# hongsukchoi/Pose2Mesh_RELEASE

Hardware: AMD Instinct MI355X
Metric: SMPL meshes/sec fwd+bwd at batch 256 (higher is better)
Workload: dtype f32 (emulated on the BF16 matrix pipe: every operand as 3 exact bf16 slices = 24-bit significands, 6 slice products per fp32 product, fp32 accumulate)

## Files before the change

include/p2m.h:

```cpp
#ifndef P2M_H_
#define P2M_H_

#include <stddef.h>
#include <stdint.h>

#ifdef __cplusplus
extern "C" {
#endif

typedef enum {
  P2M_OK = 0,
  P2M_ERR_INVALID = -1,
  P2M_ERR_HIP = -2,
  P2M_ERR_NOMEM = -3
} p2m_status;

enum { P2M_ARITH_F32 = 0, P2M_ARITH_BF16X3 = 1, P2M_ARITH_F16X2 = 2 };

typedef struct p2m_graph* p2m_graph_t;

const char* p2m_last_error_string(void);
const char* p2m_version(void);
int p2m_stream_capture_id(void* stream, unsigned long long* id_out);

int p2m_graph_create(const int32_t* row_ptr, const int32_t* col, const float* val,
                     int32_t V, int32_t nnz, p2m_graph_t* out);
int p2m_graph_destroy(p2m_graph_t g);
int p2m_graph_info(p2m_graph_t g, int32_t info[4]);

int p2m_cheb_basis_fwd(p2m_graph_t g, const float* X, float* T1, float* T2,
                       int32_t B, int32_t F, int32_t in_shift, void* stream);

int p2m_cheb_basis_bwd(p2m_graph_t g, const float* d0, const float* d1, const float* d2,
                       const float* resid, float* dX,
                       int32_t B, int32_t F, int32_t out_shift, void* stream);

int p2m_cheb_combine_small(p2m_graph_t g, const float* P, int32_t ldp, int32_t nc, const float* bias,
                           float* Y, int32_t B, void* stream);
int p2m_cheb_expand_small(p2m_graph_t g, const float* G, int32_t nc, float* E, int32_t lde, int32_t B,
                          void* stream);
int p2m_cheb_combine_small_real(p2m_graph_t g, const float* P, int32_t ldp, int32_t nc, const float* bias, float* Y,
                                int32_t B, const int32_t* out_index, int32_t out_rows, float scale, void* stream);

int p2m_weight_pack(const float* W, float* Wt, float* W2, float* W3, int32_t Fout, int32_t Fin, int32_t K,
                    void* stream);
int p2m_weight_grad_unpack(const float* P, const float* Pdb, int32_t nchunks, float* dW, float* db,
                           int32_t Fout, int32_t Fin, int32_t K, int32_t accumulate, int32_t layout,
                           int32_t pdb_stride, void* stream);

int p2m_gemm_planes(const float* A0, const float* A1, const float* A2, int32_t nplanesA, int32_t Ka,
                    int32_t a0_shift, const float* Bm, const void* Bsplit, int32_t arith, const void* a_amax,
                    int32_t a_bits, const float* bias, const float* addend,
                    float* C0, float* C1, float* C2, int32_t nplanesC, int32_t Nc, int32_t pair_out,
                    int64_t M, float* stats, const float* act_scale, const float* act_shift, int32_t act_relu,
                    void* amax_out, void* stream);
int64_t p2m_weight_split_elems(int32_t K, int32_t N, int32_t arith);
int p2m_weight_split(const float* Bm, int32_t K, int32_t N, int32_t arith, const void* amax_in, int32_t amax_bits,
                     void* Bx, void* stream);
typedef struct p2m_conv_weights {
  const float* W;
  int32_t Fout, Fin;
  float fake_a, fake_b;
  int32_t eff_bits, reserved;
  void *Bx_f, *Bx_ef, *Bx_b, *Bx_eb;
  void* amax;
} p2m_conv_weights;
int p2m_conv_weights_prepare(const p2m_conv_weights* dev_desc, int32_t n, int32_t arith, void* stream);
int p2m_amax(const float* x, int64_t n, void* word, void* stream);
int p2m_amax_rows(p2m_graph_t g, int32_t row_set, const float* x, int32_t B, int32_t F, void* word, void* stream);
int32_t p2m_stats_tile_rows(void);

int p2m_gemm_tn(const float* A0, const float* A1, const float* A2, int32_t nplanesA, int32_t Ka,
                int32_t a0_shift, const float* G0, const float* G1, const float* G2, int32_t nplanesG,
                int32_t Gc, int64_t M, int64_t chunk_rows, float* P, float* Pdb, int32_t arith,
                const void* a_amax, int32_t a_bits, const void* g_amax, int32_t g_bits, void* stream);

int p2m_bn_finalize(const float* stats, int32_t ntiles, int64_t M, const float* gamma, const float* beta,
                    float* running_mean, float* running_var, float momentum, float eps,
                    float* mean, float* invstd, float* scale, float* shift, int32_t N, int32_t tile_rows,
                    void* stream);
int p2m_bn_eval_coeffs(const float* gamma, const float* beta, const float* running_mean,
                       const float* running_var, float eps, float* mean, float* invstd, float* scale,
                       float* shift, int32_t N, void* stream);
int p2m_bn_act_fwd(const float* y, const float* scale, const float* shift, int32_t relu,
                   const float* resid, int32_t Fres, int32_t res_shift,
                   float* x, int64_t M, int32_t F, p2m_graph_t classes , int32_t real_rows_only,
                   void* amax_out, void* stream);
int32_t p2m_bn_bwd_blocks(int64_t M, int32_t F);
int32_t p2m_bn_bwd_blocks_classes(p2m_graph_t classes, int64_t M, int32_t F);
int p2m_bn_bwd_reduce(const float* gx, const float* y, const float* scale, const float* shift,
                      const float* mean, const float* invstd, int32_t relu, float* part,
                      int64_t M, int32_t F, p2m_graph_t classes, void* stream);
int p2m_bn_bwd_finalize(const float* part, int32_t nblk, int64_t M, float* dgamma, float* dbeta,
                        float* coef, int32_t accumulate, int32_t F, void* stream);
int32_t p2m_bn_bwd_blocks_fake(p2m_graph_t g, int32_t B, int32_t F);
int p2m_bn_bwd_reduce_fake(p2m_graph_t g, const float* gx, const float* y, const float* scale, const float* shift,
                           const float* mean, const float* invstd, int32_t relu, float* part, int32_t B, int32_t F,
                           void* stream);
int p2m_bn_bwd_apply(const float* gx, const float* y, const float* scale, const float* shift,
                     const float* mean, const float* invstd, const float* gamma, const float* coef,
                     int32_t relu, float* gy, float* pair_gx, float* pair_gy, int64_t M, int32_t F,
                     p2m_graph_t classes, int32_t zero_holes, void* amax_out, void* stream);

int p2m_pair_sum(const float* in, float* out, int64_t Mout, int32_t F, p2m_graph_t classes ,
                 void* stream);
int p2m_lerp_bwd_add(const float* g, float* dst, int64_t M, int32_t F, int32_t Fres, void* stream);

int p2m_graph_split_info(p2m_graph_t g, int32_t counts[2] , float coef[2] );
int p2m_cheb_basis_fwd_real(p2m_graph_t g, const float* X, float* T1c, float* T2c, int32_t B, int32_t F,
                            int32_t in_shift, const float* act_scale , const float* act_shift, void* stream);
int p2m_graph_pair_info(p2m_graph_t g, int32_t counts[2] );
int p2m_graph_plan_info(p2m_graph_t g, int32_t ntiles[3]);
int p2m_cheb_basis_pair(p2m_graph_t g, const float* G, float* P1c, float* P2c, int32_t B, int32_t F, void* stream);
int p2m_gemm_planes_rows(p2m_graph_t g, int32_t row_set, int32_t B, const float* A0, const float* A1,
                         const float* A2, int32_t nplanesA, int32_t Ka, int32_t a0_shift, int32_t planes_compact,
                         const float* Bm, const void* Bsplit, int32_t arith, const void* a_amax, int32_t a_bits,
                         const float* bias, const float* addend, float* C,
                         int32_t N, float* stats, const float* act_scale, const float* act_shift, int32_t act_relu,
                         void* amax_out, const float* in_scale , const float* in_shift, void* stream);
int32_t p2m_rows_tiles_per_sample(p2m_graph_t g, int32_t row_set);
int p2m_gemm_tn_rows(p2m_graph_t g, int32_t row_set, int32_t B, const float* A, int32_t Ka, int32_t a0_shift,
                     const float* G0, const float* G1, const float* G2, int32_t nplanesG, int32_t Gc,
                     int32_t planes_compact, int32_t splits, float* P, float* Pdb, int32_t arith,
                     const void* a_amax, const void* g_amax, int32_t g_bits, const float* a_scale,
                     const float* a_shift, void* stream);
int p2m_weight_eff(const float* Wt, float* We, int32_t Ka, int32_t N, float a, float b, void* stream);
int p2m_weight_grad_unpack2(const float* P, const float* Pdb, int32_t nchunks, const float* P2, const float* Pdb2,
                            int32_t nchunks2, float s1, float s2, float* dW, float* db, int32_t Fout, int32_t Fin,
                            int32_t K, int32_t accumulate, void* stream);
int p2m_bn_finalize_rows(const float* stats_a, int32_t tps_a, int32_t rows_a, const float* stats_b, int32_t tps_b,
                         int32_t rows_b, int32_t B, const float* gamma, const float* beta, float* running_mean,
                         float* running_var, float momentum, float eps, float* mean, float* invstd, float* scale,
                         float* shift, int32_t N, void* stream);

int p2m_bn_finalize_split(p2m_graph_t g, const float* stats_real, const float* stats_fake, int32_t B,
                          const float* gamma, const float* beta, float* running_mean, float* running_var,
                          float momentum, float eps, float* mean, float* invstd, float* scale, float* shift,
                          int32_t N, void* stream);

int32_t p2m_cheb_tile_gemm_supported(p2m_graph_t g, int32_t plan, int32_t Ka, int32_t N);
int32_t p2m_cheb_tile_gemm_bnr_slots(p2m_graph_t g, int32_t plan, int32_t arith, int32_t N, int32_t B);
int32_t p2m_cheb_tile_gemm_mg(int32_t arith, int32_t N);
int p2m_cheb_tile_gemm(p2m_graph_t g, int32_t plan, const float* X, const float* A0, int32_t Ka, const void* Bx,
                       int32_t arith, const void* x_amax, const float* bias, const float* addend, float* C, int32_t N,
                       float* stats, float* E1, float* E2, const float* act_scale, const float* act_shift,
                       int32_t act_relu, void* amax_out, const float* in_scale, const float* in_shift,
                       const float* bnr_y, const float* bnr_co, float* bnr_part, int32_t B, void* stream);
int p2m_act_bound(const float* scale, const float* shift, int32_t N, const void* y_amax, void* word, void* stream);
int32_t p2m_graph_plane_bits(p2m_graph_t g, int32_t plan);
int p2m_bn_finalize_tiles(p2m_graph_t g, int32_t plan, const float* stats_real, const float* stats_fake, int32_t B,
                          const float* gamma, const float* beta, float* running_mean, float* running_var,
                          float momentum, float eps, float* mean, float* invstd, float* scale, float* shift,
                          int32_t N, void* stream);

int p2m_graph_fake_ids(p2m_graph_t g, int32_t* out );
int p2m_graph_real_ids(p2m_graph_t g, int32_t* out);
int p2m_graph_set_classes(p2m_graph_t g, const int32_t* rep_of );
int p2m_graph_class_info(p2m_graph_t g, int32_t counts[3] );
int p2m_stats_rows_w(p2m_graph_t g, const float* y, int32_t B, int32_t N, float* stats, void* stream);
int p2m_class_reduce(p2m_graph_t g, const float* in, float* out, int32_t B, int32_t F, void* stream);

int p2m_chebconv_fwd(p2m_graph_t g, const float* X, const float* Wt, const float* bias,
                     float* T1, float* T2, float* Y, float* stats,
                     int32_t B, int32_t Fin, int32_t Fout, int32_t in_shift, void* stream);

int64_t p2m_mesh_loss_workspace(int32_t B, int32_t nv, int32_t F, int32_t J);
int p2m_mesh_loss(const float* cam_mesh, int32_t V0, const int32_t* perm, int32_t nv, const float* gt_mesh,
                  const float* valid_mesh, const int32_t* faces, int32_t F, const int32_t* vf_ptr,
                  const int32_t* vf_idx, const int32_t* jr_ptr, const int32_t* jr_idx, const float* jr_val,
                  const int32_t* vj_ptr, const int32_t* vj_idx, const float* vj_val, int32_t J,
                  const float* gt_pose, const float* valid_pose, float w_vertex, float w_normal, float w_edge,
                  float w_joint, float* workspace, float* losses, float* grad_cam, int32_t B, void* stream);

int p2m_coord_loss(const float* pred, const float* target, const float* valid, int32_t per_mask, int64_t n, float w,
                   float* loss, float* grad, void* stream);

int p2m_mesh_epilogue(const float* cam_mesh, int32_t V0, const int32_t* perm, int32_t nv, float scale,
                      const int32_t* jr_ptr, const int32_t* jr_idx, const float* jr_val, int32_t J,
                      float* mesh, float* joints, int32_t B, void* stream);

int p2m_rigid_align(const float* A, const float* B, int32_t nb, int32_t N, float* c, float* R, float* t, float* A2,
                    void* stream);
int p2m_mesh_eval(const float* pred_mesh, const float* gt_mesh, int32_t B, int32_t B_real, int32_t nv, float gt_mesh_scale,
                  const int32_t* ra_ptr, const int32_t* ra_idx, const float* ra_val, int32_t JA, int32_t root_A,
                  const int32_t* sub_A, int32_t nsub_A, const float* pred_joints_A, const float* gt_joints_A,
                  const int32_t* re_ptr, const int32_t* re_idx, const float* re_val, int32_t JE, int32_t root_E, const int32_t* sub_E,
                  int32_t nsub_E, const float* gt_joints_E, int32_t pa_mesh, float* mpjpe_A, float* mpvpe, float* mpjpe_E,
                  float* pa_mpjpe_E, float* pa_mpvpe, double* sample_means, const int32_t* group, int32_t n_groups,
                  double* totals, void* stream);

int32_t p2m_nn_target_tile(void);
int32_t p2m_nn_query_tile(int32_t n);
int64_t p2m_nn_workspace(int32_t B, int32_t nA, int32_t nB);
int p2m_mesh_fscore(const float* pred_mesh, const float* gt_mesh, int32_t B, int32_t B_real, int32_t nv, float gt_mesh_scale,
                    const int32_t* r_ptr, const int32_t* r_idx, const float* r_val, int32_t J, int32_t root,
                    const float* pred_centre, const float* gt_centre, int32_t variants, const float* thresholds,
                    int32_t n_thresholds, void* workspace, int64_t workspace_bytes, float* d_pred, float* d_gt,
                    float* pa_d_pred, float* pa_d_gt, int32_t* counts, double* scores, const int32_t* group, int32_t n_groups,
                    double* totals, void* stream);
int p2m_point_nn(const float* A, const float* B, int32_t nb, int32_t nA, int32_t nB, float* dAB, float* dBA, void* workspace,
                 int64_t workspace_bytes, void* stream);

// ... 142 lines not shown
```

pose2mesh_release_amd/_lib.py:

```python
import ctypes
import os

HERE = os.path.dirname(os.path.abspath(__file__))
LIBDIR = os.path.join(HERE, "lib")


class P2MError(RuntimeError):
    pass


_c = ctypes
_i32, _i64, _f32, _f64, _vp = _c.c_int32, _c.c_int64, _c.c_float, _c.c_double, _c.c_void_p


class FitSchedule(_c.Structure):
    _fields_ = [("n", _i32), ("first_step", _i32 * 8), ("lr", _f64 * 8)]


HIP_SYMBOLS = {
    "p2m_last_error_string": (_c.c_char_p, []),
    "p2m_version": (_c.c_char_p, []),
    "p2m_stream_capture_id": (_c.c_int, [_vp, _c.POINTER(_c.c_uint64)]),
    "p2m_graph_create": (_c.c_int, [_vp, _vp, _vp, _i32, _i32, _c.POINTER(_vp)]),
    "p2m_graph_destroy": (_c.c_int, [_vp]),
    "p2m_graph_info": (_c.c_int, [_vp, _c.POINTER(_i32 * 4)]),
    "p2m_cheb_basis_fwd": (_c.c_int, [_vp, _vp, _vp, _vp, _i32, _i32, _i32, _vp]),
    "p2m_cheb_basis_bwd": (_c.c_int, [_vp, _vp, _vp, _vp, _vp, _vp, _i32, _i32, _i32, _vp]),
    "p2m_cheb_combine_small": (_c.c_int, [_vp, _vp, _i32, _i32, _vp, _vp, _i32, _vp]),
    "p2m_cheb_combine_small_real": (_c.c_int, [_vp, _vp, _i32, _i32, _vp, _vp, _i32, _vp, _i32, _f32, _vp]),
    "p2m_cheb_expand_small": (_c.c_int, [_vp, _vp, _i32, _vp, _i32, _i32, _vp]),
    "p2m_weight_pack": (_c.c_int, [_vp, _vp, _vp, _vp, _i32, _i32, _i32, _vp]),
    "p2m_weight_grad_unpack": (_c.c_int, [_vp, _vp, _i32, _vp, _vp, _i32, _i32, _i32, _i32, _i32, _i32, _vp]),
    "p2m_graph_split_info": (_c.c_int, [_vp, _c.POINTER(_i32 * 2), _c.POINTER(_f32 * 2)]),
    "p2m_cheb_basis_fwd_real": (_c.c_int, [_vp, _vp, _vp, _vp, _i32, _i32, _i32, _vp, _vp, _vp]),
    "p2m_graph_pair_info": (_c.c_int, [_vp, _c.POINTER(_i32 * 2)]),
    "p2m_graph_plan_info": (_c.c_int, [_vp, _c.POINTER(_i32 * 3)]),
    "p2m_cheb_basis_pair": (_c.c_int, [_vp, _vp, _vp, _vp, _i32, _i32, _vp]),
    "p2m_gemm_planes_rows": (_c.c_int, [_vp, _i32, _i32, _vp, _vp, _vp, _i32, _i32, _i32, _i32, _vp, _vp, _i32, _vp, _i32,
                                        _vp, _vp, _vp, _i32, _vp, _vp, _vp, _i32, _vp, _vp, _vp, _vp]),
    "p2m_rows_tiles_per_sample": (_i32, [_vp, _i32]),
    "p2m_gemm_tn_rows": (_c.c_int, [_vp, _i32, _i32, _vp, _i32, _i32, _vp, _vp, _vp, _i32, _i32, _i32, _i32, _vp, _vp,
                                    _i32, _vp, _vp, _i32, _vp, _vp, _vp]),
    "p2m_weight_eff": (_c.c_int, [_vp, _vp, _i32, _i32, _f32, _f32, _vp]),
    "p2m_weight_grad_unpack2": (_c.c_int, [_vp, _vp, _i32, _vp, _vp, _i32, _f32, _f32, _vp, _vp, _i32, _i32, _i32,
                                           _i32, _vp]),
    "p2m_bn_finalize_rows": (_c.c_int, [_vp, _i32, _i32, _vp, _i32, _i32, _i32, _vp, _vp, _vp, _vp, _f32, _f32, _vp,
                                        _vp, _vp, _vp, _i32, _vp]),
    "p2m_bn_finalize_split": (_c.c_int, [_vp, _vp, _vp, _i32, _vp, _vp, _vp, _vp, _f32, _f32, _vp, _vp, _vp, _vp, _i32,
                                         _vp]),
    "p2m_cheb_tile_gemm_supported": (_i32, [_vp, _i32, _i32, _i32]),
    "p2m_cheb_tile_gemm_mg": (_i32, [_i32, _i32]),
    "p2m_cheb_tile_gemm": (_c.c_int, [_vp, _i32, _vp, _vp, _i32, _vp, _i32, _vp, _vp, _vp, _vp, _i32, _vp, _vp, _vp, _vp,
                                      _vp, _i32, _vp, _vp, _vp, _vp, _vp, _vp, _i32, _vp]),
    "p2m_cheb_tile_gemm_bnr_slots": (_i32, [_vp, _i32, _i32, _i32, _i32]),
    "p2m_bn_bwd_blocks_fake": (_i32, [_vp, _i32, _i32]),
    "p2m_bn_bwd_reduce_fake": (_c.c_int, [_vp, _vp, _vp, _vp, _vp, _vp, _vp, _i32, _vp, _i32, _i32, _vp]),
    "p2m_act_bound": (_c.c_int, [_vp, _vp, _i32, _vp, _vp, _vp]),
    "p2m_graph_plane_bits": (_i32, [_vp, _i32]),
    "p2m_amax": (_c.c_int, [_vp, _i64, _vp, _vp]),
    "p2m_conv_weights_prepare": (_c.c_int, [_vp, _i32, _i32, _vp]),
    "p2m_amax_rows": (_c.c_int, [_vp, _i32, _vp, _i32, _i32, _vp, _vp]),
    "p2m_bn_finalize_tiles": (_c.c_int, [_vp, _i32, _vp, _vp, _i32, _vp, _vp, _vp, _vp, _f32, _f32, _vp, _vp, _vp, _vp,
                                         _i32, _vp]),
    "p2m_graph_fake_ids": (_c.c_int, [_vp, _vp]),
    "p2m_graph_real_ids": (_c.c_int, [_vp, _vp]),
    "p2m_graph_set_classes": (_c.c_int, [_vp, _vp]),
    "p2m_graph_class_info": (_c.c_int, [_vp, _c.POINTER(_i32 * 3)]),
    "p2m_stats_rows_w": (_c.c_int, [_vp, _vp, _i32, _i32, _vp, _vp]),
    "p2m_class_reduce": (_c.c_int, [_vp, _vp, _vp, _i32, _i32, _vp]),
    "p2m_gemm_planes": (_c.c_int, [_vp, _vp, _vp, _i32, _i32, _i32, _vp, _vp, _i32, _vp, _i32, _vp, _vp, _vp, _vp, _vp,
                                   _i32, _i32, _i32, _i64, _vp, _vp, _vp, _i32, _vp, _vp]),
    "p2m_weight_split_elems": (_i64, [_i32, _i32, _i32]),
    "p2m_weight_split": (_c.c_int, [_vp, _i32, _i32, _i32, _vp, _i32, _vp, _vp]),
    "p2m_stats_tile_rows": (_i32, []),
    "p2m_gemm_tn": (_c.c_int, [_vp, _vp, _vp, _i32, _i32, _i32, _vp, _vp, _vp, _i32, _i32, _i64, _i64, _vp, _vp,
                               _i32, _vp, _i32, _vp, _i32, _vp]),
    "p2m_bn_finalize": (_c.c_int, [_vp, _i32, _i64, _vp, _vp, _vp, _vp, _f32, _f32, _vp, _vp, _vp, _vp,
                                   _i32, _i32, _vp]),
    "p2m_bn_eval_coeffs": (_c.c_int, [_vp, _vp, _vp, _vp, _f32, _vp, _vp, _vp, _vp, _i32, _vp]),
    "p2m_bn_act_fwd": (_c.c_int, [_vp, _vp, _vp, _i32, _vp, _i32, _i32, _vp, _i64, _i32, _vp, _i32, _vp, _vp]),
    "p2m_bn_bwd_blocks": (_i32, [_i64, _i32]),
    "p2m_bn_bwd_blocks_classes": (_i32, [_vp, _i64, _i32]),
    "p2m_bn_bwd_reduce": (_c.c_int, [_vp, _vp, _vp, _vp, _vp, _vp, _i32, _vp, _i64, _i32, _vp, _vp]),
    "p2m_bn_bwd_finalize": (_c.c_int, [_vp, _i32, _i64, _vp, _vp, _vp, _i32, _i32, _vp]),
    "p2m_bn_bwd_apply": (_c.c_int, [_vp, _vp, _vp, _vp, _vp, _vp, _vp, _vp, _i32, _vp, _vp, _vp, _i64, _i32, _vp,
                                    _i32, _vp, _vp]),
    "p2m_pair_sum": (_c.c_int, [_vp, _vp, _i64, _i32, _vp, _vp]),
    "p2m_lerp_bwd_add": (_c.c_int, [_vp, _vp, _i64, _i32, _i32, _vp]),
    "p2m_coord_loss": (_c.c_int, [_vp, _vp, _vp, _i32, _i64, _f32, _vp, _vp, _vp]),
    "p2m_mesh_loss_workspace": (_i64, [_i32, _i32, _i32, _i32]),
    "p2m_mesh_loss": (_c.c_int, [_vp, _i32, _vp, _i32, _vp, _vp, _vp, _i32, _vp, _vp, _vp, _vp, _vp, _vp, _vp, _vp,
                                 _i32, _vp, _vp, _f32, _f32, _f32, _f32, _vp, _vp, _vp, _i32, _vp]),
    "p2m_mesh_epilogue": (_c.c_int, [_vp, _i32, _vp, _i32, _f32, _vp, _vp, _vp, _i32, _vp, _vp, _i32, _vp]),
    "p2m_adam_step": (_c.c_int, [_vp, _vp, _vp, _vp, _i64, _i64, _f32, _f32, _f32, _f32, _f32, _vp]),
    "p2m_rmsprop_step": (_c.c_int, [_vp, _vp, _vp, _i64, _f32, _f32, _f32, _f32, _vp]),
    "p2m_adam_step_dev": (_c.c_int, [_vp, _vp, _vp, _vp, _i64, _vp, _f32, _f32, _f32, _vp]),
    "p2m_rmsprop_step_dev": (_c.c_int, [_vp, _vp, _vp, _i64, _vp, _f32, _f32, _vp]),
    "p2m_gemm_tn_acc": (_c.c_int, [_vp, _i32, _vp, _i32, _i64, _vp, _i32, _vp, _vp, _vp]),
    "p2m_pn_stage_fwd": (_c.c_int, [_vp, _i32, _vp, _vp, _vp, _i32, _i32, _vp, _vp, _vp, _vp, _f32, _f32, _vp, _f32, _vp,
                                    _vp, _vp, _vp, _vp, _i32, _i32, _i32, _vp]),
    "p2m_pn_stage_bwd": (_c.c_int, [_vp, _i32, _vp, _i32, _i32, _vp, _vp, _vp, _vp, _vp, _vp, _f32, _vp, _vp, _vp, _vp,
                                    _vp, _i32, _vp, _i32, _i32, _i32, _vp]),
    "p2m_chebconv_fwd": (_c.c_int, [_vp, _vp, _vp, _vp, _vp, _vp, _vp, _vp, _i32, _i32, _i32, _i32, _vp]),
    "p2m_rigid_align": (_c.c_int, [_vp, _vp, _i32, _i32, _vp, _vp, _vp, _vp, _vp]),
    "p2m_mesh_eval": (_c.c_int, [_vp, _vp, _i32, _i32, _i32, _f32, _vp, _vp, _vp, _i32, _i32, _vp, _i32, _vp, _vp, _vp, _vp,
                                 _vp, _i32, _i32, _vp, _i32, _vp, _i32, _vp, _vp, _vp, _vp, _vp, _vp, _vp, _i32, _vp, _vp]),
    "p2m_nn_target_tile": (_i32, []),
    "p2m_nn_query_tile": (_i32, [_i32]),
    "p2m_nn_workspace": (_i64, [_i32, _i32, _i32]),
    "p2m_mesh_fscore": (_c.c_int, [_vp, _vp, _i32, _i32, _i32, _f32, _vp, _vp, _vp, _i32, _i32, _vp, _vp, _i32, _vp, _i32,
                                   _vp, _i64, _vp, _vp, _vp, _vp, _vp, _vp, _vp, _i32, _vp, _vp]),
    "p2m_point_nn": (_c.c_int, [_vp, _vp, _i32, _i32, _i32, _vp, _vp, _vp, _i64, _vp]),
    "p2m_error_profile_workspace": (_i64, [_i32, _i32]),
    "p2m_error_profile": (_c.c_int, [_vp, _vp, _vp, _i32, _i32, _i32, _f32, _i32, _i32, _vp, _i32, _vp, _i64, _vp, _vp, _vp,
                                     _vp, _i32, _vp, _vp, _vp, _vp, _vp, _vp, _vp]),
    "p2m_body_sample_tile": (_i32, []),
    "p2m_body_vertex_tile": (_i32, []),
    "p2m_body_workspace": (_i64, [_i32, _i32, _i32]),
    "p2m_body_forward": (_c.c_int, [_vp, _vp, _vp, _i32, _vp, _i32, _f32, _i32, _i32, _i32, _i32, _vp, _vp, _vp, _vp, _vp,
                                    _vp, _vp, _i32, _vp, _vp, _i32, _vp, _vp, _vp, _i32, _vp, _i64, _vp, _vp, _vp, _vp]),
    "p2m_body_backward_workspace": (_i64, [_i32, _i32, _i32, _i32]),
    "p2m_body_backward": (_c.c_int, [_vp, _vp, _vp, _i32, _i32, _i32, _f32, _i32, _i32, _i32, _i32, _vp, _vp, _vp, _vp, _vp,
                                     _vp, _vp, _vp, _i32, _vp, _vp, _i32, _vp, _vp, _vp, _i32, _vp, _i64, _vp, _vp, _vp, _vp,
                                     _i64, _vp, _vp, _vp, _vp]),
    "p2m_pose_noise_coco": (_c.c_int, [_vp, _vp, _vp, _vp, _vp, _vp, _i32, _vp]),
    "p2m_pose_noise_table": (_c.c_int, [_vp, _vp, _vp, _vp, _i32, _f32, _f32, _vp, _vp, _i32, _vp]),
    "p2m_train_sample_workspace": (_i64, [_i32]),
    "p2m_train_sample": (_c.c_int, [_vp, _vp, _f32, _vp, _vp, _i32, _i32, _vp, _vp, _vp, _i32, _i32, _vp, _vp, _vp, _i32, _vp,
                                    _i32, _i32, _vp, _vp, _f32, _vp, _vp, _f32, _i32, _i32, _vp, _vp, _vp, _vp, _vp, _i32,
                                    _f32, _f32, _vp, _vp, _i64] + [_vp] * 12),
    "p2m_annot_gather": (_c.c_int, [_vp] * 10 + [_i64, _i32, _i32, _i32, _vp, _i32, _i32, _vp, _vp, _i32, _i32, _i32, _i32,
                                    _f64, _f64] + [_vp] * 10),
    "p2m_body_select": (_c.c_int, [_vp, _vp, _vp, _i32, _vp, _i32, _i32, _i32, _i32, _vp, _vp, _vp, _vp]),
    "p2m_mesh_project": (_c.c_int, [_vp, _vp, _i32, _i32, _i32, _i32, _vp, _vp, _vp]),
    "p2m_mesh_render_workspace": (_c.c_int, [_i32, _i32, _i32, _i32, _i32, _c.POINTER(_i64)]),
    "p2m_mesh_render": (_c.c_int, [_vp, _vp, _i32, _vp, _vp, _vp, _i32, _f32, _f32, _f32, _i32, _vp, _i32, _i32, _i32, _i32,
                                   _i32, _i32, _vp, _vp, _vp, _vp, _vp, _vp, _vp]),
    "p2m_vertex_normals": (_c.c_int, [_vp, _vp, _vp, _vp, _i32, _i32, _i32, _i32, _vp, _vp, _vp]),
    "p2m_mesh_shade": (_c.c_int, [_vp, _vp, _vp, _vp, _i32, _vp, _vp, _vp, _i32, _vp, _vp, _i32, _f32, _vp, _i32, _i32, _vp, _i32,
                                  _vp, _i32, _f32, _i32, _i32, _i32, _i32, _i32, _vp, _vp, _vp, _vp, _vp]),
    "p2m_pose_prepare": (_c.c_int, [_vp, _i32, _i32, _f32, _f32, _f32, _vp, _vp, _vp, _vp, _vp]),
    "p2m_camera_fit": (_c.c_int, [_vp, _vp, _vp, _vp, _vp, _i32, _i32, FitSchedule, _i32, _f32, _f64, _f64, _f64, _vp, _vp, _vp,
                                  _vp]),
    "p2m_one_euro_lookahead": (_i32, []),
    "p2m_one_euro": (_c.c_int, [_vp, _vp, _vp, _i32, _i32, _i32, _f64, _f64, _f64, _f64, _vp, _vp, _vp, _vp, _vp]),
    "p2m_video_eval": (_c.c_int, [_vp, _vp, _vp, _vp, _i32, _i32, _i32, _i32, _vp, _vp, _vp, _vp, _vp, _vp, _vp, _vp]),
    "p2m_pose_overlay_workspace": (_c.c_int, [_i32, _i32, _i32, _i32, _c.POINTER(_i64)]),
    "p2m_pose_overlay": (_c.c_int, [_vp, _i32, _i32, _i32, _i32, _vp, _i32, _vp, _i32, _vp, _c.c_uint32, _vp, _vp, _i32, _i32,
                                    _f32, _i32, _i32, _i32, _i32, _i32, _vp, _vp, _i64, _vp]),
    "p2m_crowd_select": (_c.c_int, [_vp, _vp, _i32, _i32, _i32, _vp, _i32, _f64, _f64, _f64, _vp, _vp, _vp, _vp, _vp, _vp, _vp,
                                    _vp]),
    "p2m_person_colours": (_c.c_int, [_vp, _i32, _f64, _f64, _vp, _vp, _vp]),
    "p2m_pose_track": (_c.c_int, [_vp, _i32, _i32, _i32, _i32, _i32, _f64, _f64, _i32, _i32, _vp, _vp, _vp, _vp, _vp, _vp, _vp,
                                  _vp, _vp, _vp, _vp, _vp]),
}

HOST_SYMBOLS = {
    "p2m_hem_match": (_i64, [_vp, _vp, _vp, _i64, _vp, _i64, _vp, _vp]),
    "p2m_tree_order_level": (_i64, [_vp, _i64, _vp, _i64, _vp]),
# ... 40 lines not shown
```

pose2mesh_release_amd/csrc/basis.hip:

```cpp
#include <cstdlib>

#include "p2m_common.h"

namespace p2m {

constexpr int ROWS_PER_BLOCK = 4;

static int basis_spb() { return 8; }

static bool basis_tiled() {
  static int v = [] { const char* e = getenv("P2M_BASIS_TILED"); return e ? atoi(e) : 1; }();
  return v != 0;
}

__device__ __forceinline__ int xcd_swizzle(int bid, int nb) {
  return (nb & 7) == 0 ? (bid & 7) * (nb >> 3) + (bid >> 3) : bid;
}

__device__ __forceinline__ void fma4(float4& acc, float s, const float4& x) {
  acc.x = fmaf(s, x.x, acc.x); acc.y = fmaf(s, x.y, acc.y);
  acc.z = fmaf(s, x.z, acc.z); acc.w = fmaf(s, x.w, acc.w);
}

template <int LPR>
// ... 137 lines not shown
  const long ibase = (long)b * g.V * F + f;
  float acc = 0.f;
  for (int ch = 0; ch < (1 << out_shift); ch++) {
    int row = (p << out_shift) + ch;
    acc += d0[ibase + (long)row * F];
    if (resid) acc += resid[ibase + (long)row * F];
    for (int j = g.rowptr[row]; j < g.rowptr[row + 1]; j++) {
      long o = ibase + (long)g.col[j] * F;
      acc = fmaf(g.a[j], d1[o], acc);
      acc = fmaf(g.b[j], d2[o], acc);
    }
  }
  dX[idx] = acc;
}

template <int NC>
__global__ __launch_bounds__(256) void k_combine_small(Graph g, const float* __restrict__ P, int ldp,
                                                        const float* __restrict__ bias, float* __restrict__ Y, int B,
                                                        const int* __restrict__ ids, int nset,
                                                        const int* __restrict__ out_index, int out_rows, float scale,
                                                        int skip_real) {
  const int n = ids ? nset : g.V;
  long idx = (long)blockIdx.x * blockDim.x + threadIdx.x;
  if (idx >= (long)B * n) return;
  const int b = (int)(idx / n);
  const int i = (int)(idx - (long)b * n);
  const int row = ids ? ids[i] : i;
  if (skip_real && g.rowptr[row + 1] - g.rowptr[row] > 1) return;
  const long base = (long)b * g.V * ldp;
  const int src = g.rep_of ? g.rep_of[row] : row;
  const float* p0 = P + base + (long)src * ldp;
  float acc[NC];
#pragma unroll
  for (int c = 0; c < NC; c++) acc[c] = p0[c] + (bias ? bias[c] : 0.f);
  for (int j = g.rowptr[src]; j < g.rowptr[src + 1]; j++) {
    const float* q = P + base + (long)g.col[j] * ldp;
    const float a = g.a[j], bb = g.b[j];
#pragma unroll
    for (int c = 0; c < NC; c++) acc[c] = fmaf(bb, q[2 * NC + c], fmaf(a, q[NC + c], acc[c]));
  }
  long orow = row;
  int rows_out = g.V;
  if (out_index) {
    orow = out_index[row];
    rows_out = out_rows;
    if (orow < 0) return;
  }
  float* y = Y + ((long)b * rows_out + orow) * NC;
#pragma unroll
  for (int c = 0; c < NC; c++) y[c] = out_index ? acc[c] * scale : acc[c];
}

template <int NC>
__global__ __launch_bounds__(256) void k_expand_small(Graph g, const float* __restrict__ G, float* __restrict__ E,
                                                       int lde, int B, int skip_real) {
  long idx = (long)blockIdx.x * blockDim.x + threadIdx.x;
  if (idx >= (long)B * g.V) return;
  const int row = (int)(idx % g.V);
  if (skip_real && g.rowptr[row + 1] - g.rowptr[row] > 1) return;
  const long base = (idx - row) * NC;
  float t1[NC], t2[NC];
#pragma unroll
  for (int c = 0; c < NC; c++) t1[c] = t2[c] = 0.f;
  for (int j = g.rowptr[row]; j < g.rowptr[row + 1]; j++) {
    const float* q = G + base + (long)g.col[j] * NC;
    const float a = g.a[j], b = g.b[j];
#pragma unroll
    for (int c = 0; c < NC; c++) {
      t1[c] = fmaf(a, q[c], t1[c]);
      t2[c] = fmaf(b, q[c], t2[c]);
    }
  }
  float* e = E + idx * lde;
#pragma unroll
  for (int c = 0; c < NC; c++) {
    e[c] = G[idx * NC + c];
    e[NC + c] = t1[c];
    e[2 * NC + c] = t2[c];
  }
  for (int c = 3 * NC; c < lde; c++) e[c] = 0.f;
}

constexpr int SMALL_SPB = 8;
template <int NC>
__global__ __launch_bounds__(256) void k_combine_small_tile(TilePlan pl, const int* __restrict__ real_ids, int V,
                                                             const float* __restrict__ P, int ldp,
                                                             const float* __restrict__ bias, float* __restrict__ Y, int B,
                                                             const int* __restrict__ out_index, int out_rows,
                                                             float scale) {
  __shared__ float4 ents[TILE_ECAP];
  __shared__ int rowoff[TILE_RMAX + 1];
  __shared__ float xs[SMALL_SPB][TILE_UCAP][2 * NC];
  const int tile = blockIdx.x % pl.ntiles, sg = blockIdx.x / pl.ntiles;
  const int t = threadIdx.x;
  const int r0 = pl.tile_row[tile], R = pl.tile_row[tile + 1] - r0;
  const int u0 = pl.tile_u[tile], U = pl.tile_u[tile + 1] - u0;
  const int e0 = pl.erow[r0], nE = pl.erow[r0 + R] - e0;
  for (int i = t; i < nE; i += 256) ents[i] = pl.ent[e0 + i];
  if (t <= R) rowoff[t] = pl.erow[r0 + t] - e0;
  const int b0 = sg * SMALL_SPB;
  for (int q = t; q < U * SMALL_SPB; q += 256) {
    const int u = q % U, sl = q / U, b = b0 + sl;
    if (b < B) {
      const float* src = P + ((long)b * V + pl.ucol[u0 + u]) * ldp + NC;
#pragma unroll
      for (int c = 0; c < 2 * NC; c++) xs[sl][u][c] = src[c];
    }
  }
  __syncthreads();
  const int i = t % TILE_RMAX, sl = t / TILE_RMAX, b = b0 + sl;
  if (i >= R || b >= B) return;
  const int row = real_ids[r0 + i];
  const float* p0 = P + ((long)b * V + row) * ldp;
  float acc[NC];
#pragma unroll
  for (int c = 0; c < NC; c++) acc[c] = p0[c] + (bias ? bias[c] : 0.f);
  for (int j = rowoff[i]; j < rowoff[i + 1]; j++) {
    const float4 en = ents[j];
    const float* q = xs[sl][__float_as_int(en.z)];
#pragma unroll
    for (int c = 0; c < NC; c++) acc[c] = fmaf(en.y, q[NC + c], fmaf(en.x, q[c], acc[c]));
  }
  long orow = row;
  int rows_out = V;
  if (out_index) {
    orow = out_index[row];
    rows_out = out_rows;
    if (orow < 0) return;
  }
  float* y = Y + ((long)b * rows_out + orow) * NC;
#pragma unroll
  for (int c = 0; c < NC; c++) y[c] = out_index ? acc[c] * scale : acc[c];
}

template <int NC>
__global__ __launch_bounds__(256) void k_expand_small_tile(TilePlan pl, const int* __restrict__ real_ids, int V,
                                                            const float* __restrict__ G, float* __restrict__ E, int lde,
                                                            int B) {
  __shared__ float4 ents[TILE_ECAP];
  __shared__ int rowoff[TILE_RMAX + 1];
  __shared__ float xs[SMALL_SPB][TILE_UCAP][NC];
  const int tile = blockIdx.x % pl.ntiles, sg = blockIdx.x / pl.ntiles;
  const int t = threadIdx.x;
  const int r0 = pl.tile_row[tile], R = pl.tile_row[tile + 1] - r0;
  const int u0 = pl.tile_u[tile], U = pl.tile_u[tile + 1] - u0;
  const int e0 = pl.erow[r0], nE = pl.erow[r0 + R] - e0;
  for (int i = t; i < nE; i += 256) ents[i] = pl.ent[e0 + i];
  if (t <= R) rowoff[t] = pl.erow[r0 + t] - e0;
  const int b0 = sg * SMALL_SPB;
  for (int q = t; q < U * SMALL_SPB; q += 256) {
    const int u = q % U, sl = q / U, b = b0 + sl;
    if (b < B) {
      const float* src = G + ((long)b * V + pl.ucol[u0 + u]) * NC;
#pragma unroll
      for (int c = 0; c < NC; c++) xs[sl][u][c] = src[c];
    }
  }
  __syncthreads();
  const int i = t % TILE_RMAX, sl = t / TILE_RMAX, b = b0 + sl;
  if (i >= R || b >= B) return;
  const long ridx = (long)b * V + real_ids[r0 + i];
  float t1[NC], t2[NC];
#pragma unroll
  for (int c = 0; c < NC; c++) t1[c] = t2[c] = 0.f;
  for (int j = rowoff[i]; j < rowoff[i + 1]; j++) {
    const float4 en = ents[j];
    const float* q = xs[sl][__float_as_int(en.z)];
#pragma unroll
    for (int c = 0; c < NC; c++) {
      t1[c] = fmaf(en.x, q[c], t1[c]);
      t2[c] = fmaf(en.y, q[c], t2[c]);
    }
  }
  float* e = E + ridx * lde;
#pragma unroll
  for (int c = 0; c < NC; c++) {
    e[c] = G[ridx * NC + c];
    e[NC + c] = t1[c];
    e[2 * NC + c] = t2[c];
  }
  for (int c = 3 * NC; c < lde; c++) e[c] = 0.f;
}

constexpr int EXP_NC = 3, EXP_Q = 3;

__device__ __forceinline__ void expand_stage_row(float4* r, const float* g, const float* t1, const float* t2) {
  r[0] = make_float4(g[0], g[1], g[2], t1[0]);
  r[1] = make_float4(t1[1], t1[2], t2[0], t2[1]);
  r[2] = make_float4(t2[2], 0.f, 0.f, 0.f);
}

__device__ __forceinline__ void expand_copy_out(const float4* res, const long* erow, int nrows, float* __restrict__ E, int lde) {
  const int L4 = lde >> 2;
  for (int u = threadIdx.x; u < nrows * L4; u += 256) {
    const int i = u / L4, q = u - i * L4;
    const long er = erow[i];
    if (er < 0) continue;
    const float4 v = q < EXP_Q ? res[i * EXP_Q + q] : make_float4(0.f, 0.f, 0.f, 0.f);
    reinterpret_cast<float4*>(E + er * lde)[q] = v;
// ... 23 lines not shown
          t1[c] = fmaf(a, q[c], t1[c]);
          t2[c] = fmaf(b, q[c], t2[c]);
        }
      }
#pragma unroll
      for (int c = 0; c < EXP_NC; c++) gv[c] = G[idx * EXP_NC + c];
      expand_stage_row(res + threadIdx.x * EXP_Q, gv, t1, t2);
      er = idx;
    }
  }
  erow[threadIdx.x] = er;
  __syncthreads();
  expand_copy_out(res, erow, 256, E, lde);
}

__global__ __launch_bounds__(256) void k_expand_small_tile_rows(TilePlan pl, const int* __restrict__ real_ids, int V,
                                                                 const float* __restrict__ G, float* __restrict__ E, int lde,
                                                                 int B) {
  __shared__ float4 ents[TILE_ECAP];
  __shared__ int rowoff[TILE_RMAX + 1];
  __shared__ float xs[SMALL_SPB][TILE_UCAP][EXP_NC];
  __shared__ float4 res[256 * EXP_Q];
  __shared__ long erow[256];
  const int bid = xcd_block_id(blockIdx.x, gridDim.x);
  const int tile = bid % pl.ntiles, sg = bid / pl.ntiles;
  const int t = threadIdx.x;
  const int r0 = pl.tile_row[tile], R = pl.tile_row[tile + 1] - r0;
  const int u0 = pl.tile_u[tile], U = pl.tile_u[tile + 1] - u0;
  const int e0 = pl.erow[r0], nE = pl.erow[r0 + R] - e0;
  for (int i = t; i < nE; i += 256) ents[i] = pl.ent[e0 + i];
  if (t <= R) rowoff[t] = pl.erow[r0 + t] - e0;
  const int b0 = sg * SMALL_SPB;
  for (int q = t; q < U * SMALL_SPB; q += 256) {
    const int u = q % U, sl = q / U, b = b0 + sl;
    if (b < B) {
      const float* src = G + ((long)b * V + pl.ucol[u0 + u]) * EXP_NC;
#pragma unroll
      for (int c = 0; c < EXP_NC; c++) xs[sl][u][c] = src[c];
    }
  }
  __syncthreads();
  const int i = t % TILE_RMAX, sl = t / TILE_RMAX, b = b0 + sl;
  long er = -1;
  if (i < R && b < B) {
    const long ridx = (long)b * V + real_ids[r0 + i];
    float t1[EXP_NC], t2[EXP_NC], gv[EXP_NC];
#pragma unroll
    for (int c = 0; c < EXP_NC; c++) t1[c] = t2[c] = 0.f;
    for (int j = rowoff[i]; j < rowoff[i + 1]; j++) {
      const float4 en = ents[j];
      const float* q = xs[sl][__float_as_int(en.z)];
#pragma unroll
      for (int c = 0; c < EXP_NC; c++) {
        t1[c] = fmaf(en.x, q[c], t1[c]);
        t2[c] = fmaf(en.y, q[c], t2[c]);
      }
    }
#pragma unroll
    for (int c = 0; c < EXP_NC; c++) gv[c] = G[ridx * EXP_NC + c];
    expand_stage_row(res + t * EXP_Q, gv, t1, t2);
    er = ridx;
  }
  erow[t] = er;
  __syncthreads();
  expand_copy_out(res, erow, 256, E, lde);
}

}

using namespace p2m;

static int combine_small_launch(p2m_graph_t gh, const float* P, int32_t ldp, int32_t nc, const float* bias, float* Y,
                                int32_t B, int real_only, const int32_t* out_index, int32_t out_rows, float scale,
                                void* stream) {
  const Graph& g = *reinterpret_cast<const Graph*>(gh);
  const int* ids = real_only ? g.real_ids : nullptr;
  const int nset = real_only ? g.n_real : g.V;
  const long tot = (long)B * nset;
  if (tot == 0) return P2M_OK;
  hipStream_t s = (hipStream_t)stream;
  int skip_real = 0;
  const TilePlan& pl = g.plan[0];
  if (pl.ntiles > 0 && basis_tiled() && nc == 3) {
    hipLaunchKernelGGL(k_combine_small_tile<3>, dim3(pl.ntiles * cdiv(B, SMALL_SPB)), dim3(256), 0, s, pl, g.real_ids, g.V,
                       P, ldp, bias, Y, B, out_index, out_rows, scale);
    if (real_only) return check_launch("cheb_combine_small(tiled)");
    skip_real = 1;
  }
#define P2M_COMBINE(NCv) hipLaunchKernelGGL(k_combine_small<NCv>, dim3(cdiv(tot, 256)), dim3(256), 0, s, g, P, ldp, bias, \
                                            Y, B, ids, nset, out_index, out_rows, scale, skip_real)
  switch (nc) {
    case 1: P2M_COMBINE(1); break;
    case 2: P2M_COMBINE(2); break;
    case 3: P2M_COMBINE(3); break;
    case 4: P2M_COMBINE(4); break;
    default: set_error("p2m_cheb_combine_small: nc must be 1..4 (got %d)", nc); return P2M_ERR_INVALID;
  }
#undef P2M_COMBINE
  return check_launch("cheb_combine_small");
}

extern "C" int p2m_cheb_combine_small(p2m_graph_t gh, const float* P, int32_t ldp, int32_t nc, const float* bias,
                                      float* Y, int32_t B, void* stream) {
  P2M_CHECK_ARG(gh && P && Y && ldp >= 3 * nc, "null pointer or ldp < 3*nc");
  if (B <= 0) return P2M_OK;
  return combine_small_launch(gh, P, ldp, nc, bias, Y, B, 0, nullptr, 0, 1.f, stream);
}

extern "C" int p2m_cheb_combine_small_real(p2m_graph_t gh, const float* P, int32_t ldp, int32_t nc, const float* bias,
                                           float* Y, int32_t B, const int32_t* out_index, int32_t out_rows,
                                           float scale, void* stream) {
  P2M_CHECK_ARG(gh && P && Y && ldp >= 3 * nc, "null pointer or ldp < 3*nc");
  P2M_CHECK_ARG(out_index == nullptr || out_rows > 0, "out_rows must be positive with out_index");
  if (B <= 0) return P2M_OK;
  return combine_small_launch(gh, P, ldp, nc, bias, Y, B, 1, out_index, out_rows, scale, stream);
}

extern "C" int p2m_cheb_expand_small(p2m_graph_t gh, const float* G, int32_t nc, float* E, int32_t lde, int32_t B,
                                     void* stream) {
  P2M_CHECK_ARG(gh && G && E && lde >= 3 * nc, "null pointer or lde < 3*nc");
  if (B <= 0) return P2M_OK;
  const Graph& g = *reinterpret_cast<const Graph*>(gh);
  const long tot = (long)B * g.V;
  hipStream_t s = (hipStream_t)stream;
  int skip_real = 0;
  const TilePlan& pl = g.plan[0];
  const bool rows16 = nc == 3 && lde % 4 == 0 && (reinterpret_cast<uintptr_t>(E) & 15) == 0 && narrow_rows();
  if (pl.ntiles > 0 && basis_tiled() && nc == 3) {
    if (rows16)
      hipLaunchKernelGGL(k_expand_small_tile_rows, dim3(pl.ntiles * cdiv(B, SMALL_SPB)), dim3(256), 0, s, pl, g.real_ids,
                         g.V, G, E, lde, B);
    else
      hipLaunchKernelGGL(k_expand_small_tile<3>, dim3(pl.ntiles * cdiv(B, SMALL_SPB)), dim3(256), 0, s, pl, g.real_ids, g.V,
                         G, E, lde, B);
    skip_real = 1;
  }
  if (rows16) {
    hipLaunchKernelGGL(k_expand_small_rows, dim3(cdiv(tot, 256)), dim3(256), 0, s, g, G, E, lde, B, skip_real);
    return check_launch("cheb_expand_small");
  }
  switch (nc) {
    case 1: hipLaunchKernelGGL(k_expand_small<1>, dim3(cdiv(tot, 256)), dim3(256), 0, s, g, G, E, lde, B, skip_real); break;
    case 2: hipLaunchKernelGGL(k_expand_small<2>, dim3(cdiv(tot, 256)), dim3(256), 0, s, g, G, E, lde, B, skip_real); break;
    case 3: hipLaunchKernelGGL(k_expand_small<3>, dim3(cdiv(tot, 256)), dim3(256), 0, s, g, G, E, lde, B, skip_real); break;
    case 4: hipLaunchKernelGGL(k_expand_small<4>, dim3(cdiv(tot, 256)), dim3(256), 0, s, g, G, E, lde, B, skip_real); break;
    default: set_error("p2m_cheb_expand_small: nc must be 1..4 (got %d)", nc); return P2M_ERR_INVALID;
  }
  return check_launch("cheb_expand_small");
}


namespace p2m {
typedef float f32x4v __attribute__((ext_vector_type(4)));

template <int LPR>
__global__ __launch_bounds__(512, 2) void k_basis_tile(TilePlan pl, const float* __restrict__ X,
                                                        float* __restrict__ T1, float* __restrict__ T2, int B, int F,
                                                        long x_rows, int nset, int spb,
                                                        const float* __restrict__ in_scale = nullptr,
                                                        const float* __restrict__ in_shift = nullptr) {
  constexpr int NT = 512;
  constexpr int FB = LPR * 4;
  constexpr int RPI = NT / LPR;
  constexpr int NPF = (TILE_UCAP + RPI - 1) / RPI;
  __shared__ __attribute__((aligned(16))) float xs[TILE_UCAP * FB];
  __shared__ __attribute__((aligned(16))) f32x4v ents[TILE_ECAP];
  __shared__ int rowoff[TILE_RMAX + 1];

// ... 199 lines not shown
```

pose2mesh_release_amd/csrc/gemm.hip:

```cpp
#include <cstdlib>
#include <type_traits>

#include "p2m_split.h"

namespace p2m {

constexpr int BM = 128;
constexpr int BK = 32;
constexpr int AS_LD = BK + 1;

struct GemmArgs {
  const float* A[3];
  const float* Bm;
  const float* bias;
  const float* addend;
  const float* act_scale;
  const float* act_shift;
  int act_relu;
  int pair_out;
  float* C[3];
  float* stats;
  long M;
  int nplanesA, Ka, a0_shift;
  int N, Nc;
  int ntm, ntn;
  const int* ids;
  int nset, V, tps, compact;
  const float* row_w;
  const unsigned short* Bx;
  int Npad, Ktot;
  const unsigned* a_amax;
  const unsigned* b_amax;
  int a_bits;
  unsigned* amax_out;
  const float* in_scale;
  const float* in_shift;
};

__device__ __forceinline__ bool tile_of_block(int bid, int ntm, int ntn, int& mt, int& nt) {
  int xcd = bid & 7;
  int slot = bid >> 3;
  nt = slot % ntn;
  mt = (slot / ntn) * 8 + xcd;
  return mt < ntm;
}

constexpr int ROWTAB_WORDS = 2 * BM + 2;
__device__ __forceinline__ void rows_weights_fill(const GemmArgs& g, int* rowtab, int i, int t) {
  float* wtab = reinterpret_cast<float*>(rowtab + BM);
  const float w = (i < g.nset) ? g.row_w[i] : 0.f;
  wtab[t] = w;
  float s = w;
#pragma unroll
  for (int o = 32; o > 0; o >>= 1) s += __shfl_xor(s, o);
  if ((t & 63) == 0) wtab[BM + (t >> 6)] = s;
}

template <bool ROWS>
__device__ __forceinline__ void epi_group_rows(const int* rowtab, long m0, long M, int ml0, int (&rl)[4]) {
  if (ROWS) {
    const u32x4 rt = *reinterpret_cast<const u32x4*>(rowtab + ml0);
#pragma unroll
    for (int e = 0; e < 4; e++) rl[e] = (int)rt[e];
  } else {
#pragma unroll
    for (int e = 0; e < 4; e++) rl[e] = (m0 + ml0 + e < M) ? ml0 + e : -1;
  }
}

constexpr int EPI_BARRIERS = 2;
#ifndef P2M_EPI_COPYOUT_DEFAULT
#define P2M_EPI_COPYOUT_DEFAULT true
#endif
constexpr int EPI_STRIP_ROWS = 8;
constexpr int EPI_RED_WORDS(int BN) { return 4 * BN; }
constexpr int EPI_LDS_WORDS(int BN, bool CO) { return EPI_RED_WORDS(BN) + (CO ? 4 * 2 * EPI_STRIP_ROWS * (BN / 2) : 0); }
template <int BN, bool EXTRA, bool ROWS, bool CO = false, bool CO_STATS = CO>
__device__ __forceinline__ void gemm_epilogue(const GemmArgs& g, floatx16 (&acc)[2][BN / 64], float* smem,
                                              const int* rowtab, int mt, long m0, int n0, int rs_i0, int wm, int wn,
                                              int l31, int lhi, int descale = 0) {
  constexpr int WTN = BN / 2;
  constexpr int TN = WTN / 32;
  constexpr int TM = 2;
  constexpr int NG = TM * 4;
  const int wnu = __builtin_amdgcn_readfirstlane(wn);
  const bool live = n0 + wnu * WTN < g.N;
  const bool has_stats = (!CO || CO_STATS) && g.stats != nullptr;
  const bool wst = ROWS && g.row_w != nullptr && has_stats;
  const float* wtab = reinterpret_cast<const float*>(rowtab + BM);
  const int mlw = wm * 64 + 4 * lhi;
  float csum[TN];
  float vmax = 0.f;
#pragma unroll
  for (int j = 0; j < TN; j++) csum[j] = 0.f;
  float val[TM][TN][16];
#pragma unroll
  for (int i = 0; i < TM; i++)
#pragma unroll
    for (int j = 0; j < TN; j++)
#pragma unroll
      for (int r = 0; r < 16; r++) val[i][j][r] = acc[i][j][r];

  if (live) {
    float bias_v[TN], sc_v[TN], sh_v[TN];
    bool cok[TN];
    unsigned c4[TN];
    char* Cb[TN];
    const bool pair = !CO && EXTRA && !ROWS && g.pair_out;
    const long rowbase = ROWS ? (long)(mt / g.tps) * g.V : m0;
    const int rowbase32 = (int)rowbase;
    const unsigned pitch = (unsigned)g.Nc * 4u;
#pragma unroll
    for (int j = 0; j < TN; j++) {
      const int nu = n0 + wnu * WTN + j * 32;
      const int n = nu + l31;
      cok[j] = n < g.N;
      bias_v[j] = (g.bias != nullptr && cok[j]) ? g.bias[n] : 0.f;
      sc_v[j] = (g.act_scale != nullptr && cok[j]) ? g.act_scale[n] : 1.f;
      sh_v[j] = (g.act_scale != nullptr && cok[j]) ? g.act_shift[n] : 0.f;
      const int q = (nu >= g.Nc ? 1 : 0) + (nu >= 2 * g.Nc ? 1 : 0);
      float* const Cq = q == 0 ? g.C[0] : (q == 1 ? g.C[1] : g.C[2]);
      Cb[j] = reinterpret_cast<char*>(Cq + (pair ? rowbase >> 1 : rowbase) * g.Nc);
      c4[j] = (unsigned)(n - q * g.Nc) * 4u;
    }
    const char* const Ab = reinterpret_cast<const char*>(g.addend + (EXTRA && g.addend != nullptr ? rowbase * g.Nc : 0));
    constexpr unsigned NOROW = 0xFFFFFFFFu;

    auto row_offsets = [&](int gi, unsigned (&ro)[4]) {
      int rl[4];
      epi_group_rows<ROWS>(rowtab, m0, g.M, mlw + (gi >> 2) * 32 + (gi & 3) * 8, rl);
#pragma unroll
      for (int e = 0; e < 4; e++) {
        ro[e] = rl[e] >= 0 ? (unsigned)(ROWS ? rl[e] - rowbase32 : rl[e]) * pitch : NOROW;
        asm volatile("" : "+v"(ro[e]));
      }
    };
    auto walk = [&](auto add_tag, auto keep_tag) {
      constexpr bool ADD = decltype(add_tag)::value;
      constexpr bool KEEP = decltype(keep_tag)::value;
      float ad[2][ADD ? TN : 1][4];
      auto fetch = [&](int gi) {
        unsigned ro[4];
        row_offsets(gi, ro);
#pragma unroll
        for (int e = 0; e < 4; e++) {
          const unsigned lo = ro[e] != NOROW ? ro[e] : 0u;
#pragma unroll
          for (int j = 0; j < TN; j++)
            ad[gi & 1][j][e] = *reinterpret_cast<const float*>(Ab + (lo + (cok[j] ? c4[j] : 0u)));
        }
      };
      if constexpr (ADD) fetch(0);
#pragma unroll
      for (int j = 0; j < TN; j++) asm volatile("" : "+v"(bias_v[j]), "+v"(sc_v[j]), "+v"(sh_v[j]));
#pragma unroll
      for (int gi = 0; gi < NG; gi++) {
        const int i = gi >> 2, r0 = (gi & 3) * 4;
        const int ml0 = mlw + i * 32 + (gi & 3) * 8;
        if constexpr (ADD) {
          if (gi + 1 < NG) fetch(gi + 1);
        }
        __builtin_amdgcn_sched_barrier(0);
        unsigned ro[4];
        row_offsets(gi, ro);
        float vg[TN][4];
#pragma unroll
        for (int e = 0; e < 4; e++) {
          const int r = r0 + e;
          const bool rok = ro[e] != NOROW;
#pragma unroll
          for (int j = 0; j < TN; j++) {
            float v = __builtin_ldexpf(val[i][j][r], descale) + bias_v[j];
            if (g.act_scale != nullptr) v = fmaf(v, sc_v[j], sh_v[j]);
            if (g.act_relu) v = fmaxf(v, 0.f);
            if constexpr (ADD) v += ad[gi & 1][j][e];
            asm volatile("" : "+v"(v));
            vg[j][e] = v;
            if constexpr (KEEP) val[i][j][r] = v;
            if (!pair && rok && cok[j]) {
#ifdef P2M_PL_ABL_NOSTORE
              if (v == 12345.678f)
#endif
              *reinterpret_cast<float*>(Cb[j] + (ro[e] + c4[j])) = v;
            }
          }
        }
        if (pair) {
#pragma unroll
          for (int e = 0; e < 4; e += 2) {
            if (m0 + ml0 + e < g.M) {
#pragma unroll
              for (int j = 0; j < TN; j++)
                if (cok[j]) {
                  const float pv = vg[j][e] + (m0 + ml0 + e + 1 < g.M ? vg[j][e + 1] : 0.f);
                  *reinterpret_cast<float*>(Cb[j] + ((unsigned)((ml0 + e) >> 1) * pitch + c4[j])) = pv;
                  vmax = fmaxf(vmax, amax_abs(pv));
                }
            }
          }
        } else {
          f32x4 w4 = {0.f, 0.f, 0.f, 0.f};
          if (KEEP && wst) w4 = *reinterpret_cast<const f32x4*>(wtab + ml0);
#pragma unroll
          for (int e = 0; e < 4; e++)
#pragma unroll
            for (int j = 0; j < TN; j++) {
              const float v = vg[j][e];
              const bool ok = ro[e] != NOROW && cok[j];
              if constexpr (KEEP) {
                const float term = wst ? w4[e] * v : v;
                csum[j] += ok ? term : 0.f;
              }
              vmax = fmaxf(vmax, ok ? amax_abs(v) : 0.f);
            }
        }
#pragma unroll
        for (int j = 0; j < TN; j++) asm volatile("" : "+v"(csum[j]));
        asm volatile("" : "+v"(vmax));
        __builtin_amdgcn_sched_barrier(0);
      }
    };
    auto walk_co = [&](auto add_tag, auto keep_tag) {
      constexpr bool ADD = decltype(add_tag)::value;
      constexpr bool KEEP = decltype(keep_tag)::value;
      static_assert(!(ADD && KEEP), "statistics with an addend keep the 4-byte walk");
      constexpr int SB = EPI_STRIP_ROWS * WTN;
      float* const strip = smem + EPI_RED_WORDS(BN) + (wm * 2 + wnu) * 2 * SB;
      int lane = lhi * 32 + l31;
      asm volatile("" : "+v"(lane));
      const int srow = lane >> 3;
      const unsigned col16 = (unsigned)(lane & 7) * 16u;
      float* const wr = strip + (lane >> 5) * 4 * WTN + (lane & 31);
      const int rd0 = srow * WTN + (TN == 2 ? (srow & 1) * 32 : 0) + (lane & 7) * 4;
      const float* rd[TN];
      char* Cc[TN];
      const char* Ac[TN];
      bool ju[TN];
#pragma unroll
      for (int j = 0; j < TN; j++) {
        const int nu = n0 + wnu * WTN + j * 32;
        const int q = (nu >= g.Nc ? 1 : 0) + (nu >= 2 * g.Nc ? 1 : 0);
        ju[j] = nu < g.N;
        Cc[j] = Cb[j] + (unsigned)(nu - q * g.Nc) * 4u;
        Ac[j] = Ab + (ADD && ju[j] ? (unsigned)nu * 4u : 0u);
        rd[j] = strip + (rd0 ^ (j * 32));
      }
      auto co_row = [&](int gi) {
        const int tr = wm * 64 + (gi >> 2) * 32 + (gi & 3) * 8 + srow;
        unsigned ro;
        if (ROWS) {
          const int rl = rowtab[tr];
          ro = rl >= 0 ? (unsigned)(rl - rowbase32) * pitch + col16 : NOROW;
        } else {
          ro = m0 + tr < g.M ? (unsigned)tr * pitch + col16 : NOROW;
        }
        asm volatile("" : "+v"(ro));
        return ro;
      };
      f32x4 cp[TN];
      f32x4 ad[2][ADD ? TN : 1];
      unsigned ro_cur = NOROW, ro_nxt = co_row(0);
#pragma unroll
      for (int j = 0; j < TN; j++) asm volatile("" : "+v"(bias_v[j]), "+v"(sc_v[j]), "+v"(sh_v[j]));
      auto stage = [&](int gi) {
        if constexpr (ADD) {
          const unsigned lo = ro_nxt != NOROW ? ro_nxt : col16;
#pragma unroll
          for (int j = 0; j < TN; j++) ad[gi & 1][j] = *reinterpret_cast<const f32x4*>(Ac[j] + lo);
        }
        __builtin_amdgcn_sched_barrier(0);
        const int i = gi >> 2, r0 = (gi & 3) * 4;
        unsigned ro4[4] = {0u, 0u, 0u, 0u};
        f32x4 w4 = {0.f, 0.f, 0.f, 0.f};
        if constexpr (KEEP) {
          row_offsets(gi, ro4);
          if (wst) w4 = *reinterpret_cast<const f32x4*>(wtab + mlw + i * 32 + (gi & 3) * 8);
        }
#pragma unroll
        for (int e = 0; e < 4; e++)
#pragma unroll
          for (int j = 0; j < TN; j++) {
            const int r = r0 + e;
            float v = __builtin_ldexpf(val[i][j][r], descale) + bias_v[j];
            if (g.act_scale != nullptr) v = fmaf(v, sc_v[j], sh_v[j]);
            if (g.act_relu) v = fmaxf(v, 0.f);
            asm volatile("" : "+v"(v));
            if constexpr (KEEP) {
              val[i][j][r] = v;
              const float term = wst ? w4[e] * v : v;
              csum[j] += (ro4[e] != NOROW && cok[j]) ? term : 0.f;
            }
            wr[(gi & 1) * SB + e * WTN + (TN == 2 ? (j ^ (e & 1)) * 32 : 0)] = v;
          }
        if constexpr (KEEP) {
#pragma unroll
          for (int j = 0; j < TN; j++) asm volatile("" : "+v"(csum[j]));
        }
      };
      auto fetch = [&](int gi) {
        asm volatile("s_waitcnt lgkmcnt(0)" ::: "memory");
        ro_cur = ro_nxt;
        if (gi + 1 < NG) ro_nxt = co_row(gi + 1);
#pragma unroll
        for (int j = 0; j < TN; j++) cp[j] = *reinterpret_cast<const f32x4*>(rd[j] + (gi & 1) * SB);
      };
      auto copy_out = [&](int gi) {
#pragma unroll
        for (int j = 0; j < TN; j++) {
          f32x4 v = cp[j];
          if constexpr (ADD) v += ad[gi & 1][j];
          const bool ok = ro_cur != NOROW && ju[j];
          if (ok) *reinterpret_cast<f32x4*>(Cc[j] + ro_cur) = v;
          const float m4 = fmaxf(fmaxf(amax_abs(v[0]), amax_abs(v[1])), fmaxf(amax_abs(v[2]), amax_abs(v[3])));
          vmax = fmaxf(vmax, ok ? m4 : 0.f);
        }
        asm volatile("" : "+v"(vmax));
      };
      constexpr bool PIPE = !KEEP;
#pragma unroll
      for (int gi = 0; gi <= NG; gi++) {
        if (gi < NG) stage(gi);
        if constexpr (PIPE) {
          if (gi >= 1) copy_out(gi - 1);
          if (gi < NG) fetch(gi);
        } else if (gi < NG) {
          fetch(gi);
          copy_out(gi);
        }
        __builtin_amdgcn_sched_barrier(0);
      }
    };
    const bool add = EXTRA && g.addend != nullptr;
    if constexpr (CO) {
      if (has_stats) {
        if (add) walk(std::true_type{}, std::true_type{});
        else walk_co(std::false_type{}, std::true_type{});
      } else {
        if (add) walk_co(std::true_type{}, std::false_type{});
        else walk_co(std::false_type{}, std::false_type{});
      }
    } else if (has_stats) {
      if (add) walk(std::true_type{}, std::true_type{});
      else walk(std::false_type{}, std::true_type{});
    } else {
      if (add) walk(std::true_type{}, std::false_type{});
      else walk(std::false_type{}, std::false_type{});
    }
  }

  if (has_stats) {
    float* red = smem;
    float* red2 = smem + 2 * BN;
    long rows_valid = ROWS ? (long)(g.nset - rs_i0) : g.M - m0;
    if (rows_valid > BM) rows_valid = BM;
    if (live) {
#pragma unroll
      for (int j = 0; j < TN; j++) {
        csum[j] += __shfl_xor(csum[j], 32);
        if (lhi == 0) red[wm * BN + wn * WTN + j * 32 + l31] = csum[j];
      }
    }
    __syncthreads();
    if (live) {
      float mean[TN], m2[TN];
#pragma unroll
      for (int j = 0; j < TN; j++) {
        const int cl = wn * WTN + j * 32 + l31;
        const float tot = red[cl] + red[BN + cl];
        mean[j] = tot / (wst ? wtab[BM] + wtab[BM + 1] : (float)rows_valid);
        m2[j] = 0.f;
        csum[j] = tot;
      }
#pragma unroll
      for (int gi = 0; gi < NG; gi++) {
        const int i = gi >> 2, r0 = (gi & 3) * 4;
        const int ml0 = mlw + i * 32 + (gi & 3) * 8;
        int rl[4];
        epi_group_rows<ROWS>(rowtab, m0, g.M, ml0, rl);
        f32x4 w4 = {0.f, 0.f, 0.f, 0.f};
        if (wst) w4 = *reinterpret_cast<const f32x4*>(wtab + ml0);
#pragma unroll
        for (int e = 0; e < 4; e++)
#pragma unroll
          for (int j = 0; j < TN; j++) {
            const float d = val[i][j][r0 + e] - mean[j];
            const float wd = wst ? w4[e] * d : d;
            m2[j] = rl[e] >= 0 ? fmaf(wd, d, m2[j]) : m2[j];
          }
      }
#pragma unroll
      for (int j = 0; j < TN; j++) {
        m2[j] += __shfl_xor(m2[j], 32);
        if (lhi == 0) red2[wm * BN + wn * WTN + j * 32 + l31] = m2[j];
// ... 842 lines not shown
  auto store_stage = [&](int buf) {
    float* as = As + buf * RK * BM;
#pragma unroll
    for (int ps = 0; ps < 4; ps++)
      *reinterpret_cast<float4*>(as + (ps * 8 + a_r) * BM + a_c4) = ra[ps];
    float* gs = Gs + buf * RK * BN;
#pragma unroll
    for (int ps = 0; ps < GPASS; ps++)
      *reinterpret_cast<float4*>(gs + (ps * GROWS + g_r) * BN + g_c4) = rg[ps];
  };

  load_ids(r_begin);
  load_stage(r_begin);
  store_stage(0);
  __syncthreads();
  int it = 0;
  for (long r0 = r_begin; r0 < r_end; r0 += RK, it++) {
    const int cur = it & 1;
    const bool more = (r0 + RK) < r_end;
    if (more) load_stage(r0 + RK);
    const float* as = As + cur * RK * BM + lhi * BM + wm * 64 + l31;
    const float* gs = Gs + cur * RK * BN + lhi * BN + wn * WTN + l31;
#pragma unroll
    for (int ks = 0; ks < RK / 2; ks++) {
      float a[TM], b[TN];
#pragma unroll
      for (int i = 0; i < TM; i++) a[i] = as[2 * ks * BM + i * 32];
#pragma unroll
      for (int j = 0; j < TN; j++) b[j] = gs[2 * ks * BN + j * 32];
#pragma unroll
      for (int i = 0; i < TM; i++)
#pragma unroll
        for (int j = 0; j < TN; j++)
          acc[i][j] = __builtin_amdgcn_mfma_f32_32x32x2f32(a[i], b[j], acc[i][j], 0, 0, 0);
    }
    if (more) store_stage(cur ^ 1);
    __syncthreads();
  }

  float* Pc = g.P + (long)chunk * g.Ktot * g.N;
#pragma unroll
  for (int i = 0; i < TM; i++)
#pragma unroll
    for (int j = 0; j < TN; j++) {
      const int n = n0 + wn * WTN + j * 32 + l31;
#pragma unroll
      for (int r = 0; r < 16; r++) {
        const int krow = kk0 + wm * 64 + i * 32 + (r & 3) + 8 * (r >> 2) + 4 * lhi;
        if (krow < g.Ktot && n < g.N) {
          float* d = Pc + (long)krow * g.N + n;
          *d = g.accum ? *d + acc[i][j][r] : acc[i][j][r];
        }
      }
    }
  if (kt == 0 && g.Pdb != nullptr) {
    float* red = smem;
    *reinterpret_cast<float4*>(red + g_r * BN + g_c4) = dbs;
    __syncthreads();
    if (t < BN) {
      float s = 0.f;
#pragma unroll
      for (int q = 0; q < GROWS; q++) s += red[q * BN + t];
      if (n0 + t < g.N) g.Pdb[(long)chunk * g.N + n0 + t] = s;
    }
  }
}

typedef int i32x4 __attribute__((ext_vector_type(4)));

#ifdef P2M_TN_TRACE
__device__ unsigned long long g_tn_tr[8][32][4];
#ifndef P2M_TN_TRACE_S0
#define P2M_TN_TRACE_S0 40
#endif
#define P2M_TNT(s, ev)                                                                                          \
  do {                                                                                                          \
    if (tnt_on && (s) >= P2M_TN_TRACE_S0 && (s) < P2M_TN_TRACE_S0 + 32)                                         \
      g_tn_tr[threadIdx.x >> 6][(s) - P2M_TN_TRACE_S0][ev] = __builtin_amdgcn_s_memtime();                      \
  } while (0)
#else
#define P2M_TNT(s, ev) do { } while (0)
#endif

template <int BN, bool ROWS, int NS>
__global__ __launch_bounds__(512, 2) void k_gemm_tn_ws(TnArgs g) {
  typedef typename SliceFrag<NS>::type frag_t;
  constexpr int RK = 16;
  constexpr int LDX = RK + 8;
  constexpr int WTN = BN / 2;
  constexpr int TN = WTN / 32;
  constexpr int TM = 2;
  constexpr int A_BUF = NS * BM * LDX;
  constexpr int G_BUF = NS * BN * LDX;
  __shared__ __attribute__((aligned(16))) float smem[(2 * A_BUF + 2 * G_BUF) / 2];
  unsigned short* As = reinterpret_cast<unsigned short*>(smem);
  unsigned short* Gs = As + 2 * A_BUF;

  const int ntiles = g.nkt * g.ntn;
  int tile, chunk;
  if (g.nchunks >= 8) {
    const int slot = blockIdx.x >> 3;
    tile = slot % ntiles;
    chunk = (slot / ntiles) * 8 + (blockIdx.x & 7);
  } else {
    tile = blockIdx.x % ntiles;
    chunk = blockIdx.x / ntiles;
  }
  if (chunk >= g.nchunks) return;
  const int kt = tile / g.ntn, nt = tile % g.ntn;
  const int kk0 = kt * BM, n0 = nt * BN;
  const int spc = ROWS ? g.spc : 1;
  const int rs_b = ROWS ? (spc > 1 ? chunk * spc : chunk / g.splits) : 0;
  const int nsamp = (ROWS && spc > 1) ? (g.B - rs_b < spc ? g.B - rs_b : spc) : 1;
  const long r_begin = ROWS ? (spc > 1 ? 0L : (long)(chunk - rs_b * g.splits) * g.chunk_rows) : (long)chunk * g.chunk_rows;
  long r_end = r_begin + g.chunk_rows;
  if (r_end > (ROWS ? (long)g.nset : g.M)) r_end = ROWS ? (long)g.nset : g.M;
  const int nst = r_end > r_begin ? (int)((r_end - r_begin + RK - 1) / RK) : 0;

  const int t = threadIdx.x;
  const bool producer = t >= 256;
#ifdef P2M_TN_TRACE
  const bool tnt_on = blockIdx.x == P2M_TN_TRACE && (t & 63) == 0 && BN == 128 && ROWS;
#endif
  const int pt = t & 255;
  const int lane = t & 63, wave = (t >> 6) & 3;
  const int wm = wave >> 1, wn = wave & 1;
  const int l31 = lane & 31, lhi = lane >> 5;

  floatx16 acc[TM][TN];
#pragma unroll
  for (int i = 0; i < TM; i++)
#pragma unroll
    for (int j = 0; j < TN; j++)
#pragma unroll
      for (int r = 0; r < 16; r++) acc[i][j][r] = 0.f;

  const bool is_a = __builtin_amdgcn_readfirstlane((int)(pt < 128)) != 0;
  const int st = pt & 127;
  const int rq = st & 3;
  const int c4 = is_a ? (st >> 2) : (st >> 2) % (BN / 4);
  const float* src;
  int pitch, shift;
  bool compact_rows;
  unsigned short* dst;
  int slice_stride;
  {
    if (is_a) {
      int kk = kk0 + c4 * 4;
      if (kk >= g.Ktot) kk = 0;
      const int ap = kk / g.Ka;
      src = g.A[ap] + (kk - ap * g.Ka);
      pitch = g.Ka;
      shift = (ap == 0) ? g.a0_shift : 0;
      compact_rows = false;
      dst = As + (c4 >> 2) * 16 * LDX + (c4 & 3) * 2 * LDX + rq * 4;
      slice_stride = BM * LDX;
    } else {
      int n = n0 + c4 * 4;
      if (n >= g.N) n = 0;
      const int gq = n / g.Gc;
      src = g.G[gq] + (n - gq * g.Gc);
      pitch = g.Gc;
      shift = 0;
      compact_rows = ROWS && gq != 0 && g.compact;
      dst = Gs + (c4 >> 2) * 16 * LDX + (c4 & 3) * 2 * LDX + rq * 4;
      slice_stride = BN * LDX;
    }
  }
  const int buf_stride = is_a ? A_BUF : G_BUF;
  const bool a_act = __builtin_amdgcn_readfirstlane((int)(is_a && g.a_scale != nullptr)) != 0;
  f32x4 act_sc = {1.f, 1.f, 1.f, 1.f}, act_sh = {0.f, 0.f, 0.f, 0.f};
  if (a_act) {
    int kk = kk0 + c4 * 4;
    if (kk >= g.Ktot) kk = 0;
    act_sc = *reinterpret_cast<const f32x4*>(g.a_scale + kk);
    act_sh = *reinterpret_cast<const f32x4*>(g.a_shift + kk);
  }
  float my_sc = 1.f;
  int descale = 0;
  if (NS == 2) {
    const int sa = slice_scale_exp(*g.a_amax, g.a_bits), sg = slice_scale_exp(*g.g_amax, g.g_bits);
    my_sc = exp2_int(is_a ? sa : sg);
    descale = -(sa + sg);
  }
  const int* idp = ROWS ? g.ids + r_begin + rq * 4 : nullptr;
  const long base_row = ROWS ? (compact_rows ? (long)rs_b * g.nset + r_begin : (long)rs_b * g.V) : r_begin;
  const char* srcb = reinterpret_cast<const char*>(src + (base_row >> shift) * pitch);
  const long samp_bytes = ROWS ? (((long)(compact_rows ? g.nset : g.V) >> shift) * pitch) * 4 : 0;
  const unsigned pitch4 = (unsigned)pitch * 4u;
  const int nrows_m1 = (int)(r_end - r_begin) - 1;

  f32x4 x0[4], x1[4];
  i32x4 id0 = {0, 0, 0, 0}, id1 = {0, 0, 0, 0};
  f32x4 dbs = {0.f, 0.f, 0.f, 0.f};

  static_assert(ID_SLACK >= 5 * RK && RK == ID_STAGE_ROWS, "the id prefetch of the prologue reads stages 0 .. 4");
  auto load_ids = [&](int kc, i32x4& id) {
    if (ROWS) id = *reinterpret_cast<const i32x4*>(idp + (long)kc * RK);
  };
  auto load_stage = [&](int kc, f32x4 (&x)[4], const i32x4& id, auto clamp_tag) {
    constexpr bool CLAMP = decltype(clamp_tag)::value;
#pragma unroll
    for (int ps = 0; ps < 4; ps++) {
      int rel = kc * RK + rq * 4 + ps;
      if (CLAMP && rel > nrows_m1) rel = nrows_m1;
      if (ROWS && !compact_rows) rel = id[ps];
      const unsigned off = __umul24((unsigned)(rel >> shift), pitch4);
#ifdef P2M_TN_ABL_NOLOAD
      x[ps] = f32x4{__uint_as_float(off), 1.f, 2.f, 3.f};
#else
      x[ps] = *reinterpret_cast<const f32x4*>(srcb + off);
#endif
    }
  };
  auto store_stage = [&](int buf, int kc, f32x4 (&x)[4], auto tail_tag) {
    constexpr bool TAIL = decltype(tail_tag)::value;
#pragma unroll
    for (int ps = 0; ps < 4; ps++) asm volatile("" : "+v"(x[ps]));
    P2M_TNT(kc, 1);
    if (a_act) {
#pragma unroll
      for (int ps = 0; ps < 4; ps++)
#pragma unroll
        for (int e = 0; e < 4; e++) x[ps][e] = fmaxf(fmaf(x[ps][e], act_sc[e], act_sh[e]), 0.f);
    }
    if (TAIL) {
      const int rlast = nrows_m1 + 1 - (kc * RK + rq * 4);
#pragma unroll
      for (int ps = 0; ps < 4; ps++)
        if (ps >= rlast) x[ps] = f32x4{0.f, 0.f, 0.f, 0.f};
    }
    if (!is_a) {
#pragma unroll
      for (int ps = 0; ps < 4; ps++) dbs += x[ps];
    }
    unsigned short* d = dst + buf * buf_stride;
#pragma unroll
    for (int e = 0; e < 4; e++) {
      u32x2 sl[NS];
#ifdef P2M_TN_ABL_NOSLICE
      for (int q = 0; q < NS; q++) sl[q] = u32x2{__float_as_uint(x[q & 1][e]), __float_as_uint(x[2 + (q & 1)][e])};
#else
      split_pack4<NS>(x[0][e], x[1][e], x[2][e], x[3][e], my_sc, sl);
#endif
#pragma unroll
      for (int q = 0; q < NS; q++)
        *reinterpret_cast<u32x2*>(d + ((e & 1) + 8 * (e >> 1)) * LDX + q * slice_stride) = sl[q];
    }
    P2M_TNT(kc, 2);
  };
  using std::false_type;
  using std::true_type;
  auto compute = [&](int cur, int kc) {
    const int lrow = (l31 & 16) + 2 * ((l31 & 15) >> 2) + (l31 & 1) + 8 * ((l31 & 3) >> 1);
    const unsigned short* as = As + cur * A_BUF + (wm * 64 + lrow) * LDX + lhi * 8;
    const unsigned short* gs = Gs + cur * G_BUF + (wn * WTN + lrow) * LDX + lhi * 8;
    frag_t fa[NS][TM], fb[NS][TN];
#pragma unroll
    for (int sl = 0; sl < NS; sl++) {
#pragma unroll
      for (int i = 0; i < TM; i++)
        fa[sl][i] = __builtin_bit_cast(frag_t, *reinterpret_cast<const u32x4*>(as + (sl * BM + i * 32) * LDX));
#pragma unroll
      for (int j = 0; j < TN; j++)
        fb[sl][j] = __builtin_bit_cast(frag_t, *reinterpret_cast<const u32x4*>(gs + (sl * BN + j * 32) * LDX));
    }
#ifdef P2M_TN_TRACE
    asm volatile("s_waitcnt lgkmcnt(0)" ::: "memory");
    P2M_TNT(kc, 1);
#endif
#define P2M_PAIR(SA, SB)                                                                       \
  _Pragma("unroll") for (int i = 0; i < TM; i++) _Pragma("unroll") for (int j = 0; j < TN; j++) \
      acc[i][j] = slice_mfma<NS>(fa[SA][i], fb[SB][j], acc[i][j]);
#ifdef P2M_TN_ABL_NOMFMA
    if constexpr (NS == 3) {
      P2M_PAIR(0, 0)
      for (int sl = 1; sl < NS; sl++)
        for (int i = 0; i < TM; i++) for (int j = 0; j < TN; j++) { asm volatile("" :: "v"(fa[sl][i])); asm volatile("" :: "v"(fb[sl][j])); }
    } else
#endif
    if constexpr (NS == 3) {
      P2M_PAIR(2, 0)
      P2M_PAIR(0, 2)
      P2M_PAIR(1, 1)
      P2M_PAIR(1, 0)
      P2M_PAIR(0, 1)
      P2M_PAIR(0, 0)
    } else {
      P2M_PAIR(1, 0)
      P2M_PAIR(0, 1)
      P2M_PAIR(0, 0)
    }
#undef P2M_PAIR
    P2M_TNT(kc, 2);
    (void)kc;
  };
  auto lds_barrier = [] { asm volatile("s_waitcnt lgkmcnt(0)\n\ts_barrier" ::: "memory"); };

  for (int sb = 0; sb < nsamp; sb++) {
  if (nst > 0) {
    if (producer) {
      load_ids(0, id0);
      load_ids(1, id1);
      load_stage(0, x0, id0, true_type{});
      load_ids(2, id0);
      load_stage(nst > 1 ? 1 : 0, x1, id1, true_type{});
      load_ids(3, id1);
      store_stage(0, 0, x0, true_type{});
      load_stage(nst > 2 ? 2 : nst - 1, x0, id0, true_type{});
      load_ids(4, id0);
      lds_barrier();
      int kc = 0;
      for (; kc + 5 < nst; kc += 2) {
        P2M_TNT(kc + 1, 0);
        store_stage(1, kc + 1, x1, false_type{});
        load_stage(kc + 3, x1, id1, false_type{});
        load_ids(kc + 5, id1);
        P2M_TNT(kc + 1, 3);
        lds_barrier();
        P2M_TNT(kc + 2, 0);
        store_stage(0, kc + 2, x0, false_type{});
        load_stage(kc + 4, x0, id0, false_type{});
        load_ids(kc + 6, id0);
        P2M_TNT(kc + 2, 3);
        lds_barrier();
      }
      for (; kc < nst; kc += 2) {
        if (kc + 1 < nst) store_stage(1, kc + 1, x1, true_type{});
        if (kc + 3 < nst) {
          load_stage(kc + 3, x1, id1, true_type{});
          load_ids(kc + 5, id1);
        }
        lds_barrier();
        if (kc + 1 < nst) {
          if (kc + 2 < nst) store_stage(0, kc + 2, x0, true_type{});
          if (kc + 4 < nst) {
            load_stage(kc + 4, x0, id0, true_type{});
            load_ids(kc + 6, id0);
          }
          lds_barrier();
        }
      }
    } else {
      lds_barrier();
      for (int kc = 0; kc < nst; kc++) {
        P2M_TNT(kc, 0);
        compute(kc & 1, kc);
        P2M_TNT(kc, 3);
        lds_barrier();
      }
    }
  }
  srcb += samp_bytes;
  }
  __syncthreads();

  float* Pc = g.P + (long)chunk * g.Ktot * g.N;
  if (!producer) {
#pragma unroll
    for (int i = 0; i < TM; i++)
#pragma unroll
      for (int j = 0; j < TN; j++) {
        const int n = n0 + wn * WTN + j * 32 + l31;
        if (g.accum) {
          float old[16];
#pragma unroll
          for (int r = 0; r < 16; r++) {
            const int krow = kk0 + wm * 64 + i * 32 + (r & 3) + 8 * (r >> 2) + 4 * lhi;
            old[r] = (krow < g.Ktot && n < g.N) ? Pc[(long)krow * g.N + n] : 0.f;
          }
#pragma unroll
          for (int r = 0; r < 16; r++) {
            const int krow = kk0 + wm * 64 + i * 32 + (r & 3) + 8 * (r >> 2) + 4 * lhi;
            if (krow < g.Ktot && n < g.N) Pc[(long)krow * g.N + n] = __builtin_ldexpf(acc[i][j][r], descale) + old[r];
          }
        } else {
#pragma unroll
          for (int r = 0; r < 16; r++) {
            const int krow = kk0 + wm * 64 + i * 32 + (r & 3) + 8 * (r >> 2) + 4 * lhi;
            if (krow < g.Ktot && n < g.N) Pc[(long)krow * g.N + n] = __builtin_ldexpf(acc[i][j][r], descale) + 0.f;
          }
        }
      }
  }
  if (kt == 0 && g.Pdb != nullptr) {
    float* red = smem;
    if (producer && !is_a && (st >> 2) < BN / 4) *reinterpret_cast<f32x4*>(red + rq * BN + c4 * 4) = dbs;
    __syncthreads();
    if (t < BN) {
      const float sum = red[t] + red[BN + t] + red[2 * BN + t] + red[3 * BN + t];
      if (n0 + t < g.N) g.Pdb[(long)chunk * g.N + n0 + t] = sum;
    }
  }
}

__global__ void k_naive_gemm_tn(TnArgs g) {
  int o = blockIdx.x * blockDim.x + threadIdx.x;
  const int chunk = blockIdx.y;
  const long r_begin = (long)chunk * g.chunk_rows;
  long r_end = r_begin + g.chunk_rows;
  if (r_end > g.M) r_end = g.M;
  const int nout = g.Ktot * g.N;
  if (o < nout) {
    int kk = o / g.N, n = o - kk * g.N;
    int p = kk / g.Ka, k = kk - p * g.Ka;
    const float* Ap = g.A[p];
    int sh = p == 0 ? g.a0_shift : 0;
    float acc = 0.f;
    const int q = n / g.Gc;
    const float* Gq = g.G[q] + (n - q * g.Gc);
    for (long r = r_begin; r < r_end; r++) acc = fmaf(Ap[(r >> sh) * g.Ka + k], Gq[r * g.Gc], acc);
    g.P[(long)chunk * nout + o] = g.accum ? g.P[(long)chunk * nout + o] + acc : acc;
  }
  if (g.Pdb != nullptr && o < g.N) {
    float s = 0.f;
    const int q = o / g.Gc;
    const float* Gq = g.G[q] + (o - q * g.Gc);
    for (long r = r_begin; r < r_end; r++) s += Gq[r * g.Gc];
    g.Pdb[(long)chunk * g.N + o] = s;
  }
}

__global__ void k_weight_pack(const float* __restrict__ W, float* __restrict__ Wt, float* __restrict__ W2,
                              float* __restrict__ W3, int Fout, int Fin, int K) {
  long idx = (long)blockIdx.x * blockDim.x + threadIdx.x;
  long tot = (long)Fout * Fin * K;
  if (idx >= tot) return;
  int fout = (int)(idx % Fout);
  long kk = idx / Fout;
  int k = (int)(kk / Fin), fin = (int)(kk % Fin);
  float v = W[(long)fout * Fin * K + (long)fin * K + k];
  Wt[idx] = v;
  if (W2) W2[(long)fout * Fin * K + kk] = v;
  if (W3) W3[((long)k * Fout + fout) * Fin + fin] = v;
}

__global__ __launch_bounds__(256) void k_transpose_tiled(const float* __restrict__ W, float* __restrict__ Wt, int R, int C) {
  __shared__ float tile[64][65];
  const int r0 = blockIdx.y * 64, c0 = blockIdx.x * 64;
  const int tq = threadIdx.x & 15, ty = threadIdx.x >> 4;
  const bool vec = (C & 3) == 0 && (R & 3) == 0;
#pragma unroll
  for (int p = 0; p < 4; p++) {
    const int r = r0 + ty + 16 * p, c = c0 + 4 * tq;
    if (r < R) {
      if (vec && c + 3 < C) {
        const float4 v = *reinterpret_cast<const float4*>(W + (long)r * C + c);
        tile[ty + 16 * p][4 * tq] = v.x; tile[ty + 16 * p][4 * tq + 1] = v.y;
        tile[ty + 16 * p][4 * tq + 2] = v.z; tile[ty + 16 * p][4 * tq + 3] = v.w;
      } else {
        for (int e = 0; e < 4; e++)
          if (c + e < C) tile[ty + 16 * p][4 * tq + e] = W[(long)r * C + c + e];
      }
    }
  }
  __syncthreads();
#pragma unroll
  for (int p = 0; p < 4; p++) {
    const int c = c0 + ty + 16 * p, r = r0 + 4 * tq;
    if (c < C) {
      if (vec && r + 3 < R) {
        float4 v;
        v.x = tile[4 * tq][ty + 16 * p]; v.y = tile[4 * tq + 1][ty + 16 * p];
        v.z = tile[4 * tq + 2][ty + 16 * p]; v.w = tile[4 * tq + 3][ty + 16 * p];
        *reinterpret_cast<float4*>(Wt + (long)c * R + r) = v;
      } else {
        for (int e = 0; e < 4; e++)
          if (r + e < R) Wt[(long)c * R + r + e] = tile[4 * tq + e][ty + 16 * p];
// ... 449 lines not shown
  if (g.Bx != nullptr) {
    const bool co_ws = co && !(ROWS && wide && g.stats != nullptr);
#define P2M_LAUNCH_WS(BNv, EX)                                                                              \
  do {                                                                                                      \
    if (g.a_amax != nullptr) {                                                                              \
      if (co_ws) hipLaunchKernelGGL((k_gemm_planes_ws<BNv, EX, ROWS, 2, true>), grid, dim3(512), 0, s, g);  \
      else hipLaunchKernelGGL((k_gemm_planes_ws<BNv, EX, ROWS, 2, false>), grid, dim3(512), 0, s, g);       \
    } else {                                                                                                \
      if (co_ws) hipLaunchKernelGGL((k_gemm_planes_ws<BNv, EX, ROWS, 3, true>), grid, dim3(512), 0, s, g);  \
      else hipLaunchKernelGGL((k_gemm_planes_ws<BNv, EX, ROWS, 3, false>), grid, dim3(512), 0, s, g);       \
    }                                                                                                       \
  } while (0)
    if (wide) { if (extra) P2M_LAUNCH_WS(128, true); else P2M_LAUNCH_WS(128, false); }
    else { if (extra) P2M_LAUNCH_WS(64, true); else P2M_LAUNCH_WS(64, false); }
#undef P2M_LAUNCH_WS
  } else {
#define P2M_LAUNCH(BNv, EX) hipLaunchKernelGGL((k_gemm_planes<BNv, 32, EX, ROWS>), grid, dim3(256), 0, s, g)
    if (wide) { if (extra) P2M_LAUNCH(128, true); else P2M_LAUNCH(128, false); }
    else { if (extra) P2M_LAUNCH(64, true); else P2M_LAUNCH(64, false); }
#undef P2M_LAUNCH
  }
}

extern "C" int p2m_gemm_planes(const float* A0, const float* A1, const float* A2, int32_t nplanesA, int32_t Ka,
                               int32_t a0_shift, const float* Bm, const void* Bsplit, int32_t arith,
                               const void* a_amax, int32_t a_bits, const float* bias,
                               const float* addend, float* C0, float* C1, float* C2, int32_t nplanesC, int32_t Nc,
                               int32_t pair_out, int64_t M, float* stats, const float* act_scale,
                               const float* act_shift, int32_t act_relu, void* amax_out, void* stream) {
  P2M_CHECK_ARG(nplanesA >= 1 && nplanesA <= 3 && nplanesC >= 1 && nplanesC <= 3, "plane count must be 1..3");
  P2M_CHECK_ARG(arith == P2M_ARITH_F32 || arith == P2M_ARITH_BF16X3 || arith == P2M_ARITH_F16X2, "unknown arithmetic");
  P2M_CHECK_ARG((act_scale == nullptr) == (act_shift == nullptr), "act_scale / act_shift must both be given or both NULL");
  P2M_CHECK_ARG(!((act_scale || act_relu) && (stats || pair_out)), "fused activation excludes stats and pair_out");
  P2M_CHECK_ARG(A0 && Bm && C0 && Ka > 0 && Nc > 0, "null pointer or empty shape");
  P2M_CHECK_ARG(a0_shift == 0 || a0_shift == 1, "a0_shift must be 0 or 1");
  if (M <= 0) return P2M_OK;
  GemmArgs g;
  g.A[0] = A0; g.A[1] = A1; g.A[2] = A2;
  g.C[0] = C0; g.C[1] = C1; g.C[2] = C2;
  for (int p = 0; p < nplanesA; p++) P2M_CHECK_ARG(g.A[p] != nullptr, "missing A plane");
  for (int p = 0; p < nplanesC; p++) P2M_CHECK_ARG(g.C[p] != nullptr, "missing C plane");
  P2M_CHECK_ARG((addend == nullptr && !pair_out) || nplanesC == 1, "addend / pair_out need a single output plane");
  P2M_CHECK_ARG(!(pair_out && stats), "pair_out and stats are mutually exclusive");
  g.Bm = Bm; g.bias = bias; g.addend = addend; g.pair_out = pair_out; g.stats = stats; g.M = M;
  g.act_scale = act_scale; g.act_shift = act_shift; g.act_relu = act_relu;
  g.nplanesA = nplanesA; g.Ka = Ka; g.a0_shift = a0_shift;
  g.N = nplanesC * Nc; g.Nc = Nc;
  g.ids = nullptr; g.nset = 0; g.V = 0; g.tps = 0; g.compact = 0; g.row_w = nullptr;
  g.Bx = nullptr; g.Npad = 0; g.Ktot = 0;
  g.a_amax = g.b_amax = nullptr; g.a_bits = 0;
  g.amax_out = static_cast<unsigned*>(amax_out);
  g.in_scale = g.in_shift = nullptr;
  hipStream_t s = (hipStream_t)stream;
  const bool mfma_ok = (Ka % BK == 0) && (g.N % 32 == 0) && (Nc % 32 == 0);
  if (!mfma_ok) {
    P2M_CHECK_ARG(!pair_out, "pair_out needs the MFMA path (Ka % 32 == 0, N % 32 == 0)");
    P2M_CHECK_ARG(!amax_out, "amax_out needs the MFMA path (Ka % 32 == 0, N % 32 == 0)");
    long tot = M * g.N;
    g.ntm = g.ntn = 0;
    hipLaunchKernelGGL(k_naive_gemm_planes, dim3(cdiv(tot, 256)), dim3(256), 0, s, g);
    if (stats) {
      P2M_CHECK_ARG(nplanesC == 1, "stats need a single output plane");
      hipLaunchKernelGGL(k_naive_tile_stats, dim3(cdiv(M, BM)), dim3(64), 0, s, C0, stats, (long)M, g.N);
    }
    return check_launch("gemm_planes(naive)");
  }
  if (arith != P2M_ARITH_F32) {
    P2M_CHECK_ARG(Bsplit != nullptr, "the slice arithmetics need the pre-split weight (p2m_weight_split)");
    P2M_CHECK_ARG(arith != P2M_ARITH_F16X2 || a_amax != nullptr, "P2M_ARITH_F16X2 needs the amax word of the A planes");
    g.Bx = static_cast<const unsigned short*>(Bsplit);
    g.Npad = cdiv(g.N, 128) * 128;
    g.Ktot = nplanesA * Ka;
    if (arith == P2M_ARITH_F16X2) {
      g.a_amax = static_cast<const unsigned*>(a_amax);
      g.a_bits = a_bits;
      g.b_amax = weight_amax_word(Bsplit, arith, g.Npad, g.Ktot);
    }
  }
  g.ntm = cdiv(M, BM);
  launch_gemm_planes<false>(g, addend != nullptr || pair_out, s);
  return check_launch("gemm_planes");
}

extern "C" int p2m_gemm_planes_rows(p2m_graph_t gh, int32_t row_set, int32_t B, const float* A0, const float* A1,
                                    const float* A2, int32_t nplanesA, int32_t Ka, int32_t a0_shift,
                                    int32_t planes_compact, const float* Bm, const void* Bsplit, int32_t arith,
                                    const void* a_amax, int32_t a_bits, const float* bias,
                                    const float* addend, float* C, int32_t N, float* stats, const float* act_scale,
                                    const float* act_shift, int32_t act_relu, void* amax_out, const float* in_scale,
                                    const float* in_shift, void* stream) {
  P2M_CHECK_ARG(gh && A0 && Bm && C, "null pointer");
  P2M_CHECK_ARG((in_scale == nullptr) == (in_shift == nullptr), "in_scale / in_shift must both be given or both NULL");
  P2M_CHECK_ARG(in_scale == nullptr || (arith != P2M_ARITH_F32 && Ka <= 256),
                "activation on load exists in the slice arithmetics only, for Ka <= 256");
  P2M_CHECK_ARG(arith == P2M_ARITH_F32 || arith == P2M_ARITH_BF16X3 || arith == P2M_ARITH_F16X2, "unknown arithmetic");
  P2M_CHECK_ARG(arith == P2M_ARITH_F32 || Bsplit != nullptr, "the slice arithmetics need the pre-split weight (p2m_weight_split)");
  P2M_CHECK_ARG(arith != P2M_ARITH_F16X2 || a_amax != nullptr, "P2M_ARITH_F16X2 needs the amax word of the A planes");
  P2M_CHECK_ARG((act_scale == nullptr) == (act_shift == nullptr), "act_scale / act_shift must both be given or both NULL");
  P2M_CHECK_ARG(!((act_scale || act_relu) && stats), "fused activation excludes stats");
  P2M_CHECK_ARG(row_set_valid(row_set), "row_set must be 1 (real), 2 (fake), 3 (paired real) or 4 (paired fake)");
  P2M_CHECK_ARG(nplanesA >= 1 && nplanesA <= 3, "plane count must be 1..3");
  P2M_CHECK_ARG(Ka > 0 && Ka % BK == 0 && N > 0 && N % 32 == 0, "Ka and N must be positive multiples of 32");
  P2M_CHECK_ARG(a0_shift == 0 || a0_shift == 1, "a0_shift must be 0 or 1");
  const Graph& gr = *reinterpret_cast<const Graph*>(gh);
  const RowSet rs = row_set_of(gr, row_set);
  if (B <= 0 || rs.n == 0) return P2M_OK;
  P2M_CHECK_ARG((long)rs.V * N < (1l << 30), "one sample of C must stay below 4 GiB (V * N < 2^30)");
  GemmArgs g;
  g.A[0] = A0; g.A[1] = A1; g.A[2] = A2;
  for (int p = 0; p < nplanesA; p++) P2M_CHECK_ARG(g.A[p] != nullptr, "missing A plane");
  g.C[0] = C; g.C[1] = nullptr; g.C[2] = nullptr;
  g.Bm = Bm; g.bias = bias; g.addend = addend; g.pair_out = 0; g.stats = stats;
  g.act_scale = act_scale; g.act_shift = act_shift; g.act_relu = act_relu;
  g.nplanesA = nplanesA; g.Ka = Ka; g.a0_shift = a0_shift; g.N = N; g.Nc = N;
  g.ids = rs.ids; g.nset = rs.n; g.V = rs.V; g.tps = cdiv(rs.n, BM); g.compact = planes_compact;
  g.row_w = (stats != nullptr && row_set == 2) ? gr.fake_wts : nullptr;
  g.Bx = arith == P2M_ARITH_F32 ? nullptr : static_cast<const unsigned short*>(Bsplit);
  g.Npad = cdiv(N, 128) * 128;
  g.Ktot = nplanesA * Ka;
  g.a_amax = g.b_amax = nullptr; g.a_bits = 0;
  if (arith == P2M_ARITH_F16X2) {
    g.a_amax = static_cast<const unsigned*>(a_amax);
    g.a_bits = a_bits;
    g.b_amax = weight_amax_word(Bsplit, arith, g.Npad, g.Ktot);
  }
  g.amax_out = static_cast<unsigned*>(amax_out);
  g.in_scale = in_scale; g.in_shift = in_shift;
  g.M = (long)B * g.tps * BM;
  g.ntm = B * g.tps;
  launch_gemm_planes<true>(g, addend != nullptr, (hipStream_t)stream);
  return check_launch("gemm_planes_rows");
}

extern "C" int32_t p2m_rows_tiles_per_sample(p2m_graph_t gh, int32_t row_set) {
  if (!gh || !row_set_valid(row_set)) return 0;
  const Graph& gr = *reinterpret_cast<const Graph*>(gh);
  return cdiv(row_set_of(gr, row_set).n, BM);
}

static int gemm_tn_impl(const float* A0, const float* A1, const float* A2, int32_t nplanesA, int32_t Ka,
                        int32_t a0_shift, const float* G0, const float* G1, const float* G2, int32_t nplanesG,
                        int32_t Gc, int64_t M, int64_t chunk_rows, float* P, float* Pdb, int32_t arith,
                        const void* a_amax, int32_t a_bits, const void* g_amax, int32_t g_bits, int32_t accumulate,
                        void* stream);
extern "C" int p2m_gemm_tn(const float* A0, const float* A1, const float* A2, int32_t nplanesA, int32_t Ka,
                           int32_t a0_shift, const float* G0, const float* G1, const float* G2, int32_t nplanesG,
                           int32_t Gc, int64_t M, int64_t chunk_rows, float* P, float* Pdb, int32_t arith,
                           const void* a_amax, int32_t a_bits, const void* g_amax, int32_t g_bits, void* stream) {
  return gemm_tn_impl(A0, A1, A2, nplanesA, Ka, a0_shift, G0, G1, G2, nplanesG, Gc, M, chunk_rows, P, Pdb, arith, a_amax,
                      a_bits, g_amax, g_bits, 0, stream);
}
extern "C" int p2m_gemm_tn_acc(const float* A, int32_t Ka, const float* G, int32_t N, int64_t M, float* P, int32_t arith,
                               const void* a_amax, const void* g_amax, void* stream) {
  const int64_t chunk_rows = ((M + 31) / 32) * 32;
  return gemm_tn_impl(A, nullptr, nullptr, 1, Ka, 0, G, nullptr, nullptr, 1, N, M, chunk_rows > 0 ? chunk_rows : 32, P,
                      nullptr, arith, a_amax, 0, g_amax, 0, 1, stream);
}
static int gemm_tn_impl(const float* A0, const float* A1, const float* A2, int32_t nplanesA, int32_t Ka,
                        int32_t a0_shift, const float* G0, const float* G1, const float* G2, int32_t nplanesG,
                        int32_t Gc, int64_t M, int64_t chunk_rows, float* P, float* Pdb, int32_t arith,
                        const void* a_amax, int32_t a_bits, const void* g_amax, int32_t g_bits, int32_t accumulate,
                        void* stream) {
  P2M_CHECK_ARG(nplanesA >= 1 && nplanesA <= 3 && nplanesG >= 1 && nplanesG <= 3, "plane count must be 1..3");
  P2M_CHECK_ARG(arith == P2M_ARITH_F32 || arith == P2M_ARITH_BF16X3 || arith == P2M_ARITH_F16X2, "unknown arithmetic");
  P2M_CHECK_ARG(arith != P2M_ARITH_F16X2 || (a_amax && g_amax), "P2M_ARITH_F16X2 needs the amax words of both operands");
  const int N = nplanesG * Gc;
  P2M_CHECK_ARG(A0 && G0 && P && Ka > 0 && Gc > 0 && chunk_rows > 0, "null pointer or empty shape");
  P2M_CHECK_ARG(a0_shift == 0 || a0_shift == 1, "a0_shift must be 0 or 1");
  if (M <= 0) return P2M_OK;
  TnArgs g;
  g.A[0] = A0; g.A[1] = A1; g.A[2] = A2;
  for (int p = 0; p < nplanesA; p++) P2M_CHECK_ARG(g.A[p] != nullptr, "missing A plane");
  g.G[0] = G0; g.G[1] = G1; g.G[2] = G2; g.Gc = Gc;
  for (int p = 0; p < nplanesG; p++) P2M_CHECK_ARG(g.G[p] != nullptr, "missing G plane");
  g.P = P; g.Pdb = Pdb; g.M = M; g.chunk_rows = chunk_rows;
  g.nplanesA = nplanesA; g.Ka = Ka; g.a0_shift = a0_shift; g.Ktot = nplanesA * Ka; g.N = N;
  g.ids = nullptr; g.nset = 0; g.V = 0; g.splits = 1; g.compact = 0;
  g.a_amax = static_cast<const unsigned*>(a_amax); g.g_amax = static_cast<const unsigned*>(g_amax);
  g.a_bits = a_bits; g.g_bits = g_bits;
  g.a_scale = g.a_shift = nullptr;
  const int nchunks = cdiv(M, chunk_rows);
  g.nchunks = nchunks;
  g.accum = accumulate;
  P2M_CHECK_ARG(!accumulate || nchunks == 1, "accumulation needs the whole reduction in one chunk");
  hipStream_t s = (hipStream_t)stream;
  const bool mfma_ok = (Ka % 4 == 0) && (N % 32 == 0) && (Gc % 4 == 0) && (g.Ktot >= 32);
  if (!mfma_ok) {
    g.nkt = g.ntn = 0;
    int nout = g.Ktot * N;
    if (nout < N) nout = N;
    hipLaunchKernelGGL(k_naive_gemm_tn, dim3(cdiv(nout, 256), nchunks), dim3(256), 0, s, g);
    return check_launch("gemm_tn(naive)");
  }
  g.nkt = cdiv(g.Ktot, BM);
  const bool bx = arith != P2M_ARITH_F32;
  if (N % 128 == 0 || (bx && N > 128)) {
    g.ntn = cdiv(N, 128);
    const dim3 grid(g.nkt * g.ntn, nchunks), grid_ws((nchunks >= 8 ? cdiv(nchunks, 8) * 8 : nchunks) * g.nkt * g.ntn);
    if (arith == P2M_ARITH_F16X2) hipLaunchKernelGGL((k_gemm_tn_ws<128, false, 2>), grid_ws, dim3(512), 0, s, g);
    else if (bx) hipLaunchKernelGGL((k_gemm_tn_ws<128, false, 3>), grid_ws, dim3(512), 0, s, g);
    else hipLaunchKernelGGL((k_gemm_tn<128, false>), grid, dim3(256), 0, s, g);
  } else {
    g.ntn = cdiv(N, 64);
    const dim3 grid(g.nkt * g.ntn, nchunks), grid_ws((nchunks >= 8 ? cdiv(nchunks, 8) * 8 : nchunks) * g.nkt * g.ntn);
    if (arith == P2M_ARITH_F16X2) hipLaunchKernelGGL((k_gemm_tn_ws<64, false, 2>), grid_ws, dim3(512), 0, s, g);
    else if (bx) hipLaunchKernelGGL((k_gemm_tn_ws<64, false, 3>), grid_ws, dim3(512), 0, s, g);
    else hipLaunchKernelGGL((k_gemm_tn<64, false>), grid, dim3(256), 0, s, g);
  }
  return check_launch("gemm_tn");
}

extern "C" int p2m_gemm_tn_rows(p2m_graph_t gh, int32_t row_set, int32_t B, const float* A, int32_t Ka,
                                int32_t a0_shift, const float* G0, const float* G1, const float* G2, int32_t nplanesG,
                                int32_t Gc, int32_t planes_compact, int32_t splits, float* P, float* Pdb,
                                int32_t arith, const void* a_amax, const void* g_amax, int32_t g_bits,
                                const float* a_scale, const float* a_shift, void* stream) {
  P2M_CHECK_ARG(gh && A && G0 && P, "null pointer");
  P2M_CHECK_ARG((a_scale == nullptr) == (a_shift == nullptr), "a_scale / a_shift must both be given or both NULL");
  P2M_CHECK_ARG(a_scale == nullptr || arith != P2M_ARITH_F32, "activation on load exists in the slice arithmetics only");
  P2M_CHECK_ARG(arith == P2M_ARITH_F32 || arith == P2M_ARITH_BF16X3 || arith == P2M_ARITH_F16X2, "unknown arithmetic");
  P2M_CHECK_ARG(arith != P2M_ARITH_F16X2 || (a_amax && g_amax), "P2M_ARITH_F16X2 needs the amax words of both operands");
  P2M_CHECK_ARG(row_set_valid(row_set), "row_set must be 1 (real), 2 (fake), 3 (paired real) or 4 (paired fake)");
  P2M_CHECK_ARG(nplanesG >= 1 && nplanesG <= 3 && (splits >= 1 || splits <= -2),
                "plane count must be 1..3; splits >= 1, or <= -2 (that many whole samples per chunk)");
  P2M_CHECK_ARG(splits >= 1 || arith != P2M_ARITH_F32, "several samples per chunk exist in the slice arithmetics only");
  P2M_CHECK_ARG(Ka % 32 == 0 && Gc % 32 == 0, "Ka and Gc must be multiples of 32");
  P2M_CHECK_ARG(a0_shift == 0 || a0_shift == 1, "a0_shift must be 0 or 1");
  const Graph& gr = *reinterpret_cast<const Graph*>(gh);
  const RowSet rs = row_set_of(gr, row_set);
  if (B <= 0 || rs.n == 0) return P2M_OK;
  TnArgs g;
  g.A[0] = A; g.A[1] = nullptr; g.A[2] = nullptr;
  g.G[0] = G0; g.G[1] = G1; g.G[2] = G2; g.Gc = Gc;
  for (int p = 0; p < nplanesG; p++) P2M_CHECK_ARG(g.G[p] != nullptr, "missing G plane");
  const int N = nplanesG * Gc;
  g.P = P; g.Pdb = Pdb; g.M = (long)B * rs.n;
  const int spc = splits < 0 ? -splits : 1;
  if (splits < 0) splits = 1;
  g.chunk_rows = cdiv(rs.n, splits);
  g.nplanesA = 1; g.Ka = Ka; g.a0_shift = a0_shift; g.Ktot = Ka; g.N = N;
  g.ids = rs.ids; g.nset = rs.n; g.V = rs.V; g.splits = splits; g.compact = planes_compact;
  g.spc = spc; g.B = B;
  g.a_amax = static_cast<const unsigned*>(a_amax); g.g_amax = static_cast<const unsigned*>(g_amax);
  g.a_bits = 0; g.g_bits = g_bits;
  g.a_scale = a_scale; g.a_shift = a_shift;
  const int nchunks = spc > 1 ? cdiv(B, spc) : B * splits;
  g.nchunks = nchunks;
  hipStream_t s = (hipStream_t)stream;
  g.nkt = cdiv(g.Ktot, BM);
  const bool bx = arith != P2M_ARITH_F32;
  if (bx) g.chunk_rows = cdiv(g.chunk_rows, 16) * 16;
  if (N % 128 == 0 || (bx && N > 128)) {
    g.ntn = cdiv(N, 128);
    const dim3 grid(g.nkt * g.ntn, nchunks), grid_ws((nchunks >= 8 ? cdiv(nchunks, 8) * 8 : nchunks) * g.nkt * g.ntn);
    if (arith == P2M_ARITH_F16X2) hipLaunchKernelGGL((k_gemm_tn_ws<128, true, 2>), grid_ws, dim3(512), 0, s, g);
    else if (bx) hipLaunchKernelGGL((k_gemm_tn_ws<128, true, 3>), grid_ws, dim3(512), 0, s, g);
    else hipLaunchKernelGGL((k_gemm_tn<128, true>), grid, dim3(256), 0, s, g);
  } else {
    g.ntn = cdiv(N, 64);
    const dim3 grid(g.nkt * g.ntn, nchunks), grid_ws((nchunks >= 8 ? cdiv(nchunks, 8) * 8 : nchunks) * g.nkt * g.ntn);
    if (arith == P2M_ARITH_F16X2) hipLaunchKernelGGL((k_gemm_tn_ws<64, true, 2>), grid_ws, dim3(512), 0, s, g);
    else if (bx) hipLaunchKernelGGL((k_gemm_tn_ws<64, true, 3>), grid_ws, dim3(512), 0, s, g);
    else hipLaunchKernelGGL((k_gemm_tn<64, true>), grid, dim3(256), 0, s, g);
  }
  return check_launch("gemm_tn_rows");
}

extern "C" int p2m_weight_pack(const float* W, float* Wt, float* W2, float* W3, int32_t Fout, int32_t Fin, int32_t K,
                               void* stream) {
  P2M_CHECK_ARG(W && Wt && Fout > 0 && Fin > 0 && K > 0, "null pointer or empty shape");
  long tot = (long)Fout * Fin * K;
  if (K == 1 && W2 == nullptr && W3 == nullptr && (reinterpret_cast<uintptr_t>(W) & 15) == 0 &&
      (reinterpret_cast<uintptr_t>(Wt) & 15) == 0) {
    hipLaunchKernelGGL(k_transpose_tiled, dim3(cdiv(Fin, 64), cdiv(Fout, 64)), dim3(256), 0, (hipStream_t)stream, W, Wt, Fout,
                       Fin);
    return check_launch("weight_pack(transpose)");
  }
  hipLaunchKernelGGL(k_weight_pack, dim3(cdiv(tot, 256)), dim3(256), 0, (hipStream_t)stream, W, Wt, W2, W3, Fout, Fin, K);
  return check_launch("weight_pack");
}

extern "C" int p2m_weight_eff(const float* Wt, float* We, int32_t Ka, int32_t N, float a, float b, void* stream) {
  P2M_CHECK_ARG(Wt && We && Ka > 0 && N > 0, "null pointer or empty shape");
  hipLaunchKernelGGL(k_weight_eff, dim3(cdiv((long)Ka * N, 256)), dim3(256), 0, (hipStream_t)stream, Wt, We, Ka, N, a, b);
  return check_launch("weight_eff");
}

extern "C" int p2m_weight_grad_unpack2(const float* P, const float* Pdb, int32_t nchunks, const float* P2,
// ... 35 lines not shown
```

pose2mesh_release_amd/meshnet.py:

```python
import sys

import numpy as np
import torch
import torch.nn as nn

from . import ops
from ._lib import P2MError
from .cheby_graph_conv import bn_momentum

K_CHEB = 3


def channel_plan(mano, cin, cout):
    if mano:
        return [(cin, 32, 64, 64), (64, 128, 256), (256, 256, 256), (256, 256, 256), (256, 256, 256),
                (256, 128, 128), (128, 64, cout)]
    return [(cin, 32, 64, 64), (64, 128, 256), (256, 256, 256), (256, 256, 256), (256, 256, 256),
            (256, 256, 256), (256, 128, 128), (128, 128, 128), (128, 128, 128), (128, 64, cout)]


def _cfg_says_mano():
    mod = sys.modules.get("core.config")
    try:
        return None if mod is None else (mod.cfg.DATASET.target_joint_set == "mano")
# ... 172 lines not shown
            split = g.split and bwd_fwdform
            images = cws is not None and L.ci in cws.images
            batched = split and images
            want_w3 = bwd_fwdform
            if images:
                Wt, W2, W3 = W, None, W
            else:
                Wt, W2, W3 = wc.get((L.ci, "pack"), W, lambda: ops.weight_pack(W, L.Fin, K_CHEB, need_w2=not want_w3,
                                                                               need_w3=want_w3))
            if split:
                y = torch.empty((M, L.Fout), device=cur.device, dtype=torch.float32)
                opf = cws.fwd(L.ci, W) if batched else wc.get(
                    (L.ci, "split_fwd"), W, lambda: ops.split_operands(Wt, L.Fin, L.Fout, g.fake_a, g.fake_b,
                                                                      wc.get((L.ci, "amax"), W, lambda: ops.param_amax(W))))
                Ln = net._layers[L.ci + 1] if L.ci + 1 < len(net._layers) else None
                fold_out = bool(training and L.has_bn and not L.last_in_block and Ln is not None and Ln.graph == L.graph
                                and (ops.fold_act_ok(g, Ln.Fin, 32, B, narrow=True) if _narrow(Ln) else
                                     (_bwd_forward_form(Ln) and ops.fold_act_ok(g, Ln.Fin, Ln.Fout, B))))
                yword = ops.new_amax(cur.device) if (fold_out and ops.f16x2()) else None
                T1, T2, st, st2, tiled = ops.conv_split(g, B, cur, L.Fin, cur_shift, Wt, bvec, None, y, L.Fout, g.fake_a,
                                                        g.fake_b, need_stats, operands=opf, want_planes=False,
                                                        amax_out=yword, in_act=fold)
                tile_rows = ("tiles", cur_shift) if tiled else "rows"
            else:
                T1, T2 = ops.cheb_basis_fwd(g, cur, B, L.Fin, cur_shift)
                if images:
                    Wtx = cws.images[L.ci][0]
                else:
                    Wtx = wc.get((L.ci, "wtx"), W, lambda: ops.weight_split(Wt, wc.get((L.ci, "amax"), W, lambda: ops.param_amax(W)))) \
                        if (L.Fin % 32 == 0 and L.Fout % 32 == 0) else None
                (y,), st = ops.gemm_planes([cur, T1, T2], L.Fin, cur_shift, Wt, bvec, M, L.Fout, 1, need_stats, Bx=Wtx,
                                           amax=ops.amax_of(cur), amax_bits=g.plane_bits)
                tile_rows = None
                fold_out, yword = False, None
            fold_in, fold = fold, None
            co = None
            if L.has_bn:
                bn = net.bn[L.ci]
                gamma, beta = params[P[f"bn.{L.ci}.weight"]], params[P[f"bn.{L.ci}.bias"]]
                if training and isinstance(tile_rows, tuple):
                    co = ops.bn_finalize_tiles(g, tile_rows[1], B, st, st2, gamma, beta, bn.running_mean, bn.running_var,
                                               bn_momentum(bn), bn.eps)
                    nbt.append(bn.num_batches_tracked)
                elif training and tile_rows == "rows":
                    co = ops.bn_finalize_rows(g, B, st, st2, gamma, beta, bn.running_mean, bn.running_var,
                                              bn_momentum(bn), bn.eps)
                    nbt.append(bn.num_batches_tracked)
                elif training:
                    co = ops.bn_finalize(st, M, gamma, beta, bn.running_mean, bn.running_var, bn_momentum(bn), bn.eps,
                                         tile_rows)
                    nbt.append(bn.num_batches_tracked)
                else:
                    co = ops.bn_eval_coeffs(gamma, beta, bn.running_mean, bn.running_var, bn.eps)
                resid = None
                if L.last_in_block and 1 <= L.block <= nblk - 2:
                    resid = block_in
                if fold_out:
                    out = y.view(M, L.Fout)
                    if yword is not None:
                        ops.tag_amax(out, ops.act_bound(co[2], co[3], yword, ops.new_amax(y.device)))
                    fold = (co[2], co[3])
                else:
                    out = ops.bn_act_fwd(y, co, True, resid, block_in_F, block_in_shift, M, L.Fout,
                                         classes=g if (g.classes and split) else None)
                if net._tap is not None:
                    yt = y
                    if g.classes and g.split:
                        rep = torch.as_tensor(net._class_rep[L.graph], device=y.device, dtype=torch.long)
                        yt = y.view(B, g.V, L.Fout)[:, rep].reshape(M, L.Fout)
                    net._tap.append((L.ci, yt, co[2], co[3]))
            else:
                out = y
            if keep:
                if bwd_fwdform:
                    T1 = T2 = None
                saved.append((cur, cur_shift, T1, T2, y, co, W3 if bwd_fwdform else W2, fold_in))
            cur, cur_shift = out, 0
            if L.last_in_block:
                if L.block == 0:
                    h = ops.view_tagged(cur, B, J * L.Fout)
                    fw, fb = params[P["fc.weight"]], params[P["fc.bias"]]
                    Nf, Kf = fw.shape
                    if ops.GEMM_ARITH != "f32" and B % 4 == 0 and B >= 32 and Nf % 32 == 0 and Kf % 32 == 0:
                        fwt = wc.get("fc_t", fw, lambda: ops.weight_pack(fw, Kf, 1, need_w2=False)[0])
                        ha = ops.amax_of(h)
                        Pu, _, nchu = ops.gemm_tn([ops.tag_amax(h.t().contiguous(), ha)], B, 0, fwt, Kf, Nf, a_amax=ha,
                                                  g_amax=wc.get("fc_amax", fw, lambda: ops.param_amax(fw)))
                        u = (Pu[0] if nchu == 1 else Pu.sum(0)).add_(fb)
                    else:
                        fwt, fwx = wc.get("fc", fw, lambda: _fc_operands(fw, wc.get("fc_amax", fw, lambda: ops.param_amax(fw))))
                        (u,), _ = ops.gemm_planes([h], Kf, 0, fwt, fb, B, Nf, 1, False, Bx=fwx, want_amax=True)
                    if keep:
                        fc_saved = h
                    cur = ops.view_tagged(u, B * net._Vc, net.CL_F[1][0])
                elif L.block < nblk - 2:
                    cur_shift = 1
        if nbt:
            torch._foreach_add_(nbt, 1)
        V0 = graphs[0].V
        ctx.net, ctx.saved, ctx.fc_saved, ctx.B, ctx.training, ctx.cws = net, saved, fc_saved, B, training, cws
        ctx.n_params = len(params)
        ctx.param_shapes = [p.shape for p in params]
        return cur.view(B, V0, net.num_mesh_output_chan)

    @staticmethod
    def backward(ctx, grad_out):
        with torch.cuda.device(grad_out.device):
            ops.set_phase("_bwd")
            try:
                return _MeshNetFn._backward(ctx, grad_out)
            finally:
                ops.set_phase("")

    @staticmethod
    def _backward(ctx, grad_out):
        net, saved, B, training = ctx.net, ctx.saved, ctx.B, ctx.training
        if saved is None or len(saved) == 0:
            raise P2MError("backward called but the forward ran without gradient tracking (or twice)")
        graphs = net._graph_cache.on(grad_out.device)
        wc = net._weight_cache
        cws = ctx.cws
        P = net._param_index
        params = ctx.saved_params
        grads = [None] * ctx.n_params
        nblk = len(net.CL_F)
        J = net.num_joint

        def tgt(*names):
            if not net._direct_grad:
                return None
            out = []
            for n in names:
                gbuf = params[P[n]].grad
                if gbuf is None or gbuf.dtype != torch.float32 or not gbuf.is_contiguous() \
                        or gbuf.device != grad_out.device:
                    return None
                out.append(gbuf)
            return out
        def ready(*names):
            if net._grad_sink is not None and net._direct_grad:
                net._grad_sink([params[P[n]] for n in names])
        G = grad_out.contiguous().float().view(-1, net.num_mesh_output_chan)
        g_out = graphs[net._layers[-1].graph]
        if g_out.classes:
            G = ops.class_reduce(g_out, G, B, net.num_mesh_output_chan)
        g_cur = G
        keep = []
        main_stream = torch.cuda.current_stream()
        side = ops.side_stream(grad_out.device) if ops.DW_SIDE_STREAM else None

        class side_ctx:

            def __init__(self, keep_list, *tensors):
                keep_list.extend(tensors)

            def __enter__(self):
                if side is not None:
                    side.wait_stream(main_stream)
                    self.cm = torch.cuda.stream(side)
                    self.cm.__enter__()

            def __exit__(self, *a):
                if side is not None:
                    self.cm.__exit__(*a)
                return False
        Gs_block = None
        bnr_pending = None
        for L in reversed(net._layers):
            gph = graphs[L.graph]
            M = B * gph.V
            X, x_shift, T1, T2, y, co, W2, fold_in = saved[L.ci]
            if L.last_in_block:
                if L.block == 0:
                    fw = params[P["fc.weight"]]
                    dU = ops.view_tagged(G, B, fw.shape[0])
                    h = ctx.fc_saved
                    Nf, Kf = fw.shape
                    tg = tgt("fc.weight", "fc.bias")
                    if ops.GEMM_ARITH != "f32" and B % 4 == 0 and B >= 32 and Nf % 32 == 0 and Kf % 32 == 0:
                        dUa = ops.amax_of(dU)
                        Pw, _, nch = ops.gemm_tn([dU], Nf, 0, h, B, Kf, a_amax=dUa, g_amax=ops.amax_of(h))
                        dbv = dU.sum(0)
                        if tg is not None:
                            if nch == 1:
                                tg[0].add_(Pw[0])
                            else:
                                ops.weight_grad_unpack(Pw, None, nch, Nf, Kf, 1, dW=tg[0], db=None, layout=2)
                            tg[1].add_(dbv)
                            ready("fc.weight", "fc.bias")
                        else:
                            grads[P["fc.weight"]] = Pw[0] if nch == 1 else \
                                ops.weight_grad_unpack(Pw, None, nch, Nf, Kf, 1, layout=2)[0]
                            grads[P["fc.bias"]] = dbv
                        dUt = ops.tag_amax(dU.t().contiguous(), dUa)
                        Ph, _, nch2 = ops.gemm_tn([dUt], B, 0, fw, Nf, Kf, a_amax=dUa,
                                                  g_amax=wc.get("fc_amax", fw, lambda: ops.param_amax(fw)))
                        dh = Ph[0] if nch2 == 1 else Ph.sum(0)
                    else:
                        Pw, Pb, nch = ops.gemm_tn([h], Kf, 0, dU, B, Nf)
                        if tg is not None:
                            ops.weight_grad_unpack(Pw, Pb, nch, Nf, Kf, 1, dW=tg[0], db=tg[1])
                            ready("fc.weight", "fc.bias")
                        else:
                            grads[P["fc.weight"]], grads[P["fc.bias"]] = ops.weight_grad_unpack(Pw, Pb, nch, Nf, Kf, 1)
                        (dh,), _ = ops.gemm_planes([dU], Nf, 0, fw, None, B, Kf, 1, False)
                    G = dh.view(B * J, L.Fout)
                g_cur = G
            if _narrow(L):
                Wp = W2
                E = ops.cheb_expand_small(gph, g_cur, L.Fout, 32, B)
                ew = ops.amax_of(g_cur.view(-1)) if (gph.classes and g_cur.numel() % 4 == 0) else None
                ebits = gph.plane_bits if ew is not None else 0
                if gph.classes:
                    dW32 = db32 = None
                    for rs in (1, 2):
                        Pw, Pb, nch = ops.gemm_tn_rows(gph, rs, B, X, L.Fin, x_shift, [E], 32, False,
                                                       a_amax=ops.amax_of(X) if fold_in is not None else None, a_act=fold_in,
                                                       g_amax=ew, g_bits=ebits)
                        dW32, db32 = ops.weight_grad_unpack(Pw, Pb, nch, 32, L.Fin, 1, dW=dW32, db=db32)
                else:
                    Pw, Pb, nch = ops.gemm_tn([X], L.Fin, x_shift, E, M, 32)
                    dW32, db32 = ops.weight_grad_unpack(Pw, Pb, nch, 32, L.Fin, 1)
                nco = K_CHEB * L.Fout
                dWn = dW32[:nco].view(K_CHEB, L.Fout, L.Fin).permute(1, 2, 0).reshape(L.Fout, L.Fin * K_CHEB)
                tg = tgt(f"cl.{L.ci}.weight", f"cl.{L.ci}.bias")
                if tg is not None:
                    tg[0].add_(dWn)
                    tg[1].add_(db32[:L.Fout])
                    ready(f"cl.{L.ci}.weight", f"cl.{L.ci}.bias")
                else:
                    grads[P[f"cl.{L.ci}.weight"]] = dWn.contiguous()
                    grads[P[f"cl.{L.ci}.bias"]] = db32[:L.Fout].contiguous()
                Wl = params[P[f"cl.{L.ci}.weight"]]
                Wpt, Wptx = wc.get((L.ci, "narrow_bwd"), Wl, lambda: _transposed_operands(
                    Wp, wc.get((L.ci, "amax"), Wl, lambda: ops.param_amax(Wl))))
                if gph.classes:
                    dX = torch.empty((M, L.Fin), device=E.device, dtype=torch.float32)
                    for rs in (1, 2):
                        ops.gemm_planes_rows(gph, rs, B, [E], 32, 0, False, Wpt, None, None, dX, L.Fin, Bx=Wptx, amax=ew,
                                             amax_bits=ebits)
                else:
                    (dX,), _ = ops.gemm_planes([E], 32, 0, Wpt, None, M, L.Fin, 1, False, Bx=Wptx)
                saved[L.ci] = None
                g_cur = dX
                continue
            has_res = L.first_in_block and 1 <= L.block <= nblk - 2
            Fblk = net.CL_F[L.block][-1]
            fuse_res = has_res and (L.Fin == Fblk)
            pair_path = _bwd_forward_form(L) and gph.split and x_shift and gph.pair \
                and (L.Fout in (32, 64) or L.Fout % 128 == 0)
            want_Gs = want_P0 = False
            if L.has_bn and M % 2 == 0 and L.Fout in (32, 64, 128, 256):
                if L.last_in_block and not L.first_in_block:
                    F0 = net._layers[net._block_first[L.block]]
                    want_Gs = bool(saved[F0.ci][1]) and 1 <= F0.block <= nblk - 2 and L.Fout == Fblk
                want_P0 = pair_path
            P0 = None
            if L.has_bn:
                gamma = params[P[f"bn.{L.ci}.weight"]]
                tg = tgt(f"bn.{L.ci}.weight", f"bn.{L.ci}.bias")
                kw = dict(dgamma=tg[0], dbeta=tg[1]) if tg is not None else {}
                res = ops.bn_relu_bwd(g_cur, y, co, gamma, True, training, M, L.Fout, pair_in=want_Gs,
                                      pair_out=want_P0, classes=gph, zero_holes=not gph.split, real_part=bnr_pending, **kw)
                bnr_pending = None
                gy = res[0]
                if tg is None:
                    grads[P[f"bn.{L.ci}.weight"]], grads[P[f"bn.{L.ci}.bias"]] = res[1], res[2]
                else:
                    ready(f"bn.{L.ci}.weight", f"bn.{L.ci}.bias")
                if want_Gs:
                    Gs_block = res[3]
                if want_P0:
                    P0 = res[4]
            else:
                gy = g_cur
            if pair_path:
                Mc = M >> 1
                coarse_full = gph.classes and not graphs[net._layers[L.ci - 1].graph].split
                dX = (torch.zeros if coarse_full else torch.empty)((Mc, L.Fin), device=gy.device, dtype=torch.float32)
                add = (Gs_block if Gs_block is not None else ops.pair_sum(G, Mc, Fblk, classes=gph)) if fuse_res else None
                Wl = params[P[f"cl.{L.ci}.weight"]]
                opb = cws.bwd(L.ci, Wl) if (cws is not None and L.ci in cws.images) else wc.get(
                    (L.ci, "split_bwd"), Wl, lambda: ops.split_operands(W2, L.Fout, L.Fin, gph.fake_a, gph.fake_b,
                                                                      wc.get((L.ci, "amax"), Wl, lambda: ops.param_amax(Wl))))
                P0, E1, E2 = ops.conv_pair(gph, B, gy, L.Fout, W2, add, dX, L.Fin, opb, P0=P0)
                ga = ops.amax_of(gy, gph, B)
                with side_ctx(keep, X, P0, E1, E2):
                    Pw, Pb, nch = ops.gemm_tn_rows(gph, 3, B, X, L.Fin, 0, [P0, E1, E2], L.Fout, True, g_amax=ga,
                                                   g_bits=gph.plane_bits + 1)
                    Pw2, Pb2, nch2 = ops.gemm_tn_rows(gph, 4, B, X, L.Fin, 0, [P0], L.Fout, False, g_amax=ga, g_bits=1)
                    tg = tgt(f"cl.{L.ci}.weight", f"cl.{L.ci}.bias")
                    dW, db = ops.weight_grad_unpack2(Pw, Pb, nch, Pw2, Pb2, nch2, gph.fake_a, gph.fake_b, L.Fout,
                                                     L.Fin, *(tg or ()))
                    keep.extend((Pw, Pb, Pw2, Pb2))
                    if tg is not None:
                        ready(f"cl.{L.ci}.weight", f"cl.{L.ci}.bias")
                if tg is None:
                    grads[P[f"cl.{L.ci}.weight"]], grads[P[f"cl.{L.ci}.bias"]] = dW, db
                del Pw, Pb, Pw2, Pb2, P0, E1, E2, add
            elif _bwd_forward_form(L) and gph.split:
                dXf = torch.empty((M, L.Fin), device=gy.device, dtype=torch.float32)
                add = G if fuse_res else None
                Wl = params[P[f"cl.{L.ci}.weight"]]
                opb = cws.bwd(L.ci, Wl) if (cws is not None and L.ci in cws.images) else wc.get(
                    (L.ci, "split_bwd"), Wl, lambda: ops.split_operands(W2, L.Fout, L.Fin, gph.fake_a, gph.fake_b,
                                                                      wc.get((L.ci, "amax"), Wl, lambda: ops.param_amax(Wl))))
                bnr = None
                if not L.first_in_block and not x_shift and L.ci > 0:
                    Lp, sp = net._layers[L.ci - 1], saved[L.ci - 1]
                    if Lp.has_bn and Lp.graph == L.graph and sp is not None and sp[5] is not None \
                            and ops.tile_gemm_ok(gph, 0, L.Fout, L.Fin, True, B=B):
                        pr = ops.bnr_parts(gph, 0, L.Fin, B, gy.device)
                        if pr is not None:
                            bnr = (sp[4], sp[5], pr[0][pr[1]:])
                            bnr_pending = (gph, pr[0], pr[1])
                E1, E2, _, _, _ = ops.conv_split(gph, B, gy, L.Fout, 0, W2, None, add, dXf, L.Fin, gph.fake_a,
                                                 gph.fake_b, operands=opb, bnr=bnr)
                dX = ops.pair_sum(dXf, M >> 1, L.Fin) if x_shift else dXf
                xa_w = ops.amax_of(X) if fold_in is not None else None
                with side_ctx(keep, X, gy, E1, E2):
                    Pw, Pb, nch = ops.gemm_tn_rows(gph, 1, B, X, L.Fin, x_shift, [gy, E1, E2], L.Fout, True, a_amax=xa_w,
                                                   g_amax=ops.amax_of(gy, gph, B), g_bits=gph.plane_bits, a_act=fold_in)
                    Pw2, Pb2, nch2 = ops.gemm_tn_rows(gph, 2, B, X, L.Fin, x_shift, [gy], L.Fout, False, a_amax=xa_w,
                                                      a_act=fold_in)
                    tg = tgt(f"cl.{L.ci}.weight", f"cl.{L.ci}.bias")
                    dW, db = ops.weight_grad_unpack2(Pw, Pb, nch, Pw2, Pb2, nch2, gph.fake_a, gph.fake_b, L.Fout,
                                                     L.Fin, *(tg or ()))
                    keep.extend((Pw, Pb, Pw2, Pb2))
                    if tg is not None:
                        ready(f"cl.{L.ci}.weight", f"cl.{L.ci}.bias")
                if tg is None:
                    grads[P[f"cl.{L.ci}.weight"]], grads[P[f"cl.{L.ci}.bias"]] = dW, db
                del Pw, Pb, Pw2, Pb2, E1, E2, dXf
            elif _bwd_forward_form(L):
                E1, E2 = ops.cheb_basis_fwd(gph, gy, B, L.Fout, 0)
                Wl = params[P[f"cl.{L.ci}.weight"]]
                if cws is not None and L.ci in cws.images:
                    W3x = cws.images[L.ci][2]
                else:
                    W3x = wc.get((L.ci, "w3x"), Wl, lambda: ops.weight_split(
                        W2, wc.get((L.ci, "amax"), Wl, lambda: ops.param_amax(Wl))))
                (dX,), _ = ops.gemm_planes([gy, E1, E2], L.Fout, 0, W2, None, M, L.Fin, 1, False,
                                           addend=G if fuse_res else None, pair_out=bool(x_shift), Bx=W3x,
                                           amax=ops.amax_of(gy), amax_bits=gph.plane_bits)
                with side_ctx(keep, X, gy, E1, E2):
                    Pw, Pb, nch = ops.gemm_tn([X], L.Fin, x_shift, [gy, E1, E2], M, K_CHEB * L.Fout,
                                              g_amax=ops.amax_of(gy), g_bits=gph.plane_bits)
                    tg = tgt(f"cl.{L.ci}.weight", f"cl.{L.ci}.bias")
                    if tg is not None:
                        ops.weight_grad_unpack(Pw, Pb, nch, L.Fout, L.Fin, K_CHEB, dW=tg[0], db=tg[1], layout=1)
                        ready(f"cl.{L.ci}.weight", f"cl.{L.ci}.bias")
                    else:
                        dW, db = ops.weight_grad_unpack(Pw, Pb, nch, L.Fout, L.Fin, K_CHEB, layout=1)
                    keep.extend((Pw, Pb))
                if tg is None:
                    grads[P[f"cl.{L.ci}.weight"]], grads[P[f"cl.{L.ci}.bias"]] = dW, db
                del Pw, Pb, E1, E2
            else:
                Pw, Pb, nch = ops.gemm_tn([X, T1, T2], L.Fin, x_shift, gy, M, L.Fout, a_amax=ops.amax_of(X),
                                          a_bits=gph.plane_bits)
                tg = tgt(f"cl.{L.ci}.weight", f"cl.{L.ci}.bias")
                if tg is not None:
                    ops.weight_grad_unpack(Pw, Pb, nch, L.Fout, L.Fin, K_CHEB, dW=tg[0], db=tg[1])
                    ready(f"cl.{L.ci}.weight", f"cl.{L.ci}.bias")
                else:
                    dW, db = ops.weight_grad_unpack(Pw, Pb, nch, L.Fout, L.Fin, K_CHEB)
                    grads[P[f"cl.{L.ci}.weight"]], grads[P[f"cl.{L.ci}.bias"]] = dW, db
                del Pw, Pb
                d, _ = ops.gemm_planes([gy], L.Fout, 0, W2, None, M, K_CHEB * L.Fin, K_CHEB, False)
                dX = ops.cheb_basis_bwd(gph, d[0], d[1], d[2], G if fuse_res else None, B, L.Fin, x_shift)
            if has_res and not fuse_res:
                Gs = (Gs_block if Gs_block is not None else ops.pair_sum(G, M >> 1, Fblk, classes=gph)) if x_shift else G
                ops.lerp_bwd_add(Gs, dX, M >> x_shift, Fblk, L.Fin)
            saved[L.ci] = None
            g_cur = dX
            if L.first_in_block:
                G = dX
                Gs_block = None
        if side is not None:
            main_stream.wait_stream(side)
        keep.clear()
        ctx.saved = None
        gx = None
        if ctx.needs_input_grad[2]:
            gx = g_cur.view(ctx.x_shape)
        return (None, None, gx) + tuple(grads)


class Pose2Mesh(nn.Module):

    def __init__(self, num_joint_input_chan, num_mesh_output_chan, graph_L, mano=None):
        super().__init__()
        self.num_joint_input_chan = num_joint_input_chan
        self.num_mesh_output_chan = num_mesh_output_chan
        graph_L = list(graph_L)
        if mano is None:
            mano = _cfg_says_mano()
        if mano is None:
            if len(graph_L) not in (7, 10):
                raise ValueError(f"cannot infer SMPL/MANO topology from {len(graph_L)} graph levels; pass mano=")
            mano = len(graph_L) == 7
        self.mano = bool(mano)
        self.CL_F = channel_plan(self.mano, num_joint_input_chan, num_mesh_output_chan)
        self.CL_K = [K_CHEB] * len(self.CL_F)
        need = len(self.CL_F)
        if len(graph_L) != need:
            raise ValueError(f"{'MANO' if self.mano else 'SMPL'} topology needs {need} graph levels "
                             f"(levels={need - 1} in build_coarse_graphs), got {len(graph_L)}")
        del graph_L[-2]
        self.graph_L = graph_L
        self.num_joint = int(graph_L[-1].shape[0])
        self._Vc = int(graph_L[-2].shape[0])
        for a, b in zip(graph_L[:-2], graph_L[1:-1]):
            if a.shape[0] != 2 * b.shape[0]:
                raise ValueError("mesh levels must halve exactly (binary coarsening tree)")
        self.fc = nn.Linear(self.num_joint * self.CL_F[0][-1], self._Vc * self.CL_F[1][0])

        cl, bn, layers = [], [], []
        nblk = len(self.CL_F)
        for i, blk in enumerate(self.CL_F):
            for l in range(len(blk) - 1):
                Fin, Fout = blk[l], blk[l + 1]
                lin = nn.Linear(K_CHEB * Fin, Fout)
                scale = np.sqrt(2.0 / (K_CHEB * Fin + Fout))
                lin.weight.data.uniform_(-scale, scale)
                lin.bias.data.fill_(0.0)
                cl.append(lin)
                last = (i == nblk - 1 and l == len(blk) - 2)
                bn.append(None if last else nn.BatchNorm1d(Fout))
                ldx = -(i + 1) + (1 if i == nblk - 1 else 0)
                layers.append(_Layer(ci=len(cl) - 1, block=i, graph=len(graph_L) + ldx, Fin=Fin, Fout=Fout,
                                     has_bn=not last, first_in_block=(l == 0), last_in_block=(l == len(blk) - 2)))
        self.cl = nn.ModuleList(cl)
        self.bn = nn.ModuleList(bn)
        self._layers = layers
        self._block_first = {L.block: i for i, L in enumerate(layers) if L.first_in_block}
        self._class_rep = {}
        self._graph_cache = ops.GraphCache(graph_L, class_plan=self._class_plan)
        self._weight_cache = ops.WeightCache()
        self._conv_weight_sets = {}
        self._direct_grad = False
        self._grad_sink = None
        self._infer_real_only = False
        self._out_perm, self._out_nv, self._out_scale, self._out_index = None, 0, 1.0, {}
        self._tap = None
        names, _ = self._param_list()
        self._param_index = {n: i for i, n in enumerate(names)}

    def _class_plan(self, graphs):
        nblk = len(self.CL_F)
        chain = [self._layers[self._block_first[b]].graph for b in range(1, nblk - 1)]
        if not any(graphs[gi].split for gi in chain):
            return None
        seen = False
# ... 104 lines not shown
```

pose2mesh_release_amd/ops.py:

```python
import ctypes
import os as _os
import threading

import numpy as np
import torch

from . import _lib
from ._lib import P2MError, check

_vp = ctypes.c_void_p


def _p(t):
    return None if t is None else _vp(t.data_ptr())


def _stream():
    return _vp(torch.cuda.current_stream().cuda_stream)


def _req(t, name):
    if not (isinstance(t, torch.Tensor) and t.is_cuda and t.dtype == torch.float32 and t.is_contiguous()):
        raise P2MError(f"{name}: expected a contiguous fp32 tensor on the GPU (got "
                       f"{type(t).__name__} {getattr(t, 'dtype', None)} {getattr(t, 'device', None)}); "
# ... 369 lines not shown
        if t.numel() != B * g.V * F:
            raise P2MError("amax_of: the tensor is not a [B, V, F] tensor of this level (un-pooled operands must come "
                           "tagged from their producer)")
        check(_lib.hip().p2m_amax_rows(g.handle, row_set, _p(_req(t, "x")), B, F, _p(w), _stream()), "p2m_amax_rows")
    else:
        check(_lib.hip().p2m_amax(_p(_req(t, "x")), t.numel(), _p(w), _stream()), "p2m_amax")
    tag_amax(t, w)
    return w


WEIGHT_EPOCH = 0


def bump_weight_epoch():
    global WEIGHT_EPOCH
    WEIGHT_EPOCH += 1


class WeightCache:
    def __init__(self):
        self._d = {}
        self.builds = 0

    def get(self, key, W, builder):
        Ws = W if isinstance(W, tuple) else (W,)
        tag = tuple((t.data_ptr(), t._version) for t in Ws) + (WEIGHT_EPOCH,)
        key = (key, Ws[0].device.index)
        hit = self._d.get(key)
        if hit is not None and hit[0] == tag:
            return hit[1]
        val = builder()
        self.builds += 1
        self._d[key] = (tag, val)
        return val

    def clear(self):
        self._d.clear()


def _amax_planes(planes, g=None, B=None):
    if len(planes) == 1:
        return amax_of(planes[0], g, B)
    w = new_amax(planes[0].device)
    for i, t in enumerate(planes):
        if i == 0 and g is not None:
            check(_lib.hip().p2m_amax_rows(g.handle, 0, _p(_req(t, "x")), B, t.shape[-1], _p(w), _stream()), "p2m_amax_rows")
        else:
            check(_lib.hip().p2m_amax(_p(_req(t, "x")), t.numel(), _p(w), _stream()), "p2m_amax")
    return w


def gemm_kernel_name():
    return "k_gemm_planes<" if GEMM_ARITH == "f32" else "k_gemm_planes_ws"


def arith_code():
    return {"f32": 0, "bf16x3": 1, "f16x2": 2}[GEMM_ARITH]


def weight_split(Bm, amax=None, bits=0):
    if GEMM_ARITH == "f32":
        return None
    K, N = Bm.shape
    lib = _lib.hip()
    Bx = torch.empty((int(lib.p2m_weight_split_elems(K, N, arith_code())),), device=Bm.device, dtype=torch.int16)
    check(lib.p2m_weight_split(_p(_req(Bm, "B")), K, N, arith_code(), _p(amax), int(bits), _p(Bx), _stream()),
          "p2m_weight_split")
    return Bx


def param_amax(W):
    if not f16x2():
        return None
    w = new_amax(W.device)
    check(_lib.hip().p2m_amax(_p(_req(W, "weight")), W.numel(), _p(w), _stream()), "p2m_amax")
    return w


def eff_bits(a, b):
    return int(np.ceil(np.log2(1.0 + abs(a) + abs(b)) - 1e-12))


def gemm_planes_rows(g, row_set, B, A, Ka, a0_shift, compact, Bm, bias, addend, C, N, stats=False, Bx=None, act=None,
                     amax=None, amax_bits=0, amax_out=None, in_act=None):
    n = g.set_size(row_set)
    if in_act is not None and amax is None and f16x2():
        raise P2MError("gemm_planes_rows: activation on load needs the amax word of the activated operand (act_bound)")
    if f16x2() and amax is None:
        amax = _amax_planes(A, g if (a0_shift == 0 and row_set <= 2) else None, B)
    st = None
    if stats:
        tps = int(_lib.hip().p2m_rows_tiles_per_sample(g.handle, row_set))
        st = torch.empty((B * tps, 2, N), device=C.device, dtype=torch.float32)
    a = [_p(_req(t, "A plane")) for t in A] + [None] * (3 - len(A))
    fl = 2.0 * B * n * len(A) * Ka * N
    with _timed("gemm_planes_mfma", (fl, fl, 4.0 * B * n * (len(A) * Ka + N))):
        check(_lib.hip().p2m_gemm_planes_rows(g.handle, row_set, B, a[0], a[1], a[2], len(A), Ka, a0_shift,
                                              int(compact), _p(_req(Bm, "B")),
                                              _p(Bx if Bx is not None else weight_split(Bm)), arith_code(), _p(amax),
                                              int(amax_bits),
                                              _p(bias if bias is None else _req(bias, "bias")),
                                              _p(addend if addend is None else _req(addend, "addend")), _p(C), N,
                                              _p(st), _p(None if act is None else act[0]),
                                              _p(None if act is None else act[1]), int(bool(act and act[2])),
                                              _p(amax_out), _p(None if in_act is None else _req(in_act[0], "in_scale")),
                                              _p(None if in_act is None else _req(in_act[1], "in_shift")), _stream()),
              "p2m_gemm_planes_rows")
    return st


_side_streams = {}
_side_lock = threading.Lock()


def side_stream(device, which=0):
    key = (torch.device(device).index, which)
    st = _side_streams.get(key)
    if st is None:
        with _side_lock:
            st = _side_streams.get(key)
            if st is None:
                st = torch.cuda.Stream(device=device)
                _side_streams[key] = st
    return st


class _ConvWeightsDesc(ctypes.Structure):
    _fields_ = [("W", _vp), ("Fout", ctypes.c_int32), ("Fin", ctypes.c_int32), ("fake_a", ctypes.c_float),
                ("fake_b", ctypes.c_float), ("eff_bits", ctypes.c_int32), ("reserved", ctypes.c_int32),
                ("Bx_f", _vp), ("Bx_ef", _vp), ("Bx_b", _vp), ("Bx_eb", _vp), ("amax", _vp)]


class ConvWeightSet:

    def __init__(self, entries, device):
        self.device = torch.device(device)
        self.keys = [k for k, _, _, _ in entries]
        self.weights = [w for _, w, _, _ in entries]
        self.coef = [(float(a), float(b)) for _, _, a, b in entries]
        lib = _lib.hip()
        code = arith_code()
        self.arith = code
        self.images = {}
        for k, w in zip(self.keys, self.weights):
            Fout, Fin = w.shape[0], w.shape[1] // 3
            shapes = ((3 * Fin, Fout), (Fin, Fout), (3 * Fout, Fin), (Fout, Fin))
            self.images[k] = tuple(torch.zeros((int(lib.p2m_weight_split_elems(K, N, code)),), device=self.device,
                                               dtype=torch.int16) for K, N in shapes)
        self.words = torch.zeros((len(entries),), device=self.device, dtype=torch.int32)
        self.desc = None
        self._ptrs = None
        self.tag = None

    def _upload(self):
        arr = (_ConvWeightsDesc * len(self.keys))()
        for i, (k, w, (a, b)) in enumerate(zip(self.keys, self.weights, self.coef)):
            f, ef, bw, eb = self.images[k]
            arr[i] = _ConvWeightsDesc(_req(w, "weight").data_ptr(), w.shape[0], w.shape[1] // 3, a, b, eff_bits(a, b), 0,
                                      f.data_ptr(), ef.data_ptr(), bw.data_ptr(), eb.data_ptr(),
                                      self.words[i:i + 1].data_ptr())
        host = torch.frombuffer(bytearray(bytes(arr)), dtype=torch.uint8)
        self.desc = host.to(self.device)
        self._ptrs = [w.data_ptr() for w in self.weights]

    def refresh(self):
        tag = tuple((w.data_ptr(), w._version) for w in self.weights) + (WEIGHT_EPOCH,)
        if tag == self.tag:
            return
        if self.desc is None or self._ptrs != [w.data_ptr() for w in self.weights]:
            self._upload()
        check(_lib.hip().p2m_conv_weights_prepare(_p(self.desc), len(self.keys), self.arith, _stream()),
              "p2m_conv_weights_prepare")
        self.tag = tag

    def fwd(self, key, dummy):
        f, ef, _, _ = self.images[key]
        return f, dummy, ef

    def bwd(self, key, dummy):
        _, _, b, eb = self.images[key]
        return b, dummy, eb


def split_operands(Bm, Ka, N, fake_a, fake_b, amax=None):
    We = weight_eff(Bm, Ka, N, fake_a, fake_b)
    return weight_split(Bm, amax), We, weight_split(We, amax, eff_bits(fake_a, fake_b) if amax is not None else 0)


def cheb_basis_pair(g, G, B, F):
    P1 = torch.empty((B * g.n_pair_real, F), device=G.device, dtype=torch.float32)
    P2 = torch.empty((B * g.n_pair_real, F), device=G.device, dtype=torch.float32)
    with _timed("cheb_basis_fwd", (4.0 * F * B * (g.V + 2.0 * g.n_pair_real), 12.0 * B * g.V * F)):
        check(_lib.hip().p2m_cheb_basis_pair(g.handle, _p(_req(G, "G")), _p(P1), _p(P2), B, F, _stream()),
              "p2m_cheb_basis_pair")
    return P1, P2


def tile_gemm_ok(g, plan, Ka, N, want_planes=False, B=None):
    if TILE_GEMM in ("0", False) or GEMM_ARITH == "f32":
        return False
    if not _lib.hip().p2m_cheb_tile_gemm_supported(g.handle, plan, Ka, N):
        return False
    if TILE_GEMM in ("1", True):
        return True
    if plan == 2:
        return False
    if _lib.hip().p2m_cheb_tile_gemm_mg(arith_code(), N):
        return g.n_real >= TILE_GEMM_MG_MIN_ROWS
    if GEMM_ARITH == "bf16x3":
        return g.n_real >= TILE_GEMM_MG_MIN_ROWS and (B is None or B >= TILE_GEMM_MIN_BATCH)
    return not want_planes and g.n_real >= TILE_GEMM_MIN_ROWS and (B is None or B >= TILE_GEMM_MIN_BATCH)


def tile_bnr_slots(g, plan, N, B):
    if not BN_FUSE or GEMM_ARITH == "f32":
        return 0
    return int(_lib.hip().p2m_cheb_tile_gemm_bnr_slots(g.handle, plan, arith_code(), N, B))


def cheb_tile_gemm(g, plan, X, A0, Ka, Bx, bias, addend, C, N, B, stats=False, want_planes=False, act=None,
                   amax=None, amax_out=None, in_act=None, bnr=None):
    nset = g.n_pair_real if plan == 2 else g.n_real
    if in_act is not None and amax is None and f16x2():
        raise P2MError("cheb_tile_gemm: activation on load needs the amax word of the activated operand (act_bound)")
    if f16x2() and amax is None:
        amax = amax_of(X, g if plan != 1 else None, B)
    st = torch.empty((B * g.plan_tiles[plan], 2, N), device=C.device, dtype=torch.float32) if stats else None
    E1 = torch.empty((B * nset, Ka), device=C.device, dtype=torch.float32) if want_planes else None
    E2 = torch.empty((B * nset, Ka), device=C.device, dtype=torch.float32) if want_planes else None
    fl = 2.0 * B * nset * 3 * Ka * N
    nbytes = 4.0 * B * nset * (Ka + N + (2 * Ka if want_planes else 0) + (N if addend is not None else 0))
    with _timed("cheb_tile_gemm", (fl, fl, nbytes)):
        check(_lib.hip().p2m_cheb_tile_gemm(g.handle, plan, _p(_req(X, "X")), _p(_req(A0, "A0")), Ka, _p(Bx),
                                            arith_code(), _p(amax),
                                            _p(bias if bias is None else _req(bias, "bias")),
                                            _p(addend if addend is None else _req(addend, "addend")), _p(C), N, _p(st),
                                            _p(E1), _p(E2), _p(None if act is None else act[0]),
                                            _p(None if act is None else act[1]), int(bool(act and act[2])),
                                            _p(amax_out), _p(None if in_act is None else _req(in_act[0], "in_scale")),
                                            _p(None if in_act is None else _req(in_act[1], "in_shift")),
                                            _p(None if bnr is None else _req(bnr[0], "bnr_y")),
                                            _p(None if bnr is None else _req(bnr[1], "bnr_co")),
                                            _p(None if bnr is None else bnr[2]), B, _stream()),
              "p2m_cheb_tile_gemm")
    return st, ((E1, E2) if want_planes else None)


def bn_finalize_tiles(g, plan, B, st_real, st_fake, gamma, beta, running_mean, running_var, momentum, eps):
    N = gamma.shape[0]
    co = torch.empty((4, N), device=gamma.device, dtype=torch.float32)
    check(_lib.hip().p2m_bn_finalize_tiles(g.handle, plan, _p(st_real), _p(st_fake), B, _p(_req(gamma, "bn.weight")),
                                           _p(_req(beta, "bn.bias")), _p(running_mean), _p(running_var),
                                           float(momentum), float(eps), _p(co[0]), _p(co[1]), _p(co[2]), _p(co[3]), N,
                                           _stream()), "p2m_bn_finalize_tiles")
    return co


def conv_pair(g, B, Gy, Ka, Bm, addend, C, N, operands, P0=None, amax_out=None):
    if P0 is None:
        P0 = pair_sum(Gy, B * (g.V // 2), Ka, classes=g)
    Bx, We, Wex = operands
    ga = amax_of(Gy, g, B)
    if tile_gemm_ok(g, 2, Ka, N, want_planes=True, B=B):
        _, (P1c, P2c) = cheb_tile_gemm(g, 2, Gy, P0, Ka, Bx, None, addend, C, N, B, want_planes=True, amax=ga,
                                       amax_out=amax_out)
    else:
        P1c, P2c = cheb_basis_pair(g, Gy, B, Ka)
        gemm_planes_rows(g, 3, B, [P0, P1c, P2c], Ka, 0, True, Bm, None, addend, C, N, False, Bx=Bx, amax=ga,
                         amax_bits=g.plane_bits + 1, amax_out=amax_out)
    gemm_planes_rows(g, 4, B, [P0], Ka, 0, False, We, None, addend, C, N, False, Bx=Wex, amax=ga, amax_bits=1,
                     amax_out=amax_out)
    return P0, P1c, P2c


BASIS_TILED = _os.environ.get("P2M_BASIS_TILED", "1") == "1"


def fold_act_ok(g, Ka, N, B, narrow=False):
    if not (FOLD_ACT and GEMM_ARITH != "f32" and g.split and Ka <= 256 and Ka % 32 == 0):
        return False
    if narrow:
        return bool(g.classes)
    if tile_gemm_ok(g, 0, Ka, N, False, B=B):
        return True
    return bool(BASIS_TILED and g.plan_tiles[0] > 0 and (Ka in (32, 64) or Ka % 128 == 0) and N % 32 == 0
                and not tile_gemm_ok(g, 0, Ka, N, False, B=B))


def act_bound(scale, shift, y_amax, word):
    check(_lib.hip().p2m_act_bound(_p(_req(scale, "scale")), _p(_req(shift, "shift")), scale.shape[0], _p(y_amax),
                                   _p(word), _stream()), "p2m_act_bound")
    return word


def conv_split(g, B, X, Ka, a0_shift, Bm, bias, addend, C, N, fake_a, fake_b, stats=False, operands=None, want_planes=True,
               amax_out=None, in_act=None, bnr=None):
    Bx, We, Wex = operands if operands is not None else split_operands(Bm, Ka, N, fake_a, fake_b)
    xa = amax_of(X, g if a0_shift == 0 else None, B)
    if in_act is not None:
        if a0_shift != 0 or want_planes:
            raise P2MError("conv_split: activation on load needs the level's own plan and no planes out (fold_act_ok)")
        if tile_gemm_ok(g, 0, Ka, N, False, B=B):
            st1, _ = cheb_tile_gemm(g, 0, X, X, Ka, Bx, bias, addend, C, N, B, stats=stats, amax=xa, amax_out=amax_out,
                                    in_act=in_act)
            tiled = True
        else:
            T1c, T2c = cheb_basis_fwd_real(g, X, B, Ka, 0, in_act=in_act)
            st1 = gemm_planes_rows(g, 1, B, [X, T1c, T2c], Ka, 0, True, Bm, bias, addend, C, N, stats, Bx=Bx, amax=xa,
                                   amax_bits=g.plane_bits, amax_out=amax_out, in_act=in_act)
            tiled = False
        st2 = gemm_planes_rows(g, 2, B, [X], Ka, 0, False, We, bias, addend, C, N, stats, Bx=Wex, amax=xa,
                               amax_out=amax_out, in_act=in_act)
        return None, None, st1, st2, tiled
    if bnr is not None and not (in_act is None and tile_gemm_ok(g, a0_shift, Ka, N, want_planes, B=B)):
        raise P2MError("conv_split: bnr needs the tile kernel (tile_bnr_slots > 0 and tile_gemm_ok)")
    if tile_gemm_ok(g, a0_shift, Ka, N, want_planes, B=B):
        st1, planes = cheb_tile_gemm(g, a0_shift, X, X, Ka, Bx, bias, addend, C, N, B, stats=stats,
                                     want_planes=want_planes, amax=xa, amax_out=amax_out, bnr=bnr)
        st2 = gemm_planes_rows(g, 2, B, [X], Ka, a0_shift, False, We, bias, addend, C, N, stats, Bx=Wex, amax=xa,
                               amax_out=amax_out)
        T1c, T2c = planes if planes is not None else (None, None)
        return T1c, T2c, st1, st2, True
    T1c, T2c = cheb_basis_fwd_real(g, X, B, Ka, a0_shift)
    st1 = gemm_planes_rows(g, 1, B, [X, T1c, T2c], Ka, a0_shift, True, Bm, bias, addend, C, N, stats, Bx=Bx, amax=xa,
                           amax_bits=g.plane_bits, amax_out=amax_out)
    st2 = gemm_planes_rows(g, 2, B, [X], Ka, a0_shift, False, We, bias, addend, C, N, stats, Bx=Wex, amax=xa,
                           amax_out=amax_out)
    return T1c, T2c, st1, st2, False


TN_TARGET_BLOCKS = int(_os.environ.get("P2M_TN_TARGET_BLOCKS", "192"))
TN_SAMPLES_PER_CHUNK = _os.environ.get("P2M_TN_SPC", "1") == "1"


def gemm_tn_rows(g, row_set, B, A, Ka, a0_shift, G, Gc, compact, a_amax=None, g_amax=None, g_bits=0, a_act=None,
                 samples_per_chunk=None):
    n = g.set_size(row_set)
    if a_act is not None and a_amax is None and f16x2():
        raise P2MError("gemm_tn_rows: activation on load needs the amax word of the activated operand (act_bound)")
    if f16x2():
        if a_amax is None:
            a_amax = amax_of(A, g if (a0_shift == 0 and row_set <= 2) else None, B)
        if g_amax is None:
            g_amax = _amax_planes(G, g if row_set <= 2 else None, B)
    N = len(G) * Gc
    ntiles = ((Ka + 127) // 128) * ((N + 127) // 128)
    splits = max(1, -(-TN_TARGET_BLOCKS // (B * ntiles)))
    nch = B * splits
    spc = (B * ntiles) // TN_TARGET_BLOCKS if (TN_SAMPLES_PER_CHUNK and GEMM_ARITH != "f32") else 1
    if samples_per_chunk is not None:
        spc = int(samples_per_chunk)
    if spc >= 2:
        splits, nch = -spc, -(-B // spc)
    P = torch.empty((nch, Ka, N), device=A.device, dtype=torch.float32)
# ... 11 lines not shown

def weight_eff(Wt, Ka, N, a, b):
    We = torch.empty((Ka, N), device=Wt.device, dtype=torch.float32)
    check(_lib.hip().p2m_weight_eff(_p(_req(Wt, "Wt")), _p(We), Ka, N, float(a), float(b), _stream()), "p2m_weight_eff")
    return We


def weight_grad_unpack2(P, Pdb, nch, P2, Pdb2, nch2, s1, s2, Fout, Fin, dW=None, db=None):
    acc = 1 if dW is not None else 0
    if dW is None:
        dW = torch.empty((Fout, Fin * 3), device=P.device, dtype=torch.float32)
        db = torch.empty((Fout,), device=P.device, dtype=torch.float32)
    check(_lib.hip().p2m_weight_grad_unpack2(_p(P), _p(Pdb), nch, _p(P2), _p(Pdb2), nch2, float(s1), float(s2), _p(dW),
                                             _p(db), Fout, Fin, 3, acc, _stream()), "p2m_weight_grad_unpack2")
    return dW, db


def bn_finalize_rows(g, B, st_real, st_fake, gamma, beta, running_mean, running_var, momentum, eps):
    N = gamma.shape[0]
    co = torch.empty((4, N), device=gamma.device, dtype=torch.float32)
    check(_lib.hip().p2m_bn_finalize_split(g.handle, _p(st_real), _p(st_fake), B, _p(_req(gamma, "bn.weight")),
                                           _p(_req(beta, "bn.bias")), _p(running_mean), _p(running_var),
                                           float(momentum), float(eps), _p(co[0]), _p(co[1]), _p(co[2]), _p(co[3]), N,
                                           _stream()), "p2m_bn_finalize_split")
    return co


def weight_pack(W, Fin, K, need_w2=True, need_w3=False):
    Fout = W.shape[0]
    Wt = torch.empty((K * Fin, Fout), device=W.device, dtype=torch.float32)
    W2 = torch.empty((Fout, K * Fin), device=W.device, dtype=torch.float32) if need_w2 else None
    W3 = torch.empty((K * Fout, Fin), device=W.device, dtype=torch.float32) if need_w3 else None
    check(_lib.hip().p2m_weight_pack(_p(_req(W, "weight")), _p(Wt), _p(W2), _p(W3), Fout, Fin, K, _stream()),
          "p2m_weight_pack")
    return Wt, W2, W3


def gemm_planes(A, Ka, a0_shift, Bm, bias, M, N, nplanesC=1, stats=False, addend=None, pair_out=False, Bx=None,
                act=None, amax=None, amax_bits=0, want_amax=False):
    dev = A[0].device
    Nc = N // nplanesC
    C = [torch.empty((M >> 1 if pair_out else M, Nc), device=dev, dtype=torch.float32) for _ in range(nplanesC)]
    st = None
    if stats:
        nt = (M + stats_tile_rows() - 1) // stats_tile_rows()
        st = torch.empty((nt, 2, N), device=dev, dtype=torch.float32)
    a = [_p(_req(t, "A plane")) for t in A] + [None] * (3 - len(A))
    c = [_p(t) for t in C] + [None] * (3 - len(C))
    mfma = (Ka % 32 == 0) and (Nc % 32 == 0)
    if not mfma:
        Bx = None
    elif Bx is None:
        Bx = weight_split(Bm)
    amax_out = None
    if mfma and f16x2():
        if amax is None:
            amax = _amax_planes(A)
        if want_amax and nplanesC == 1:
            amax_out = new_amax(dev)
            tag_amax(C[0], amax_out)
    fl = 2.0 * M * len(A) * Ka * N
    nbytes = 4.0 * M * ((len(A) - 1 + 1.0 / (1 << a0_shift)) * Ka + (0.5 if pair_out else 1.0) * N
                        + (N if addend is not None else 0))
    with _timed("gemm_planes_mfma" if mfma else "gemm_planes_valu", (fl, fl, nbytes)):
        check(_lib.hip().p2m_gemm_planes(a[0], a[1], a[2], len(A), Ka, a0_shift, _p(_req(Bm, "B")), _p(Bx),
                                         arith_code() if mfma else 0, _p(amax), int(amax_bits),
                                         _p(bias if bias is None else _req(bias, "bias")),
                                         _p(addend if addend is None else _req(addend, "addend")), c[0], c[1], c[2],
                                         nplanesC, Nc, int(pair_out), M, _p(st),
                                         _p(None if act is None else act[0]), _p(None if act is None else act[1]),
                                         int(bool(act and act[2])), _p(amax_out), _stream()), "p2m_gemm_planes")
    return C, st


def pick_chunk_rows(M, ntiles_out, target_blocks=None, quantum=32):
    if target_blocks is None:
        target_blocks = TN_TARGET_BLOCKS
    nchunks = max(1, min((target_blocks + ntiles_out - 1) // ntiles_out, (M + 255) // 256))
    rows = (M + nchunks - 1) // nchunks
    rows = ((rows + quantum - 1) // quantum) * quantum
    return rows


def gemm_tn(A, Ka, a0_shift, G, M, N, a_amax=None, a_bits=0, g_amax=None, g_bits=0, tname=None, target_blocks=None):
    Gl = list(G) if isinstance(G, (list, tuple)) else [G]
    G = Gl[0]
    Gc = N // len(Gl)
    Ktot = len(A) * Ka
    ntiles = ((Ktot + 127) // 128) * ((N + 127) // 128)
    mfma = (Ka % 4 == 0) and (N % 32 == 0) and Ktot >= 32 and Gc % 4 == 0
    chunk_rows = pick_chunk_rows(M, ntiles, target_blocks) if mfma else 32
    nchunks = (M + chunk_rows - 1) // chunk_rows
    P = torch.empty((nchunks, Ktot, N), device=G.device, dtype=torch.float32)
    Pdb = torch.empty((nchunks, N), device=G.device, dtype=torch.float32)
    a = [_p(_req(t, "A plane")) for t in A] + [None] * (3 - len(A))
    gp = [_p(_req(t, "G plane")) for t in Gl] + [None] * (3 - len(Gl))
    if mfma and f16x2():
        if a_amax is None:
            a_amax = _amax_planes(A)
        if g_amax is None:
            g_amax = _amax_planes(Gl)
    with _timed(tname or ("gemm_tn_mfma" if mfma else "gemm_tn_valu"),
                (2.0 * M * Ktot * N, 2.0 * M * Ktot * N, 4.0 * M * (Ktot + N))):
        check(_lib.hip().p2m_gemm_tn(a[0], a[1], a[2], len(A), Ka, a0_shift, gp[0], gp[1], gp[2], len(Gl), Gc, M,
                                     chunk_rows, _p(P), _p(Pdb), arith_code() if mfma else 0, _p(a_amax), int(a_bits),
                                     _p(g_amax), int(g_bits), _stream()), "p2m_gemm_tn")
    return P, Pdb, nchunks


def weight_grad_unpack(P, Pdb, nchunks, Fout, Fin, K, dW=None, db=None, layout=0):
    acc = 1 if dW is not None else 0
    if dW is None:
        dW = torch.empty((Fout, Fin * K), device=P.device, dtype=torch.float32)
        db = torch.empty((Fout,), device=P.device, dtype=torch.float32) if Pdb is not None else None
    check(_lib.hip().p2m_weight_grad_unpack(_p(P), _p(Pdb), nchunks, _p(dW), _p(db if Pdb is not None else None), Fout, Fin,
                                            K, acc, layout, Pdb.shape[1] if Pdb is not None else 0, _stream()),
          "p2m_weight_grad_unpack")
    return dW, db


def bn_finalize(stats, M, gamma, beta, running_mean, running_var, momentum, eps, tile_rows=None):
    N = gamma.shape[0]
    if tile_rows is None:
        tile_rows = stats_tile_rows()
    ntiles = (M + tile_rows - 1) // tile_rows
    co = torch.empty((4, N), device=gamma.device, dtype=torch.float32)
    check(_lib.hip().p2m_bn_finalize(_p(stats), ntiles, M, _p(_req(gamma, "bn.weight")),
                                     _p(_req(beta, "bn.bias")), _p(running_mean), _p(running_var),
                                     float(momentum), float(eps), _p(co[0]), _p(co[1]), _p(co[2]), _p(co[3]), N,
                                     tile_rows, _stream()), "p2m_bn_finalize")
    return co


def bn_eval_coeffs(gamma, beta, running_mean, running_var, eps):
    N = gamma.shape[0]
    co = torch.empty((4, N), device=gamma.device, dtype=torch.float32)
    check(_lib.hip().p2m_bn_eval_coeffs(_p(_req(gamma, "bn.weight")), _p(_req(beta, "bn.bias")),
                                        _p(_req(running_mean, "running_mean")), _p(_req(running_var, "running_var")),
                                        float(eps), _p(co[0]), _p(co[1]), _p(co[2]), _p(co[3]), N, _stream()),
          "p2m_bn_eval_coeffs")
    return co


def bn_act_fwd(y, co, relu, resid, Fres, res_shift, M, F, classes=None, real_rows=None):
    x = torch.empty((M, F), device=y.device, dtype=torch.float32)
    sc = None if co is None else co[2]
    sh = None if co is None else co[3]
    cls = classes.handle if (classes is not None and classes.classes) else None
    if real_rows is not None:
        cls = real_rows.handle
    mode = 1 if real_rows is not None else 0
    word = new_amax(y.device) if (f16x2() and F % 4 == 0) else None
    check(_lib.hip().p2m_bn_act_fwd(_p(_req(y, "y")), _p(sc), _p(sh), int(relu),
                                    _p(resid if resid is None else _req(resid, "resid")), int(Fres), int(res_shift),
                                    _p(x), M, F, cls, mode, _p(word), _stream()), "p2m_bn_act_fwd")
    if word is not None:
        tag_amax(x, word)
    return x


def bnr_parts(g, plan, N, B, device):
    slots = tile_bnr_slots(g, plan, N, B)
    if slots <= 0:
        return None
    nfake = int(_lib.hip().p2m_bn_bwd_blocks_fake(g.handle, B, N)) if g.n_fake > 0 else 0
    part = torch.empty((nfake + slots, 2, N), device=device, dtype=torch.float32)
    return part, nfake


def bn_relu_bwd(gx, y, co, gamma, relu, training, M, F, dgamma=None, dbeta=None, pair_in=False, pair_out=False,
                classes=None, zero_holes=False, real_part=None):
    lib = _lib.hip()
    cls = classes.handle if (classes is not None and classes.classes) else None
    if real_part is not None:
        gfr, part, nfake = real_part
        nblk = part.shape[0]
    else:
        nblk = int(lib.p2m_bn_bwd_blocks(M, F) if cls is None else lib.p2m_bn_bwd_blocks_classes(cls, M, F))
        part = torch.empty((nblk, 2, F), device=y.device, dtype=torch.float32)
    acc = 1 if dgamma is not None else 0
    if dgamma is None:
        dgb = torch.empty((2, F), device=y.device, dtype=torch.float32)
        dgamma, dbeta = dgb[0], dgb[1]
    coef = torch.empty((2, F), device=y.device, dtype=torch.float32)
    if real_part is not None:
        if nfake > 0:
# ... 103 lines not shown
```

pose2mesh_release_amd/posenet.py:

```python
import os
import sys

import torch
import torch.nn as nn
import torch.nn.functional as F

from . import ops
from .cheby_graph_conv import bn_momentum

HIP_POSENET = os.environ.get("P2M_POSENET", "hip")
if HIP_POSENET not in ("hip", "stock"):
    raise ValueError(f"P2M_POSENET must be hip or stock, not {HIP_POSENET!r}")
_PN_BLOCKS = 512
_PAD = 64


def _reference_cfg():
    mod = sys.modules.get("core.config")
    return getattr(mod, "cfg", None) if mod is not None else None


def cfg_posenet_pretrained():
    cfg = _reference_cfg()
    try:
        return bool(cfg.MODEL.posenet_pretrained) if cfg is not None else False
    except AttributeError:
        return False


def load_checkpoint(load_dir, epoch=0, pick_best=False):
    fu = sys.modules.get("funcs_utils")
    if fu is not None and hasattr(fu, "load_checkpoint"):
        return fu.load_checkpoint(load_dir=load_dir, epoch=epoch, pick_best=pick_best)
    try:
        print(f"Fetch model weight from {load_dir}")
        return torch.load(load_dir, map_location="cuda" if torch.cuda.is_available() else "cpu")
    except Exception as e:
        raise ValueError("No checkpoint exists!\n", e)


def _wt(W):
    return ops.weight_pack(W, W.shape[1], 1, need_w2=False)[0]


def _pad_rows(W, rows):
    out = W.new_zeros((rows, W.shape[1]))
    out[:W.shape[0]] = W.detach()
    return out


class _PoseNetFn(torch.autograd.Function):

    @staticmethod
    def forward(ctx, net, keep, x, *params):
        with torch.cuda.device(x.device):
            return _PoseNetFn._forward(ctx, net, keep, x, params)

    @staticmethod
    def _forward(ctx, net, keep, x, params):
        wc = net._weight_cache
        names, _ = net._param_list()
        P = {n: t for n, t in zip(names, params)}
        Br, Fh = x.shape[0], net.linear_size
        B = max(32, (Br + 3) // 4 * 4)
        nin, nout = net.input_size, net.output_size
        training = net.training
        p_drop = [float(st.dropout.p) for st in net.linear_stages]
        nst = len(net.linear_stages)
        x = x.contiguous().float()
        if training and Br == 1 and nst > 0:
            raise ValueError(f"Expected more than 1 value per channel when training, got input size {[Br, Fh]}")

        aux = {}

        def amax_w(key, W):
            w = wc.get((key, "amax"), W, lambda: ops.param_amax(W))
            aux[key] = w
            return w

        def lin_fwd(a_T, key, W):
            Wt = wc.get((key, "t"), W, lambda: _wt(W))
            return ops.gemm_tn([a_T], B, 0, Wt, W.shape[1], W.shape[0], a_amax=ops.amax_of(a_T), g_amax=amax_w(key, W),
                               tname="pn_gemm", target_blocks=_PN_BLOCKS)

        def bn_of(i, sub):
            m = getattr(net.linear_stages[i], sub)
            track = m.track_running_stats and m.running_mean is not None
            use_batch = training or not track
            return (P[f"linear_stages.{i}.{sub}.weight"], P[f"linear_stages.{i}.{sub}.bias"],
                    m.running_mean if track else None, m.running_var if track else None,
                    bn_momentum(m) if (track and use_batch) else 0.1, m.eps, use_batch), m

        rnd = None
        if training and any(p > 0.0 for p in p_drop):
            rnd = torch.rand((2 * nst, B, Fh), device=x.device, dtype=torch.float32)
        nbt = []
        saved = {"x": x, "rnd": rnd, "stages": []}
        xp = F.pad(x, (0, _PAD - nin, 0, B - Br))
        W1 = P["w1.weight"]
        W1t = wc.get(("w1", "tpad"), W1, lambda: _pad_rows(W1.t(), _PAD))
        Pp, _, nch = ops.gemm_tn([xp.t().contiguous()], B, 0, W1t, _PAD, Fh, g_amax=amax_w("w1", W1), tname="pn_gemm", target_blocks=_PN_BLOCKS)
        bias = P["w1.bias"]
        resid = None
        y = None
        for i in range(nst):
            bn1, m1 = bn_of(i, "batch_norm1")
            y, a1, a1T, mu1, is1 = ops.pn_stage_fwd(Pp, nch, B, Fh, bias=bias, resid=resid, bn=bn1, B_real=Br,
                                                    rnd=None if rnd is None else rnd[2 * i], p_drop=p_drop[i])
            Wa = P[f"linear_stages.{i}.w1.weight"]
            Pp, _, nch = lin_fwd(a1T, f"s{i}.w1", Wa)
            bn2, m2 = bn_of(i, "batch_norm2")
            z1, a2, a2T, mu2, is2 = ops.pn_stage_fwd(Pp, nch, B, Fh, bias=P[f"linear_stages.{i}.w1.bias"], bn=bn2, B_real=Br,
                                                     rnd=None if rnd is None else rnd[2 * i + 1], p_drop=p_drop[i])
            Wb = P[f"linear_stages.{i}.w2.weight"]
            Pp, _, nch = lin_fwd(a2T, f"s{i}.w2", Wb)
            bias, resid = P[f"linear_stages.{i}.w2.bias"], y
            tap = getattr(net, "_tap", None)
            if tap is not None:
                tap.append((2 * i, y, mu1, is1, bn1[0], bn1[1]))
                tap.append((2 * i + 1, z1, mu2, is2, bn2[0], bn2[1]))
            if training:
                for m in (m1, m2):
                    if m.track_running_stats and m.num_batches_tracked is not None:
                        nbt.append(m.num_batches_tracked)
            if keep:
                saved["stages"].append((y, a1, mu1, is1, z1, a2, mu2, is2, bn1[6], bn2[6]))
            del a1T, a2T
        y_last, _, yT, _, _ = ops.pn_stage_fwd(Pp, nch, B, Fh, bias=bias, resid=resid, want_a=False, B_real=Br)
        W2 = P["w2.weight"]
        W2p = wc.get(("w2", "pad"), W2, lambda: _pad_rows(W2, _PAD))
        W2t = wc.get(("w2", "tpad"), W2, lambda: _wt(W2p))
        aux["W2p"] = W2p
        Pp, _, nch = ops.gemm_tn([yT], B, 0, W2t, Fh, _PAD, a_amax=ops.amax_of(yT), g_amax=amax_w("w2", W2),
                                 tname="pn_gemm", target_blocks=_PN_BLOCKS)
        b2 = wc.get(("w2", "bpad"), P["w2.bias"], lambda: F.pad(P["w2.bias"].detach(), (0, _PAD - nout)))
        out64, _, _, _, _ = ops.pn_stage_fwd(Pp, nch, B, _PAD, bias=b2, want_a=False, want_aT=False, B_real=Br)
        if nbt:
            torch._foreach_add_(nbt, 1)
            ops.bump_weight_epoch()
        saved["y_last"], saved["aux"] = y_last, aux
        ctx.net, ctx.saved, ctx.params, ctx.names = net, (saved if keep else None), params, names
        ctx.training, ctx.p_drop, ctx.B, ctx.Br, ctx.ran = training, p_drop, B, Br, False
        return out64[:Br, :nout].contiguous()

    @staticmethod
    def backward(ctx, g_out):
        with torch.cuda.device(g_out.device):
            return _PoseNetFn._backward(ctx, g_out)

    @staticmethod
    def _backward(ctx, g_out):
        net, saved, params, names = ctx.net, ctx.saved, ctx.params, ctx.names
        if saved is None:
            if ctx.ran:
                raise ops.P2MError("PoseNet: backward called a second time - the saved activations are freed by the first "
                                   "backward (retain_graph is not supported on this path)")
            raise ops.P2MError("backward called but the forward ran without gradient tracking")
        ctx.ran = True
        wc = net._weight_cache
        P = {n: t for n, t in zip(names, params)}
        idx = {n: i for i, n in enumerate(names)}
        B, Br, Fh = ctx.B, ctx.Br, net.linear_size
        nin, nout = net.input_size, net.output_size
        nst = len(net.linear_stages)
        rnd, p_drop = saved["rnd"], ctx.p_drop
        needs = {n: bool(ctx.needs_input_grad[3 + i]) for i, n in enumerate(names)}
        dev = g_out.device
        grads = [None] * len(params)
        direct = net._direct_grad and all(
            p.grad is not None and p.grad.dtype == torch.float32 and p.grad.is_contiguous() and p.grad.device == dev
            for p in params if p.requires_grad)

        aux = saved["aux"]

        def amax_w(key, W):
            return aux[key] if key in aux else wc.get((key, "amax"), W, lambda: ops.param_amax(W))

        def target(name, shape=None):
            if not needs[name]:
                return None
            if direct:
                return P[name].grad
            t = torch.zeros_like(P[name])
            grads[idx[name]] = t
            return t

        def ready(*ns):
            if direct and net._grad_sink is not None:
                net._grad_sink([P[n] for n in ns if needs[n]])

        g = g_out.contiguous().float()
        g64 = F.pad(g, (0, _PAD - nout, 0, B - Br))
        g64T = g64.t().contiguous()
        y_last = saved["y_last"]
        W2 = P["w2.weight"]
        if needs["w2.weight"]:
            Pw, _, _ = ops.gemm_tn([g64], _PAD, 0, y_last, B, Fh, tname="pn_gemm", target_blocks=_PN_BLOCKS)
            target("w2.weight").add_(Pw.sum(0)[:nout] if Pw.shape[0] > 1 else Pw[0, :nout])
        if needs["w2.bias"]:
            target("w2.bias").add_(g.sum(0))
        ready("w2.weight", "w2.bias")
        W2p = aux["W2p"]
        Pg, _, nchg = ops.gemm_tn([g64T], B, 0, W2p, _PAD, Fh, g_amax=amax_w("w2", W2), tname="pn_gemm", target_blocks=_PN_BLOCKS)
        gz2 = gz2T = None
        for i in reversed(range(nst)):
            y, a1, mu1, is1, z1, a2, mu2, is2, tr1, tr2 = saved["stages"][i]
            pre = f"linear_stages.{i}."
            if gz2 is None:
                gz2, gz2T = ops.pn_stage_bwd(Pg, nchg, B, Fh, dbias=target(pre + "w2.bias"), accumulate=True, B_real=Br)
            Wb = P[pre + "w2.weight"]
            if needs[pre + "w2.weight"]:
                ops.gemm_tn_acc(gz2, a2, target(pre + "w2.weight"))
            ready(pre + "w2.weight", pre + "w2.bias")
            Pa, _, nch = ops.gemm_tn([gz2T], B, 0, Wb, Fh, Fh, a_amax=ops.amax_of(gz2T), g_amax=amax_w(f"s{i}.w2", Wb),
                                     tname="pn_gemm", target_blocks=_PN_BLOCKS)
            gz1, gz1T = ops.pn_stage_bwd(Pa, nch, B, Fh, bn=(z1, mu2, is2, P[pre + "batch_norm2.weight"],
                                                            P[pre + "batch_norm2.bias"], tr2),
# ... 117 lines not shown
```

Before: 6788.

## Fuse residual lerp into conv GEMM epilogue, read untransposed weights, vectorize combine loads

Adds a GEMM-planes epilogue variant that reads a half-width residual addend and broadcasts each value with a 0.5 factor, so the separate lerp_bwd_add pass in backward can be skipped. Adds a transposed-G path to the TN GEMM so PoseNet linear layers read the weight matrix directly rather than a cached transposed copy, and drops the bias-gradient reduction on that path. Also vectorizes the small Chebyshev combine kernel with float4 row loads and XCD-aware block mapping. All three add template variants and eligibility checks, and the strided weight loads in the transposed path may coalesce less well.

```diff
diff --git a/include/p2m.h b/include/p2m.h
--- a/include/p2m.h
+++ b/include/p2m.h
@@ -74,6 +74,9 @@
                 int32_t a0_shift, const float* G0, const float* G1, const float* G2, int32_t nplanesG,
                 int32_t Gc, int64_t M, int64_t chunk_rows, float* P, float* Pdb, int32_t arith,
                 const void* a_amax, int32_t a_bits, const void* g_amax, int32_t g_bits, void* stream);
+int p2m_gemm_tn_gt(const float* A0, const float* A1, const float* A2, int32_t nplanesA, int32_t Ka,
+                   int32_t a0_shift, const float* Gt, int32_t N, int64_t M, int64_t chunk_rows, float* P, float* Pdb,
+                   int32_t arith, const void* a_amax, int32_t a_bits, const void* g_amax, int32_t g_bits, void* stream);
 
 int p2m_bn_finalize(const float* stats, int32_t ntiles, int64_t M, const float* gamma, const float* beta,
                     float* running_mean, float* running_var, float momentum, float eps,
@@ -118,6 +121,13 @@
                          const float* bias, const float* addend, float* C,
                          int32_t N, float* stats, const float* act_scale, const float* act_shift, int32_t act_relu,
                          void* amax_out, const float* in_scale , const float* in_shift, void* stream);
+int32_t p2m_gemm_planes_rows_lerp_ok(const float* addend_half, const float* C, int32_t N, int32_t arith);
+int p2m_gemm_planes_rows_lerp(p2m_graph_t g, int32_t row_set, int32_t B, const float* A0, const float* A1,
+                              const float* A2, int32_t nplanesA, int32_t Ka, int32_t a0_shift, int32_t planes_compact,
+                              const float* Bm, const void* Bsplit, int32_t arith, const void* a_amax, int32_t a_bits,
+                              const float* bias, const float* addend_half, float* C, int32_t N, const float* act_scale,
+                              const float* act_shift, int32_t act_relu, void* amax_out, const float* in_scale ,
+                              const float* in_shift, void* stream);
 int32_t p2m_rows_tiles_per_sample(p2m_graph_t g, int32_t row_set);
 int p2m_gemm_tn_rows(p2m_graph_t g, int32_t row_set, int32_t B, const float* A, int32_t Ka, int32_t a0_shift,
                      const float* G0, const float* G1, const float* G2, int32_t nplanesG, int32_t Gc,
diff --git a/pose2mesh_release_amd/_lib.py b/pose2mesh_release_amd/_lib.py
--- a/pose2mesh_release_amd/_lib.py
+++ b/pose2mesh_release_amd/_lib.py
@@ -38,6 +38,9 @@
     "p2m_cheb_basis_pair": (_c.c_int, [_vp, _vp, _vp, _vp, _i32, _i32, _vp]),
     "p2m_gemm_planes_rows": (_c.c_int, [_vp, _i32, _i32, _vp, _vp, _vp, _i32, _i32, _i32, _i32, _vp, _vp, _i32, _vp, _i32,
                                         _vp, _vp, _vp, _i32, _vp, _vp, _vp, _i32, _vp, _vp, _vp, _vp]),
+    "p2m_gemm_planes_rows_lerp_ok": (_i32, [_vp, _vp, _i32, _i32]),
+    "p2m_gemm_planes_rows_lerp": (_c.c_int, [_vp, _i32, _i32, _vp, _vp, _vp, _i32, _i32, _i32, _i32, _vp, _vp, _i32, _vp, _i32,
+                                             _vp, _vp, _vp, _i32, _vp, _vp, _i32, _vp, _vp, _vp, _vp]),
     "p2m_rows_tiles_per_sample": (_i32, [_vp, _i32]),
     "p2m_gemm_tn_rows": (_c.c_int, [_vp, _i32, _i32, _vp, _i32, _i32, _vp, _vp, _vp, _i32, _i32, _i32, _i32, _vp, _vp,
                                     _i32, _vp, _vp, _i32, _vp, _vp, _vp]),
@@ -75,6 +78,8 @@
     "p2m_stats_tile_rows": (_i32, []),
     "p2m_gemm_tn": (_c.c_int, [_vp, _vp, _vp, _i32, _i32, _i32, _vp, _vp, _vp, _i32, _i32, _i64, _i64, _vp, _vp,
                                _i32, _vp, _i32, _vp, _i32, _vp]),
+    "p2m_gemm_tn_gt": (_c.c_int, [_vp, _vp, _vp, _i32, _i32, _i32, _vp, _i32, _i64, _i64, _vp, _vp,
+                                  _i32, _vp, _i32, _vp, _i32, _vp]),
     "p2m_bn_finalize": (_c.c_int, [_vp, _i32, _i64, _vp, _vp, _vp, _vp, _f32, _f32, _vp, _vp, _vp, _vp,
                                    _i32, _i32, _vp]),
     "p2m_bn_eval_coeffs": (_c.c_int, [_vp, _vp, _vp, _vp, _f32, _vp, _vp, _vp, _vp, _i32, _vp]),
diff --git a/pose2mesh_release_amd/csrc/basis.hip b/pose2mesh_release_amd/csrc/basis.hip
--- a/pose2mesh_release_amd/csrc/basis.hip
+++ b/pose2mesh_release_amd/csrc/basis.hip
@@ -243,7 +243,7 @@
 }
 
 constexpr int SMALL_SPB = 8;
-template <int NC>
+template <int NC, bool ROWS>
 __global__ __launch_bounds__(256) void k_combine_small_tile(TilePlan pl, const int* __restrict__ real_ids, int V,
                                                              const float* __restrict__ P, int ldp,
                                                              const float* __restrict__ bias, float* __restrict__ Y, int B,
@@ -252,7 +252,9 @@
   __shared__ float4 ents[TILE_ECAP];
   __shared__ int rowoff[TILE_RMAX + 1];
   __shared__ float xs[SMALL_SPB][TILE_UCAP][2 * NC];
-  const int tile = blockIdx.x % pl.ntiles, sg = blockIdx.x / pl.ntiles;
+  static_assert(!ROWS || NC == 3, "the float4 loads are laid out for nine values per row");
+  const int bid = ROWS ? xcd_block_id(blockIdx.x, gridDim.x) : (int)blockIdx.x;
+  const int tile = bid % pl.ntiles, sg = bid / pl.ntiles;
   const int t = threadIdx.x;
   const int r0 = pl.tile_row[tile], R = pl.tile_row[tile + 1] - r0;
   const int u0 = pl.tile_u[tile], U = pl.tile_u[tile + 1] - u0;
@@ -263,9 +265,16 @@
   for (int q = t; q < U * SMALL_SPB; q += 256) {
     const int u = q % U, sl = q / U, b = b0 + sl;
     if (b < B) {
-      const float* src = P + ((long)b * V + pl.ucol[u0 + u]) * ldp + NC;
-#pragma unroll
-      for (int c = 0; c < 2 * NC; c++) xs[sl][u][c] = src[c];
+      const float* src = P + ((long)b * V + pl.ucol[u0 + u]) * ldp;
+      if constexpr (ROWS) {
+        const float4* s4 = reinterpret_cast<const float4*>(src);
+        const float4 q0 = s4[0], q1 = s4[1], q2 = s4[2];
+        float* x = xs[sl][u];
+        x[0] = q0.w; x[1] = q1.x; x[2] = q1.y; x[3] = q1.z; x[4] = q1.w; x[5] = q2.x;
+      } else {
+#pragma unroll
+        for (int c = 0; c < 2 * NC; c++) xs[sl][u][c] = src[NC + c];
+      }
     }
   }
   __syncthreads();
@@ -274,8 +283,15 @@
   const int row = real_ids[r0 + i];
   const float* p0 = P + ((long)b * V + row) * ldp;
   float acc[NC];
-#pragma unroll
-  for (int c = 0; c < NC; c++) acc[c] = p0[c] + (bias ? bias[c] : 0.f);
+  if constexpr (ROWS) {
+    const float4 q0 = *reinterpret_cast<const float4*>(p0);
+    acc[0] = q0.x + (bias ? bias[0] : 0.f);
+    acc[1] = q0.y + (bias ? bias[1] : 0.f);
+    acc[2] = q0.z + (bias ? bias[2] : 0.f);
+  } else {
+#pragma unroll
+    for (int c = 0; c < NC; c++) acc[c] = p0[c] + (bias ? bias[c] : 0.f);
+  }
   for (int j = rowoff[i]; j < rowoff[i + 1]; j++) {
     const float4 en = ents[j];
     const float* q = xs[sl][__float_as_int(en.z)];
@@ -465,8 +481,13 @@
   int skip_real = 0;
   const TilePlan& pl = g.plan[0];
   if (pl.ntiles > 0 && basis_tiled() && nc == 3) {
-    hipLaunchKernelGGL(k_combine_small_tile<3>, dim3(pl.ntiles * cdiv(B, SMALL_SPB)), dim3(256), 0, s, pl, g.real_ids, g.V,
-                       P, ldp, bias, Y, B, out_index, out_rows, scale);
+    const bool rows16 = ldp % 4 == 0 && (reinterpret_cast<uintptr_t>(P) & 15) == 0 && narrow_rows();
+    if (rows16)
+      hipLaunchKernelGGL((k_combine_small_tile<3, true>), dim3(pl.ntiles * cdiv(B, SMALL_SPB)), dim3(256), 0, s, pl,
+                         g.real_ids, g.V, P, ldp, bias, Y, B, out_index, out_rows, scale);
+    else
+      hipLaunchKernelGGL((k_combine_small_tile<3, false>), dim3(pl.ntiles * cdiv(B, SMALL_SPB)), dim3(256), 0, s, pl,
+                         g.real_ids, g.V, P, ldp, bias, Y, B, out_index, out_rows, scale);
     if (real_only) return check_launch("cheb_combine_small(tiled)");
     skip_real = 1;
   }
diff --git a/pose2mesh_release_amd/csrc/gemm.hip b/pose2mesh_release_amd/csrc/gemm.hip
--- a/pose2mesh_release_amd/csrc/gemm.hip
+++ b/pose2mesh_release_amd/csrc/gemm.hip
@@ -35,6 +35,7 @@
   unsigned* amax_out;
   const float* in_scale;
   const float* in_shift;
+  int addend_half = 0;
 };
 
 __device__ __forceinline__ bool tile_of_block(int bid, int ntm, int ntn, int& mt, int& nt) {
@@ -123,7 +124,11 @@
       Cb[j] = reinterpret_cast<char*>(Cq + (pair ? rowbase >> 1 : rowbase) * g.Nc);
       c4[j] = (unsigned)(n - q * g.Nc) * 4u;
     }
-    const char* const Ab = reinterpret_cast<const char*>(g.addend + (EXTRA && g.addend != nullptr ? rowbase * g.Nc : 0));
+    constexpr bool HALF_OK = EXTRA && ROWS && CO;
+    const int hs = HALF_OK ? g.addend_half : 0;
+    const char* const Ab = HALF_OK
+        ? reinterpret_cast<const char*>(g.addend) + (g.addend != nullptr ? (rowbase * g.Nc * 4) >> hs : 0)
+        : reinterpret_cast<const char*>(g.addend + (EXTRA && g.addend != nullptr ? rowbase * g.Nc : 0));
     constexpr unsigned NOROW = 0xFFFFFFFFu;
 
     auto row_offsets = [&](int gi, unsigned (&ro)[4]) {
@@ -242,7 +247,7 @@
         const int q = (nu >= g.Nc ? 1 : 0) + (nu >= 2 * g.Nc ? 1 : 0);
         ju[j] = nu < g.N;
         Cc[j] = Cb[j] + (unsigned)(nu - q * g.Nc) * 4u;
-        Ac[j] = Ab + (ADD && ju[j] ? (unsigned)nu * 4u : 0u);
+        Ac[j] = Ab + (ADD && ju[j] ? ((unsigned)nu * 4u) >> hs : 0u);
         rd[j] = strip + (rd0 ^ (j * 32));
       }
       auto co_row = [&](int gi) {
@@ -264,9 +269,17 @@
       for (int j = 0; j < TN; j++) asm volatile("" : "+v"(bias_v[j]), "+v"(sc_v[j]), "+v"(sh_v[j]));
       auto stage = [&](int gi) {
         if constexpr (ADD) {
-          const unsigned lo = ro_nxt != NOROW ? ro_nxt : col16;
-#pragma unroll
-          for (int j = 0; j < TN; j++) ad[gi & 1][j] = *reinterpret_cast<const f32x4*>(Ac[j] + lo);
+          const unsigned lo = (ro_nxt != NOROW ? ro_nxt : col16) >> hs;
+          if (hs) {
+#pragma unroll
+            for (int j = 0; j < TN; j++) {
+              const f32x2 h = *reinterpret_cast<const f32x2*>(Ac[j] + lo);
+              ad[gi & 1][j] = __builtin_shufflevector(h, h, 0, 1, -1, -1);
+            }
+          } else {
+#pragma unroll
+            for (int j = 0; j < TN; j++) ad[gi & 1][j] = *reinterpret_cast<const f32x4*>(Ac[j] + lo);
+          }
         }
         __builtin_amdgcn_sched_barrier(0);
         const int i = gi >> 2, r0 = (gi & 3) * 4;
@@ -308,7 +321,14 @@
 #pragma unroll
         for (int j = 0; j < TN; j++) {
           f32x4 v = cp[j];
-          if constexpr (ADD) v += ad[gi & 1][j];
+          if constexpr (ADD) {
+            if (hs) {
+              const float h0 = fmaf(0.5f, ad[gi & 1][j][0], 0.f), h1 = fmaf(0.5f, ad[gi & 1][j][1], 0.f);
+              v += f32x4{h0, h0, h1, h1};
+            } else {
+              v += ad[gi & 1][j];
+            }
+          }
           const bool ok = ro_cur != NOROW && ju[j];
           if (ok) *reinterpret_cast<f32x4*>(Cc[j] + ro_cur) = v;
           const float m4 = fmaxf(fmaxf(amax_abs(v[0]), amax_abs(v[1])), fmaxf(amax_abs(v[2]), amax_abs(v[3])));
@@ -1317,8 +1337,9 @@
 #define P2M_TNT(s, ev) do { } while (0)
 #endif
 
-template <int BN, bool ROWS, int NS>
+template <int BN, bool ROWS, int NS, bool GT = false>
 __global__ __launch_bounds__(512, 2) void k_gemm_tn_ws(TnArgs g) {
+  static_assert(!(GT && ROWS), "the transposed G exists in flat mode only");
   typedef typename SliceFrag<NS>::type frag_t;
   constexpr int RK = 16;
   constexpr int LDX = RK + 8;
@@ -1393,9 +1414,9 @@
     } else {
       int n = n0 + c4 * 4;
       if (n >= g.N) n = 0;
-      const int gq = n / g.Gc;
-      src = g.G[gq] + (n - gq * g.Gc);
-      pitch = g.Gc;
+      const int gq = GT ? 0 : n / g.Gc;
+      src = GT ? g.G[0] + (long)n * g.M : g.G[gq] + (n - gq * g.Gc);
+      pitch = GT ? 1 : g.Gc;
       shift = 0;
       compact_rows = ROWS && gq != 0 && g.compact;
       dst = Gs + (c4 >> 2) * 16 * LDX + (c4 & 3) * 2 * LDX + rq * 4;
@@ -1424,6 +1445,8 @@
   const long samp_bytes = ROWS ? (((long)(compact_rows ? g.nset : g.V) >> shift) * pitch) * 4 : 0;
   const unsigned pitch4 = (unsigned)pitch * 4u;
   const int nrows_m1 = (int)(r_end - r_begin) - 1;
+  const bool gt_role = GT && !is_a;
+  const unsigned gt_pitch4 = GT ? (unsigned)g.M * 4u : 0u;
 
   f32x4 x0[4], x1[4];
   i32x4 id0 = {0, 0, 0, 0}, id1 = {0, 0, 0, 0};
@@ -1435,6 +1458,14 @@
   };
   auto load_stage = [&](int kc, f32x4 (&x)[4], const i32x4& id, auto clamp_tag) {
     constexpr bool CLAMP = decltype(clamp_tag)::value;
+    if (gt_role) {
+      int rel = kc * RK + rq * 4;
+      if (CLAMP && rel > nrows_m1 - 3) rel = nrows_m1 - 3;
+      const unsigned off = (unsigned)rel * 4u;
+#pragma unroll
+      for (int e = 0; e < 4; e++) x[e] = *reinterpret_cast<const f32x4*>(srcb + (off + (unsigned)e * gt_pitch4));
+      return;
+    }
 #pragma unroll
     for (int ps = 0; ps < 4; ps++) {
       int rel = kc * RK + rq * 4 + ps;
@@ -1461,22 +1492,36 @@
     }
     if (TAIL) {
       const int rlast = nrows_m1 + 1 - (kc * RK + rq * 4);
-#pragma unroll
-      for (int ps = 0; ps < 4; ps++)
-        if (ps >= rlast) x[ps] = f32x4{0.f, 0.f, 0.f, 0.f};
-    }
-    if (!is_a) {
+      if (gt_role) {
+#pragma unroll
+        for (int e = 0; e < 4; e++)
+#pragma unroll
+          for (int ps = 0; ps < 4; ps++)
+            if (ps >= rlast) x[e][ps] = 0.f;
+      } else {
+#pragma unroll
+        for (int ps = 0; ps < 4; ps++)
+          if (ps >= rlast) x[ps] = f32x4{0.f, 0.f, 0.f, 0.f};
+      }
+    }
+    if (!GT && !is_a) {
 #pragma unroll
       for (int ps = 0; ps < 4; ps++) dbs += x[ps];
     }
     unsigned short* d = dst + buf * buf_stride;
+    if (gt_role) asm volatile("" : "+v"(x[0]), "+v"(x[1]), "+v"(x[2]), "+v"(x[3]));
 #pragma unroll
     for (int e = 0; e < 4; e++) {
       u32x2 sl[NS];
 #ifdef P2M_TN_ABL_NOSLICE
       for (int q = 0; q < NS; q++) sl[q] = u32x2{__float_as_uint(x[q & 1][e]), __float_as_uint(x[2 + (q & 1)][e])};
 #else
-      split_pack4<NS>(x[0][e], x[1][e], x[2][e], x[3][e], my_sc, sl);
+      if (gt_role) {
+        split_pack4<NS>(x[e][0], x[e][1], x[e][2], x[e][3], my_sc, sl);
+        asm volatile("" : "+v"(sl[0]), "+v"(sl[NS - 1]));
+      } else {
+        split_pack4<NS>(x[0][e], x[1][e], x[2][e], x[3][e], my_sc, sl);
+      }
 #endif
 #pragma unroll
       for (int q = 0; q < NS; q++)
@@ -1618,7 +1663,7 @@
         }
       }
   }
-  if (kt == 0 && g.Pdb != nullptr) {
+  if (!GT && kt == 0 && g.Pdb != nullptr) {
     float* red = smem;
     if (producer && !is_a && (st >> 2) < BN / 4) *reinterpret_cast<f32x4*>(red + rq * BN + c4 * 4) = dbs;
     __syncthreads();
@@ -2234,6 +2279,17 @@
   return check_launch("gemm_planes");
 }
 
+extern "C" int32_t p2m_gemm_planes_rows_lerp_ok(const float* addend_half, const float* C, int32_t N, int32_t arith) {
+  return (arith == P2M_ARITH_BF16X3 || arith == P2M_ARITH_F16X2) && epi_copyout() && addend_half != nullptr && C != nullptr &&
+         aligned16(addend_half) && aligned16(C) && N > 0 && N % 32 == 0;
+}
+static int gemm_planes_rows_impl(p2m_graph_t gh, int32_t row_set, int32_t B, const float* A0, const float* A1,
+                                 const float* A2, int32_t nplanesA, int32_t Ka, int32_t a0_shift,
+                                 int32_t planes_compact, const float* Bm, const void* Bsplit, int32_t arith,
+                                 const void* a_amax, int32_t a_bits, const float* bias,
+                                 const float* addend, float* C, int32_t N, float* stats, const float* act_scale,
+                                 const float* act_shift, int32_t act_relu, void* amax_out, const float* in_scale,
+                                 const float* in_shift, void* stream, bool addend_half);
 extern "C" int p2m_gemm_planes_rows(p2m_graph_t gh, int32_t row_set, int32_t B, const float* A0, const float* A1,
                                     const float* A2, int32_t nplanesA, int32_t Ka, int32_t a0_shift,
                                     int32_t planes_compact, const float* Bm, const void* Bsplit, int32_t arith,
@@ -2241,6 +2297,30 @@
                                     const float* addend, float* C, int32_t N, float* stats, const float* act_scale,
                                     const float* act_shift, int32_t act_relu, void* amax_out, const float* in_scale,
                                     const float* in_shift, void* stream) {
+  return gemm_planes_rows_impl(gh, row_set, B, A0, A1, A2, nplanesA, Ka, a0_shift, planes_compact, Bm, Bsplit, arith, a_amax,
+                               a_bits, bias, addend, C, N, stats, act_scale, act_shift, act_relu, amax_out, in_scale, in_shift,
+                               stream, false);
+}
+extern "C" int p2m_gemm_planes_rows_lerp(p2m_graph_t gh, int32_t row_set, int32_t B, const float* A0, const float* A1,
+                                         const float* A2, int32_t nplanesA, int32_t Ka, int32_t a0_shift,
+                                         int32_t planes_compact, const float* Bm, const void* Bsplit, int32_t arith,
+                                         const void* a_amax, int32_t a_bits, const float* bias,
+                                         const float* addend_half, float* C, int32_t N, const float* act_scale,
+                                         const float* act_shift, int32_t act_relu, void* amax_out, const float* in_scale,
+                                         const float* in_shift, void* stream) {
+  P2M_CHECK_ARG(p2m_gemm_planes_rows_lerp_ok(addend_half, C, N, arith),
+                "the half-width addend needs a slice arithmetic, the staged copy-out, N % 32 == 0, C and the addend 16-byte aligned");
+  return gemm_planes_rows_impl(gh, row_set, B, A0, A1, A2, nplanesA, Ka, a0_shift, planes_compact, Bm, Bsplit, arith, a_amax,
+                               a_bits, bias, addend_half, C, N, nullptr, act_scale, act_shift, act_relu, amax_out, in_scale,
+                               in_shift, stream, true);
+}
+static int gemm_planes_rows_impl(p2m_graph_t gh, int32_t row_set, int32_t B, const float* A0, const float* A1,
+                                 const float* A2, int32_t nplanesA, int32_t Ka, int32_t a0_shift,
+                                 int32_t planes_compact, const float* Bm, const void* Bsplit, int32_t arith,
+                                 const void* a_amax, int32_t a_bits, const float* bias,
+                                 const float* addend, float* C, int32_t N, float* stats, const float* act_scale,
+                                 const float* act_shift, int32_t act_relu, void* amax_out, const float* in_scale,
+                                 const float* in_shift, void* stream, bool addend_half) {
   P2M_CHECK_ARG(gh && A0 && Bm && C, "null pointer");
   P2M_CHECK_ARG((in_scale == nullptr) == (in_shift == nullptr), "in_scale / in_shift must both be given or both NULL");
   P2M_CHECK_ARG(in_scale == nullptr || (arith != P2M_ARITH_F32 && Ka <= 256),
@@ -2263,6 +2343,7 @@
   for (int p = 0; p < nplanesA; p++) P2M_CHECK_ARG(g.A[p] != nullptr, "missing A plane");
   g.C[0] = C; g.C[1] = nullptr; g.C[2] = nullptr;
   g.Bm = Bm; g.bias = bias; g.addend = addend; g.pair_out = 0; g.stats = stats;
+  g.addend_half = addend_half ? 1 : 0;
   g.act_scale = act_scale; g.act_shift = act_shift; g.act_relu = act_relu;
   g.nplanesA = nplanesA; g.Ka = Ka; g.a0_shift = a0_shift; g.N = N; g.Nc = N;
   g.ids = rs.ids; g.nset = rs.n; g.V = rs.V; g.tps = cdiv(rs.n, BM); g.compact = planes_compact;
@@ -2294,7 +2375,7 @@
                         int32_t a0_shift, const float* G0, const float* G1, const float* G2, int32_t nplanesG,
                         int32_t Gc, int64_t M, int64_t chunk_rows, float* P, float* Pdb, int32_t arith,
                         const void* a_amax, int32_t a_bits, const void* g_amax, int32_t g_bits, int32_t accumulate,
-                        void* stream);
+                        void* stream, bool g_transposed = false);
 extern "C" int p2m_gemm_tn(const float* A0, const float* A1, const float* A2, int32_t nplanesA, int32_t Ka,
                            int32_t a0_shift, const float* G0, const float* G1, const float* G2, int32_t nplanesG,
                            int32_t Gc, int64_t M, int64_t chunk_rows, float* P, float* Pdb, int32_t arith,
@@ -2302,6 +2383,13 @@
   return gemm_tn_impl(A0, A1, A2, nplanesA, Ka, a0_shift, G0, G1, G2, nplanesG, Gc, M, chunk_rows, P, Pdb, arith, a_amax,
                       a_bits, g_amax, g_bits, 0, stream);
 }
+extern "C" int p2m_gemm_tn_gt(const float* A0, const float* A1, const float* A2, int32_t nplanesA, int32_t Ka,
+                              int32_t a0_shift, const float* Gt, int32_t N, int64_t M, int64_t chunk_rows, float* P,
+                              float* Pdb, int32_t arith, const void* a_amax, int32_t a_bits, const void* g_amax,
+                              int32_t g_bits, void* stream) {
+  return gemm_tn_impl(A0, A1, A2, nplanesA, Ka, a0_shift, Gt, nullptr, nullptr, 1, N, M, chunk_rows, P, Pdb, arith, a_amax,
+                      a_bits, g_amax, g_bits, 0, stream, true);
+}
 extern "C" int p2m_gemm_tn_acc(const float* A, int32_t Ka, const float* G, int32_t N, int64_t M, float* P, int32_t arith,
                                const void* a_amax, const void* g_amax, void* stream) {
   const int64_t chunk_rows = ((M + 31) / 32) * 32;
@@ -2312,7 +2400,7 @@
                         int32_t a0_shift, const float* G0, const float* G1, const float* G2, int32_t nplanesG,
                         int32_t Gc, int64_t M, int64_t chunk_rows, float* P, float* Pdb, int32_t arith,
                         const void* a_amax, int32_t a_bits, const void* g_amax, int32_t g_bits, int32_t accumulate,
-                        void* stream) {
+                        void* stream, bool g_transposed) {
   P2M_CHECK_ARG(nplanesA >= 1 && nplanesA <= 3 && nplanesG >= 1 && nplanesG <= 3, "plane count must be 1..3");
   P2M_CHECK_ARG(arith == P2M_ARITH_F32 || arith == P2M_ARITH_BF16X3 || arith == P2M_ARITH_F16X2, "unknown arithmetic");
   P2M_CHECK_ARG(arith != P2M_ARITH_F16X2 || (a_amax && g_amax), "P2M_ARITH_F16X2 needs the amax words of both operands");
@@ -2337,6 +2425,14 @@
   P2M_CHECK_ARG(!accumulate || nchunks == 1, "accumulation needs the whole reduction in one chunk");
   hipStream_t s = (hipStream_t)stream;
   const bool mfma_ok = (Ka % 4 == 0) && (N % 32 == 0) && (Gc % 4 == 0) && (g.Ktot >= 32);
+  const bool gt = g_transposed;
+  if (gt) {
+    P2M_CHECK_ARG(arith != P2M_ARITH_F32 && mfma_ok, "G transposed exists in the slice arithmetics only (Ka % 4, N % 32, Ktot >= 32)");
+    P2M_CHECK_ARG(Pdb == nullptr, "G transposed produces no bias sums: Pdb must be NULL");
+    P2M_CHECK_ARG(nplanesG == 1 && !accumulate, "G transposed: one G plane, no accumulation");
+    P2M_CHECK_ARG(M % 4 == 0 && chunk_rows % 4 == 0 && M < (1l << 27), "G transposed: M and chunk_rows must be multiples of 4, M < 2^27");
+    P2M_CHECK_ARG((reinterpret_cast<uintptr_t>(G0) & 15) == 0, "G transposed must be 16-byte aligned");
+  }
   if (!mfma_ok) {
     g.nkt = g.ntn = 0;
     int nout = g.Ktot * N;
@@ -2349,13 +2445,17 @@
   if (N % 128 == 0 || (bx && N > 128)) {
     g.ntn = cdiv(N, 128);
     const dim3 grid(g.nkt * g.ntn, nchunks), grid_ws((nchunks >= 8 ? cdiv(nchunks, 8) * 8 : nchunks) * g.nkt * g.ntn);
-    if (arith == P2M_ARITH_F16X2) hipLaunchKernelGGL((k_gemm_tn_ws<128, false, 2>), grid_ws, dim3(512), 0, s, g);
+    if (gt && arith == P2M_ARITH_F16X2) hipLaunchKernelGGL((k_gemm_tn_ws<128, false, 2, true>), grid_ws, dim3(512), 0, s, g);
+    else if (gt) hipLaunchKernelGGL((k_gemm_tn_ws<128, false, 3, true>), grid_ws, dim3(512), 0, s, g);
+    else if (arith == P2M_ARITH_F16X2) hipLaunchKernelGGL((k_gemm_tn_ws<128, false, 2>), grid_ws, dim3(512), 0, s, g);
     else if (bx) hipLaunchKernelGGL((k_gemm_tn_ws<128, false, 3>), grid_ws, dim3(512), 0, s, g);
     else hipLaunchKernelGGL((k_gemm_tn<128, false>), grid, dim3(256), 0, s, g);
   } else {
     g.ntn = cdiv(N, 64);
     const dim3 grid(g.nkt * g.ntn, nchunks), grid_ws((nchunks >= 8 ? cdiv(nchunks, 8) * 8 : nchunks) * g.nkt * g.ntn);
-    if (arith == P2M_ARITH_F16X2) hipLaunchKernelGGL((k_gemm_tn_ws<64, false, 2>), grid_ws, dim3(512), 0, s, g);
+    if (gt && arith == P2M_ARITH_F16X2) hipLaunchKernelGGL((k_gemm_tn_ws<64, false, 2, true>), grid_ws, dim3(512), 0, s, g);
+    else if (gt) hipLaunchKernelGGL((k_gemm_tn_ws<64, false, 3, true>), grid_ws, dim3(512), 0, s, g);
+    else if (arith == P2M_ARITH_F16X2) hipLaunchKernelGGL((k_gemm_tn_ws<64, false, 2>), grid_ws, dim3(512), 0, s, g);
     else if (bx) hipLaunchKernelGGL((k_gemm_tn_ws<64, false, 3>), grid_ws, dim3(512), 0, s, g);
     else hipLaunchKernelGGL((k_gemm_tn<64, false>), grid, dim3(256), 0, s, g);
   }
diff --git a/pose2mesh_release_amd/meshnet.py b/pose2mesh_release_amd/meshnet.py
--- a/pose2mesh_release_amd/meshnet.py
+++ b/pose2mesh_release_amd/meshnet.py
@@ -278,10 +278,12 @@
                     fw, fb = params[P["fc.weight"]], params[P["fc.bias"]]
                     Nf, Kf = fw.shape
                     if ops.GEMM_ARITH != "f32" and B % 4 == 0 and B >= 32 and Nf % 32 == 0 and Kf % 32 == 0:
-                        fwt = wc.get("fc_t", fw, lambda: ops.weight_pack(fw, Kf, 1, need_w2=False)[0])
+                        fc_gt = ops.tn_gt_ok(fw, B)
+                        fwt = fw if fc_gt else wc.get("fc_t", fw, lambda: ops.weight_pack(fw, Kf, 1, need_w2=False)[0])
                         ha = ops.amax_of(h)
                         Pu, _, nchu = ops.gemm_tn([ops.tag_amax(h.t().contiguous(), ha)], B, 0, fwt, Kf, Nf, a_amax=ha,
-                                                  g_amax=wc.get("fc_amax", fw, lambda: ops.param_amax(fw)))
+                                                  g_amax=wc.get("fc_amax", fw, lambda: ops.param_amax(fw)),
+                                                  g_transposed=fc_gt)
                         u = (Pu[0] if nchu == 1 else Pu.sum(0)).add_(fb)
                     else:
                         fwt, fwx = wc.get("fc", fw, lambda: _fc_operands(fw, wc.get("fc_amax", fw, lambda: ops.param_amax(fw))))
@@ -443,6 +445,7 @@
             has_res = L.first_in_block and 1 <= L.block <= nblk - 2
             Fblk = net.CL_F[L.block][-1]
             fuse_res = has_res and (L.Fin == Fblk)
+            lerp_done = False
             pair_path = _bwd_forward_form(L) and gph.split and x_shift and gph.pair \
                 and (L.Fout in (32, 64) or L.Fout % 128 == 0)
             want_Gs = want_P0 = False
@@ -479,7 +482,15 @@
                 opb = cws.bwd(L.ci, Wl) if (cws is not None and L.ci in cws.images) else wc.get(
                     (L.ci, "split_bwd"), Wl, lambda: ops.split_operands(W2, L.Fout, L.Fin, gph.fake_a, gph.fake_b,
                                                                       wc.get((L.ci, "amax"), Wl, lambda: ops.param_amax(Wl))))
-                P0, E1, E2 = ops.conv_pair(gph, B, gy, L.Fout, W2, add, dX, L.Fin, opb, P0=P0)
+                lerp_Gs = None
+                if has_res and not fuse_res and L.Fin == 2 * Fblk and not coarse_full:
+                    Gs = Gs_block if Gs_block is not None else ops.pair_sum(G, Mc, Fblk, classes=gph)
+                    if ops.conv_pair_lerp_ok(gph, B, L.Fout, L.Fin, dX, Gs):
+                        lerp_Gs = Gs
+                    else:
+                        Gs_block = Gs
+                P0, E1, E2 = ops.conv_pair(gph, B, gy, L.Fout, W2, add, dX, L.Fin, opb, P0=P0, lerp=lerp_Gs)
+                lerp_done = lerp_Gs is not None
                 ga = ops.amax_of(gy, gph, B)
                 with side_ctx(keep, X, P0, E1, E2):
                     Pw, Pb, nch = ops.gemm_tn_rows(gph, 3, B, X, L.Fin, 0, [P0, E1, E2], L.Fout, True, g_amax=ga,
@@ -565,7 +576,7 @@
                 del Pw, Pb
                 d, _ = ops.gemm_planes([gy], L.Fout, 0, W2, None, M, K_CHEB * L.Fin, K_CHEB, False)
                 dX = ops.cheb_basis_bwd(gph, d[0], d[1], d[2], G if fuse_res else None, B, L.Fin, x_shift)
-            if has_res and not fuse_res:
+            if has_res and not fuse_res and not lerp_done:
                 Gs = (Gs_block if Gs_block is not None else ops.pair_sum(G, M >> 1, Fblk, classes=gph)) if x_shift else G
                 ops.lerp_bwd_add(Gs, dX, M >> x_shift, Fblk, L.Fin)
             saved[L.ci] = None
diff --git a/pose2mesh_release_amd/ops.py b/pose2mesh_release_amd/ops.py
--- a/pose2mesh_release_amd/ops.py
+++ b/pose2mesh_release_amd/ops.py
@@ -475,7 +475,7 @@
 
 
 def gemm_planes_rows(g, row_set, B, A, Ka, a0_shift, compact, Bm, bias, addend, C, N, stats=False, Bx=None, act=None,
-                     amax=None, amax_bits=0, amax_out=None, in_act=None):
+                     amax=None, amax_bits=0, amax_out=None, in_act=None, addend_half=False):
     n = g.set_size(row_set)
     if in_act is not None and amax is None and f16x2():
         raise P2MError("gemm_planes_rows: activation on load needs the amax word of the activated operand (act_bound)")
@@ -487,6 +487,21 @@
         st = torch.empty((B * tps, 2, N), device=C.device, dtype=torch.float32)
     a = [_p(_req(t, "A plane")) for t in A] + [None] * (3 - len(A))
     fl = 2.0 * B * n * len(A) * Ka * N
+    if addend_half:
+        if stats or addend is None:
+            raise P2MError("gemm_planes_rows: the half-width addend excludes stats")
+        with _timed("gemm_planes_mfma", (fl, fl, 4.0 * B * n * (len(A) * Ka + N + N // 2))):
+            check(_lib.hip().p2m_gemm_planes_rows_lerp(g.handle, row_set, B, a[0], a[1], a[2], len(A), Ka, a0_shift,
+                                                       int(compact), _p(_req(Bm, "B")),
+                                                       _p(Bx if Bx is not None else weight_split(Bm)), arith_code(), _p(amax),
+                                                       int(amax_bits), _p(bias if bias is None else _req(bias, "bias")),
+                                                       _p(_req(addend, "addend")), _p(C), N,
+                                                       _p(None if act is None else act[0]),
+                                                       _p(None if act is None else act[1]), int(bool(act and act[2])),
+                                                       _p(amax_out), _p(None if in_act is None else _req(in_act[0], "in_scale")),
+                                                       _p(None if in_act is None else _req(in_act[1], "in_shift")), _stream()),
+                  "p2m_gemm_planes_rows_lerp")
+        return None
     with _timed("gemm_planes_mfma", (fl, fl, 4.0 * B * n * (len(A) * Ka + N))):
         check(_lib.hip().p2m_gemm_planes_rows(g.handle, row_set, B, a[0], a[1], a[2], len(A), Ka, a0_shift,
                                               int(compact), _p(_req(Bm, "B")),
@@ -649,7 +664,23 @@
     return co
 
 
-def conv_pair(g, B, Gy, Ka, Bm, addend, C, N, operands, P0=None, amax_out=None):
+LERP_FUSE = _os.environ.get("P2M_LERP_FUSE", "1") == "1"
+
+
+def conv_pair_lerp_ok(g, B, Ka, N, C, Gs):
+    if not LERP_FUSE or GEMM_ARITH == "f32" or Gs is None or N % 2 or Gs.shape[-1] * 2 != N or not Gs.is_contiguous():
+        return False
+    if tile_gemm_ok(g, 2, Ka, N, want_planes=True, B=B):
+        return False
+    return bool(_lib.hip().p2m_gemm_planes_rows_lerp_ok(_p(Gs), _p(C), N, arith_code()))
+
+
+def conv_pair(g, B, Gy, Ka, Bm, addend, C, N, operands, P0=None, amax_out=None, lerp=None):
+    half = lerp is not None
+    if half:
+        if addend is not None or not conv_pair_lerp_ok(g, B, Ka, N, C, lerp):
+            raise P2MError("conv_pair: lerp= excludes an addend and needs conv_pair_lerp_ok")
+        addend = lerp
     if P0 is None:
         P0 = pair_sum(Gy, B * (g.V // 2), Ka, classes=g)
     Bx, We, Wex = operands
@@ -660,9 +691,9 @@
     else:
         P1c, P2c = cheb_basis_pair(g, Gy, B, Ka)
         gemm_planes_rows(g, 3, B, [P0, P1c, P2c], Ka, 0, True, Bm, None, addend, C, N, False, Bx=Bx, amax=ga,
-                         amax_bits=g.plane_bits + 1, amax_out=amax_out)
+                         amax_bits=g.plane_bits + 1, amax_out=amax_out, addend_half=half)
     gemm_planes_rows(g, 4, B, [P0], Ka, 0, False, We, None, addend, C, N, False, Bx=Wex, amax=ga, amax_bits=1,
-                     amax_out=amax_out)
+                     amax_out=amax_out, addend_half=half)
     return P0, P1c, P2c
 
 
@@ -840,7 +871,17 @@
     return rows
 
 
-def gemm_tn(A, Ka, a0_shift, G, M, N, a_amax=None, a_bits=0, g_amax=None, g_bits=0, tname=None, target_blocks=None):
+TN_GT = _os.environ.get("P2M_TN_GT", "1") == "1"
+
+
+def tn_gt_ok(Gt, Ka, nplanesA=1):
+    N, M = Gt.shape
+    return (TN_GT and GEMM_ARITH != "f32" and Gt.is_contiguous() and Gt.dtype == torch.float32 and M % 4 == 0
+            and M < (1 << 27) and Gt.data_ptr() % 16 == 0 and Ka % 4 == 0 and N % 32 == 0 and nplanesA * Ka >= 32)
+
+
+def gemm_tn(A, Ka, a0_shift, G, M, N, a_amax=None, a_bits=0, g_amax=None, g_bits=0, tname=None, target_blocks=None,
+            g_transposed=False):
     Gl = list(G) if isinstance(G, (list, tuple)) else [G]
     G = Gl[0]
     Gc = N // len(Gl)
@@ -850,7 +891,9 @@
     chunk_rows = pick_chunk_rows(M, ntiles, target_blocks) if mfma else 32
     nchunks = (M + chunk_rows - 1) // chunk_rows
     P = torch.empty((nchunks, Ktot, N), device=G.device, dtype=torch.float32)
-    Pdb = torch.empty((nchunks, N), device=G.device, dtype=torch.float32)
+    if g_transposed and (not mfma or len(Gl) != 1):
+        raise P2MError("gemm_tn: G transposed needs one plane at the shapes of the slice arithmetics (tn_gt_ok)")
+    Pdb = None if g_transposed else torch.empty((nchunks, N), device=G.device, dtype=torch.float32)
     a = [_p(_req(t, "A plane")) for t in A] + [None] * (3 - len(A))
     gp = [_p(_req(t, "G plane")) for t in Gl] + [None] * (3 - len(Gl))
     if mfma and f16x2():
@@ -860,6 +903,11 @@
             g_amax = _amax_planes(Gl)
     with _timed(tname or ("gemm_tn_mfma" if mfma else "gemm_tn_valu"),
                 (2.0 * M * Ktot * N, 2.0 * M * Ktot * N, 4.0 * M * (Ktot + N))):
+        if g_transposed:
+            check(_lib.hip().p2m_gemm_tn_gt(a[0], a[1], a[2], len(A), Ka, a0_shift, gp[0], N, M, chunk_rows, _p(P), None,
+                                            arith_code(), _p(a_amax), int(a_bits), _p(g_amax), int(g_bits), _stream()),
+                  "p2m_gemm_tn_gt")
+            return P, None, nchunks
         check(_lib.hip().p2m_gemm_tn(a[0], a[1], a[2], len(A), Ka, a0_shift, gp[0], gp[1], gp[2], len(Gl), Gc, M,
                                      chunk_rows, _p(P), _p(Pdb), arith_code() if mfma else 0, _p(a_amax), int(a_bits),
                                      _p(g_amax), int(g_bits), _stream()), "p2m_gemm_tn")
diff --git a/pose2mesh_release_amd/posenet.py b/pose2mesh_release_amd/posenet.py
--- a/pose2mesh_release_amd/posenet.py
+++ b/pose2mesh_release_amd/posenet.py
@@ -79,6 +79,9 @@
             return w
 
         def lin_fwd(a_T, key, W):
+            if ops.tn_gt_ok(W, B):
+                return ops.gemm_tn([a_T], B, 0, W, W.shape[1], W.shape[0], a_amax=ops.amax_of(a_T), g_amax=amax_w(key, W),
+                                   tname="pn_gemm", target_blocks=_PN_BLOCKS, g_transposed=True)
             Wt = wc.get((key, "t"), W, lambda: _wt(W))
             return ops.gemm_tn([a_T], B, 0, Wt, W.shape[1], W.shape[0], a_amax=ops.amax_of(a_T), g_amax=amax_w(key, W),
                                tname="pn_gemm", target_blocks=_PN_BLOCKS)
@@ -129,10 +132,11 @@
         y_last, _, yT, _, _ = ops.pn_stage_fwd(Pp, nch, B, Fh, bias=bias, resid=resid, want_a=False, B_real=Br)
         W2 = P["w2.weight"]
         W2p = wc.get(("w2", "pad"), W2, lambda: _pad_rows(W2, _PAD))
-        W2t = wc.get(("w2", "tpad"), W2, lambda: _wt(W2p))
         aux["W2p"] = W2p
+        w2_gt = ops.tn_gt_ok(W2p, B)
+        W2t = W2p if w2_gt else wc.get(("w2", "tpad"), W2, lambda: _wt(W2p))
         Pp, _, nch = ops.gemm_tn([yT], B, 0, W2t, Fh, _PAD, a_amax=ops.amax_of(yT), g_amax=amax_w("w2", W2),
-                                 tname="pn_gemm", target_blocks=_PN_BLOCKS)
+                                 tname="pn_gemm", target_blocks=_PN_BLOCKS, g_transposed=w2_gt)
         b2 = wc.get(("w2", "bpad"), P["w2.bias"], lambda: F.pad(P["w2.bias"].detach(), (0, _PAD - nout)))
         out64, _, _, _, _ = ops.pn_stage_fwd(Pp, nch, B, _PAD, bias=b2, want_a=False, want_aT=False, B_real=Br)
         if nbt:
```

Measured after the change: 6845, median of 6. No clear change (+0.8%).
